# AntoineBlanot/LC2IS

Measured on AMD Instinct MI355X. Metric: training-step images/sec (512x512, ADE20K-150), higher is better.
Workload: dtype bf16; 1 GPU; BaseModelWithText ViT-B/16 + CLIP-text + decoder + fused head/CE train step, 512x512, 151 classes, text len 16, sgd; batch_per_gpu=32, global_batch=32, parallelism=dp1

## Files before the change

include/lc2is_hip.h:

```cpp
#ifndef LC2IS_HIP_H
#define LC2IS_HIP_H
#include <stddef.h>
#include <stdint.h>

#ifdef __cplusplus
extern "C" {
#endif

#define LC2IS_ACT_NONE 0
#define LC2IS_ACT_QUICK_GELU 1
#define LC2IS_ACT_RELU 2
#define LC2IS_ACT_DQUICK_GELU 3
#define LC2IS_ACT_DRELU 4
#define LC2IS_ACT_QUICK_GELU_GRAD 5
#define LC2IS_ACT_MUL_AUX 6
#define LC2IS_ACT_GELU_ERF 7
#define LC2IS_ACT_DGELU_ERF 8
#define LC2IS_ACT_ADD_AUX 9

#define LC2IS_INTERP_BICUBIC 0
#define LC2IS_INTERP_BILINEAR 1

typedef void* lc2is_stream_t;

// ... 29 lines not shown
int lc2is_gemm_tn_bf16(const void* dY, int ldy, const void* X, int ldx, float* dW, int ldw, float* db, int M,
                       int N, int K, int accumulate, void* workspace, size_t workspace_bytes,
                       lc2is_stream_t stream);

#define LC2IS_TN_GROUP_MAX 128
typedef struct lc2is_tn_problem {
  const void* dY; const void* X; float* dW; float* db;
  int ldy, ldx, ldw, M, N, K, accumulate;
} lc2is_tn_problem;
size_t lc2is_gemm_tn_grouped_workspace_bytes(const lc2is_tn_problem* problems, int n);
int lc2is_gemm_tn_grouped(const lc2is_tn_problem* problems, int n, void* workspace, size_t workspace_bytes,
                          lc2is_stream_t stream);
int lc2is_release_captured_tables(void);
int lc2is_captured_tables_mark(void);
int lc2is_release_captured_tables_range(int first, int last);

size_t lc2is_colsum_workspace_bytes(int M, int N);
int lc2is_colsum_bf16(const void* dY, int ldy, float* db, int M, int N, int accumulate, void* workspace,
                      size_t workspace_bytes, lc2is_stream_t stream);

int lc2is_layernorm_fwd(const void* x, int ldx, int x_is_bf16, const float* gamma, const float* beta, void* y_bf16,
                        int ldy, float* y_f32, int ldyf, float* mean, float* rstd, int M, int C, float eps,
                        lc2is_stream_t stream);

size_t lc2is_layernorm_bwd_workspace_bytes(int M, int C);
int lc2is_layernorm_bwd(const void* dy_bf16, int lddy, const float* dy_f32, int lddyf, const void* x,
                        int ldx, int x_is_bf16, const float* gamma, const float* mean, const float* rstd,
                        const void* dres, int lddres, int dres_is_bf16, float* dx_f32, int lddx, void* dx_bf16,
                        int lddxb, float* dgamma, float* dbeta, int accumulate, int M, int C, void* workspace,
                        size_t workspace_bytes, lc2is_stream_t stream);

#define LC2IS_LN_PARTIALS_MAX 64
typedef struct {
  const float* partials;
  float* dgamma;
  float* dbeta;
  int nparts;
  int C;
  int accumulate;
} lc2is_ln_partials;
int lc2is_layernorm_bwd_partials(int M, int C);
int lc2is_ln_partials_reduce(const lc2is_ln_partials* items, int n, lc2is_stream_t stream);

int lc2is_attention_fwd(const void* Q, int ldq, const void* K, int ldk, const void* V, int ldv, void* O,
                        int ldo, float* lse2, const float* kbias, int B, int H, int Sq, int Sk, int D,
                        float scale, int causal, lc2is_stream_t stream);

int lc2is_attention_bwd(const void* Q, int ldq, const void* K, int ldk, const void* V, int ldv,
                        const void* O, int ldo, const void* dO, int lddo, void* dQ, int lddq, void* dK,
                        int lddk, void* dV, int lddv, const float* lse2, float* delta, const float* kbias,
                        int B, int H, int Sq, int Sk, int D, float scale, int causal, lc2is_stream_t stream);

int lc2is_attention_fwd_dropout(const void* Q, int ldq, const void* K, int ldk, const void* V, int ldv, void* O,
                                int ldo, float* lse2, const float* kbias, int B, int H, int Sq, int Sk, int D,
                                float scale, int causal, float p_drop, unsigned long long seed, lc2is_stream_t stream);
int lc2is_attention_bwd_dropout(const void* Q, int ldq, const void* K, int ldk, const void* V, int ldv,
                                const void* O, int ldo, const void* dO, int lddo, void* dQ, int lddq, void* dK,
                                int lddk, void* dV, int lddv, const float* lse2, float* delta, const float* kbias,
                                int B, int H, int Sq, int Sk, int D, float scale, int causal, float p_drop,
                                unsigned long long seed, lc2is_stream_t stream);

int lc2is_dropout_rows_f32(const float* x, int ldx, const float* resid, int ldr, float* y32, int ldy, void* y16,
                           int ldy16, int M, int C, int rows_per_sample, float p, unsigned long long seed,
                           lc2is_stream_t stream);
int lc2is_dropout_rows_bf16(const void* x, int ldx, void* y, int ldy, int M, int C, float p, unsigned long long seed,
                            lc2is_stream_t stream);
int lc2is_dropout_mask(unsigned char* out, long rows, int cols, float p, unsigned long long seed, lc2is_stream_t stream);


int lc2is_shadow_refresh(const lc2is_shadow_desc* descs, int ndesc, int total_tiles, lc2is_stream_t stream);
int lc2is_cast_f32_bf16(const float* src, int ld_src, void* dst_bf16, int ld_dst, int M, int C,
                        lc2is_stream_t stream);
int lc2is_transpose_bf16(const void* src, int ld_src, void* dst, int ld_dst, int R, int C,
                         lc2is_stream_t stream);
int lc2is_transpose_bf16_batched(const void* src, int ld_src, long stride_src, void* dst, int ld_dst, long stride_dst,
                                 int R, int C, int batch, lc2is_stream_t stream);

int lc2is_patchify(const float* pixels, void* out_bf16, int ld_out, int B, int H, int W, int patch,
                   lc2is_stream_t stream);
int lc2is_vit_embed_fwd(const float* patch, int ld_patch, const float* cls, const float* pos, float* x,
                        int ldx, int B, int P, int C, lc2is_stream_t stream);
int lc2is_vit_embed_bwd(const float* dx, int ldx, float* dpos, float* dcls, void* dpatch_bf16, int ld_dpatch,
                        int B, int P, int C, int accumulate, lc2is_stream_t stream);
int lc2is_text_embed_fwd(const int64_t* ids, const float* tok, const float* pos, float* x, int ldx, int B,
                         int L, int C, int vocab, lc2is_stream_t stream);
int lc2is_text_embed_bwd(const int64_t* ids, const float* dx, int ldx, float* dtok, float* dpos, int B, int L,
                         int C, int vocab, int accumulate, lc2is_stream_t stream);
int lc2is_rows_copy_f32(const float* src, int S_src, int src_off, float* dst_f32, void* dst_bf16, int S_dst,
                        int dst_off, int B, int n, int C, lc2is_stream_t stream);
int lc2is_rows_copy_bf16(const void* src, int S_src, int src_off, float* dst_f32, void* dst_bf16, int S_dst,
                         int dst_off, int B, int n, int C, lc2is_stream_t stream);

int lc2is_sgd_step(float* params, const float* grads, float* momentum_buf, size_t n, float lr, float momentum,
                   float weight_decay, float grad_scale, lc2is_stream_t stream);
int lc2is_adamw_step(float* params, const float* grads, float* exp_avg, float* exp_avg_sq, size_t n, float lr,
                     float beta1, float beta2, float eps, float weight_decay, int step, float grad_scale,
                     lc2is_stream_t stream);

size_t lc2is_head_upsample_ce_workspace_bytes(int B, int h, int w, int C, int S, int mode, int want_grad);
int lc2is_head_upsample_ce(const float* scores_lo, int ld, const int64_t* labels, float* dscores_lo,
                           float* scores_hi, float* loss_sum, int B, int h, int w, int C, int S, int mode,
                           long ignore_index, float grad_scale, void* workspace, size_t workspace_bytes,
                           lc2is_stream_t stream);
int lc2is_head_upsample_ce_opts(const float* scores_lo, int ld, const int64_t* labels, float* dscores_lo,
                                float* scores_hi, float* loss_sum, int B, int h, int w, int C, int S, int mode,
                                long ignore_index, float grad_scale, const float* class_weight, float label_smoothing,
                                void* workspace, size_t workspace_bytes, lc2is_stream_t stream);
int lc2is_upsample_bwd_nchw(const float* dhi, float* dlo, int ld, int B, int h, int w, int C, int S, int mode,
                            lc2is_stream_t stream);
int lc2is_ce_nchw_fwd(const float* logits, const int64_t* labels, float* lse, float* loss_sum, int B, int C,
                      long HW, long ignore_index, lc2is_stream_t stream);
int lc2is_ce_nchw_bwd(const float* logits, const int64_t* labels, const float* lse, const float* grad_scale_dev,
                      float grad_scale, float* dlogits, int B, int C, long HW, long ignore_index,
                      lc2is_stream_t stream);
int lc2is_ce_nchw_fwd_opts(const float* logits, const int64_t* labels, float* lse, float* loss_sum, float* loss_px,
                           int B, int C, long HW, long ignore_index, const float* class_weight, float label_smoothing,
                           lc2is_stream_t stream);
int lc2is_ce_nchw_bwd_opts(const float* logits, const int64_t* labels, const float* lse, const float* grad_scale_dev,
                           float grad_scale, const float* grad_px, float* dlogits, int B, int C, long HW,
                           long ignore_index, const float* class_weight, float label_smoothing,
                           lc2is_stream_t stream);
size_t lc2is_ce_nchw_fwd_workspace_bytes(int B, long HW);
int lc2is_ce_nchw_fwd_ordered(const float* logits, const int64_t* labels, float* lse, float* loss_sum, float* loss_px,
                              int B, int C, long HW, long ignore_index, const float* class_weight, float label_smoothing,
                              void* workspace, size_t workspace_bytes, lc2is_stream_t stream);

int lc2is_bilinear_up_fwd(const float* in, float* out_f32, void* out_bf16, int B, int h, int w, int C, int S,
                          lc2is_stream_t stream);
int lc2is_bilinear_up_bwd(const float* dout, float* din_f32, void* din_bf16, int B, int h, int w, int C, int S,
                          int accumulate, lc2is_stream_t stream);
int lc2is_sr_gather(const void* src_bf16, void* dst_bf16, int B, int h, int w, int C, int scatter,
                    lc2is_stream_t stream);
int lc2is_sr_scatter_add_f32(const void* src_bf16, float* dst_f32, int B, int h, int w, int C, lc2is_stream_t stream);
int lc2is_l2norm_fwd(const float* x, float* y_f32, void* y_bf16, float* inv_norm, int M, int C, float eps,
                     lc2is_stream_t stream);
int lc2is_l2norm_bwd(const float* dy, const float* x, const float* inv_norm, float* dx, int M, int C, float eps,
                     lc2is_stream_t stream);
int lc2is_add_n(const float* a, const float* b, const float* c, const float* d, float* out_f32, void* out_bf16,
                size_t n, lc2is_stream_t stream);

int lc2is_rows_gather(const void* src, int ld_src, int src_bf16, void* dst, int ld_dst, int dst_bf16, const int* map,
                      const float* add, int ld_add, int rows, int cols, lc2is_stream_t stream);
int lc2is_swin_attn_fwd(const void* qkv, int ld, void* out, int ldo, float* lse, const float* bias, int nwin,
                        int win_per_img, int nwx, int Hp, int Wp, int ws, int shift, int nH, int C, float scale,
                        lc2is_stream_t stream);
size_t lc2is_swin_attn_bwd_workspace_bytes(int nwin, int ws, int nH);
int lc2is_swin_attn_bwd(const void* qkv, int ld, const void* o, int ld_o, const void* dout, int lddo, const float* lse,
                        const float* bias, void* dqkv, int lddq, float* dbias, int accumulate_dbias, int nwin,
                        int win_per_img, int nwx, int Hp, int Wp, int ws, int shift, int nH, int C, float scale,
                        void* workspace, size_t workspace_bytes, lc2is_stream_t stream);

int lc2is_swin_bias_table_grad(const float* dbias, const int* offsets, const int* positions, float* dtable, int nH, int SS,
                               int T, int accumulate, lc2is_stream_t stream);

int lc2is_resample_u8(const void* src_u8, int H, int W, int C, void* dst_u8, int out_size, int axis, const int* bounds,
                      const int* kk, int ksize, lc2is_stream_t stream);
int lc2is_gather2d_u8(const void* src_u8, int H, int W, int C, void* dst_u8, int out_h, int out_w, const int* yi,
                      const int* xi, lc2is_stream_t stream);
int lc2is_crop_lut(const void* src_u8, int H, int W, int C, int top, int left, int S, const float* lut_f32,
                   float* dst_f32, const int64_t* lut_i64, int64_t* dst_i64, lc2is_stream_t stream);

int lc2is_rows_ce(const float* x, const int64_t* labels, float* lse, float* loss_sum, float* dx, float grad_scale,
                  int M, int K, int accumulate_dx, lc2is_stream_t stream);
int lc2is_cols_ce(const float* x, const int64_t* labels, float* loss_sum, float* dx, float grad_scale, int B, int H,
                  int W, int K, lc2is_stream_t stream);
int lc2is_npair(const float* x, const float* x_pos, const float* x_neg, float* res, int n, int n_pos, int n_neg, int d,
                lc2is_stream_t stream);
int lc2is_npair_bwd(const float* x, const float* x_pos, const float* x_neg, const float* dres, float* dx, float* dx_pos,
                    float* dx_neg, float* workspace, int n, int n_pos, int n_neg, int d, lc2is_stream_t stream);
int lc2is_miou_counts(const float* scores_hi, const int64_t* labels_lo, int* counts, int B, int K, int H, int W, int S,
                      lc2is_stream_t stream);

#define LC2IS_RESIZE_TILE 16
size_t lc2is_resize_argmax_workspace_bytes(long n_tiles, int K);
int lc2is_resize_argmax(const float* scores, int ld, int N, int h, int w, int K, const int64_t* desc, long n_tiles,
                        long total_px, const void* gt, int gt_bytes, uint8_t* pred, int* counts, void* workspace,
                        size_t workspace_bytes, lc2is_stream_t stream);

typedef struct {
  int32_t calls;
  int32_t applied;
  int32_t skipped;
  int32_t finite;
  float grad_norm;
  float clip_coef;
  float lr;
  float bc1, bc2;
  float grad_mul;
  int32_t apply;
// ... 108 lines not shown
```

lc2is_amd/csrc/head.hip:

```cpp
#include "common.h"
#include "interp.h"
#include "lc2is_hip.h"

namespace {

constexpr int HT = 16;
constexpr int FMAX = 8;
constexpr int HEAD_THREADS = 512;
constexpr int CMAX = 192;
constexpr int HEAD_PAD = 4;

struct HeadArgs {
  const float* lo; int ld;
  const int64_t* labels;
  float* dlo;
  float* hi_out;
  float* loss_sum;
  int B, h, w, H, W, C, S, mode;
  long ignore_index;
  float gscale;
  float* ws_loss;
  float* ws_dlo;
  int cq;
  const float* cw;
  float eps;
};

__device__ __forceinline__ void lds_add(float* p, float v) {
  __hip_atomic_fetch_add((__attribute__((address_space(3))) float*)LDS_PTR(p), v, __ATOMIC_RELAXED,
                         __HIP_MEMORY_SCOPE_WORKGROUP);
}

template <int MODE>
__global__ __launch_bounds__(HEAD_THREADS) void head_ce_kernel(HeadArgs p) {
  constexpr int NTAP = (MODE == LC2IS_INTERP_BICUBIC) ? 4 : 2;
  extern __shared__ __attribute__((aligned(16))) char smem[];
  const int tid = threadIdx.x, lane = tid & 63, wid = tid >> 6;
  const int tiles_x = (p.W + HT - 1) / HT, tiles_y = (p.H + HT - 1) / HT;
  const int b = blockIdx.x / (tiles_x * tiles_y);
  const int ty = (blockIdx.x / tiles_x) % tiles_y, tx = blockIdx.x % tiles_x;
  const int Y0 = ty * HT, X0 = tx * HT;
  const float inv_scale = 1.f / (float)p.S;

  const Taps ty0 = make_taps(Y0, inv_scale, p.h, MODE);
  const Taps ty1 = make_taps(min(Y0 + HT - 1, p.H - 1), inv_scale, p.h, MODE);
  const Taps tx0 = make_taps(X0, inv_scale, p.w, MODE);
  const Taps tx1 = make_taps(min(X0 + HT - 1, p.W - 1), inv_scale, p.w, MODE);
  const int fy0 = ty0.idx[0], fx0 = tx0.idx[0];
  int fy1 = ty1.idx[0], fx1 = tx1.idx[0];
#pragma unroll
  for (int k = 1; k < 4; ++k) { fy1 = max(fy1, ty1.idx[k]); fx1 = max(fx1, tx1.idx[k]); }
  const int FH = fy1 - fy0 + 1, FW = fx1 - fx0 + 1;

  const int Cp = p.ld;
  float* s_lo = (float*)smem;
  float* s_dlo = s_lo + FMAX * FMAX * Cp;
  const int fsize = FH * FW * Cp;
  for (int i = tid * 4; i < fsize; i += HEAD_THREADS * 4) {
    const int cell = i / Cp, c = i % Cp;
    const int fy = cell / FW, fx = cell % FW;
    const float4 v = *reinterpret_cast<const float4*>(
        p.lo + (((size_t)b * p.h + fy0 + fy) * p.w + fx0 + fx) * p.ld + c);
    *reinterpret_cast<float4*>(s_lo + i) = v;
    if (p.dlo) *reinterpret_cast<float4*>(s_dlo + i) = make_float4(0.f, 0.f, 0.f, 0.f);
  }
  __syncthreads();

  const int py_l = 2 * wid + ((lane >> 4) & 1), px_l = lane & 15;
  const int Yl = Y0 + py_l, Xl = X0 + px_l;
  int my_label = -1;
  const bool my_valid = (Yl < p.H && Xl < p.W);
  if (my_valid && p.labels) {
    const int64_t lab64 = p.labels[((size_t)b * p.H + Yl) * p.W + Xl];
    my_label = (lab64 == (int64_t)p.ignore_index || lab64 < 0 || lab64 >= p.C) ? -1 : (int)lab64;
  }

  const bool c_ok[3] = {lane < p.C, lane + 64 < p.C, lane + 128 < p.C};
  float loss_acc = 0.f, cnt_acc = 0.f;

  for (int px = 0; px < 32; ++px) {
    const int Y = Y0 + 2 * wid + (px >> 4), X = X0 + (px & 15);
    if (Y >= p.H || X >= p.W) continue;
    const int label = __builtin_amdgcn_readlane(my_label, px);
    const Taps ay = make_taps(Y, inv_scale, p.h, MODE);
    const Taps ax = make_taps(X, inv_scale, p.w, MODE);
    float v[3] = {0.f, 0.f, 0.f};
#pragma unroll
    for (int i = 0; i < NTAP; ++i) {
      const float* rowp = s_lo + ((ay.idx[i] - fy0) * FW - fx0) * Cp + lane;
#pragma unroll
      for (int j = 0; j < NTAP; ++j) {
        const float wgt = ay.w[i] * ax.w[j];
        const float* cp = rowp + ax.idx[j] * Cp;
        v[0] += wgt * cp[0];
        v[1] += wgt * cp[64];
        v[2] += wgt * cp[128];
      }
    }
    if (p.hi_out) {
      const size_t plane = (size_t)p.H * p.W;
      float* o = p.hi_out + ((size_t)b * p.C) * plane + (size_t)Y * p.W + X;
      if (c_ok[0]) o[(size_t)lane * plane] = v[0];
      if (c_ok[1]) o[(size_t)(lane + 64) * plane] = v[1];
      if (c_ok[2]) o[(size_t)(lane + 128) * plane] = v[2];
    }
    if (!p.loss_sum) continue;
    const float NEG = -__builtin_inff();
    float m = fmaxf(fmaxf(c_ok[0] ? v[0] : NEG, c_ok[1] ? v[1] : NEG), c_ok[2] ? v[2] : NEG);
// ... 821 lines not shown
      }
      float mxl[4];
#pragma unroll
      for (int r = 0; r < 4; ++r) { mx[r] = row16_max(mx[r]); mxl[r] = -mx[r] * LOG2E; }
      float sum[4] = {0.f, 0.f, 0.f, 0.f};
      float sb[4] = {0.f, 0.f, 0.f, 0.f};
      float ey[4] = {0.f, 0.f, 0.f, 0.f};
#pragma unroll
      for (int t = 0; t < TN; ++t) {
        const float bt = s_ab[CMAX + 16 * t + m];
#pragma unroll
        for (int r = 0; r < 4; ++r) {
          const float e = __builtin_amdgcn_exp2f(__builtin_fmaf(acc[t][r], LOG2E, mxl[r]));
          acc[t][r] = e;
          sum[r] += e;
          sb[r] += e * bt;
          ey[r] += dl[r] == 16 * t ? e : 0.f;
        }
      }
      float inv[4], k1[4], oh[4];
#pragma unroll
      for (int r = 0; r < 4; ++r) {
        const bool counted = lab4[r] >= 0;
        inv[r] = counted ? 1.f / row16_sum(sum[r]) : 0.f;
        const float ay = s_ab[counted ? lab4[r] : 0];
        const float apy = ay * (row16_sum(ey[r]) * inv[r]);
        k1[r] = ces - (row16_sum(sb[r]) * inv[r] - apy);
        oh[r] = ces + apy;
      }
      have_d = true;
#pragma unroll
      for (int t = 0; t < TN; ++t) {
        const float bt = s_ab[CMAX + 16 * t + m];
        f32x4_t gv;
#pragma unroll
        for (int r = 0; r < 4; ++r) gv[r] = (acc[t][r] * inv[r]) * (k1[r] + bt) - (dl[r] == 16 * t ? oh[r] : 0.f);
        f32x4_t dd = {0.f, 0.f, 0.f, 0.f};
        if constexpr (SUMD) dd = dsum[t];
#pragma unroll
        for (int jj = 0; jj < 4; ++jj) dd = __builtin_amdgcn_mfma_f32_16x16x4f32(gv[jj], Bb[jj], dd, 0, 0, 0);
        if constexpr (SUMD) dsum[t] = dd; else acc[t] = dd;
      }
    }
    if (!SUMD || g2 == 1) {
      constexpr int NTURN = (S == 4 && MODE != LC2IS_INTERP_BICUBIC) ? 2 : HEAD_THREADS / 64;
      const int my_turn = (S == 4 && MODE != LC2IS_INTERP_BICUBIC) ? ((wid >> 1) & 1) : wid;
      for (int turn = 0; turn < NTURN; ++turn) {
        __syncthreads();
        if (turn == my_turn && have_d && m < NT * NT) {
          float* dp = s_dlo + gbase + cellm_off;
#pragma unroll
          for (int t = 0; t < TN; ++t) {
            f32x4_t v = *reinterpret_cast<f32x4_t*>(dp + 16 * t);
            if constexpr (SUMD) v += dsum[t]; else v += acc[t];
            *reinterpret_cast<f32x4_t*>(dp + 16 * t) = v;
          }
        }
      }
    }
  }
  __syncthreads();
  {
    const int q4 = p.cq >> 2;
    float* slab = p.ws_dlo + (size_t)blockIdx.x * (F4 * F4) * p.cq;
    for (int i = tid; i < F4 * F4 * q4; i += HEAD_THREADS) {
      const int cell = i / q4, c = (i % q4) * 4;
      *reinterpret_cast<float4*>(slab + (size_t)cell * p.cq + c) = *reinterpret_cast<const float4*>(s_dlo + cell * CS + c);
    }
  }
}

template <int MODE, int S>
__global__ __launch_bounds__(256) void head_finish_kernel(HeadArgs p, int nblk_main) {
  constexpr int NT = (MODE == LC2IS_INTERP_BICUBIC) ? 4 : 2;
  constexpr int OFF = (MODE == LC2IS_INTERP_BICUBIC) ? 1 : 0;
  constexpr int G = HT / S;
  constexpr int F4 = G + NT - 1;
  const int lane = threadIdx.x & 63, wave = threadIdx.x >> 6;
  if (p.loss_sum && blockIdx.x == 0 && wave == 0) {
    float l = 0.f, c = 0.f;
    for (int k = lane; k < nblk_main; k += 64) { l += p.ws_loss[2 * (size_t)k]; c += p.ws_loss[2 * (size_t)k + 1]; }
    l = wave_sum(l);
    c = wave_sum(c);
    if (lane == 0) { p.loss_sum[0] = l; p.loss_sum[1] = c; }
  }
  if (!p.dlo) return;
  const long ncell = (long)p.B * p.h * p.w;
  const long cid = (long)blockIdx.x * 4 + wave;
  if (cid >= ncell) return;
  const int x = (int)(cid % p.w), y = (int)((cid / p.w) % p.h), b = (int)(cid / ((long)p.w * p.h));
  const int tiles_x = (p.W + S / 2 + HT - 1) / HT, tiles_y = (p.H + S / 2 + HT - 1) / HT;
  auto floordiv = [](int a, int d) { return a >= 0 ? a / d : -((-a + d - 1) / d); };
  const int ty_lo = max(0, floordiv(y + 1 + OFF - (F4 - 1), G)), ty_hi = (y == p.h - 1) ? tiles_y - 1 : min(tiles_y - 1, (y + 1 + OFF) / G);
  const int tx_lo = max(0, floordiv(x + 1 + OFF - (F4 - 1), G)), tx_hi = (x == p.w - 1) ? tiles_x - 1 : min(tiles_x - 1, (x + 1 + OFF) / G);
  const int q4 = p.cq >> 2;
  float4 acc = make_float4(0.f, 0.f, 0.f, 0.f);
  for (int ty = ty_lo; ty <= ty_hi; ++ty) {
    const int by = G * ty - 1 - OFF;
    const int fy_lo = max(0, y == 0 ? 0 : y - by), fy_hi = min(F4 - 1, y == p.h - 1 ? F4 - 1 : y - by);
    for (int fy = fy_lo; fy <= fy_hi; ++fy)
      for (int tx = tx_lo; tx <= tx_hi; ++tx) {
        const int bx = G * tx - 1 - OFF;
        const int fx_lo = max(0, x == 0 ? 0 : x - bx), fx_hi = min(F4 - 1, x == p.w - 1 ? F4 - 1 : x - bx);
        const float* slab = p.ws_dlo + (((size_t)b * tiles_y + ty) * tiles_x + tx) * (F4 * F4) * p.cq;
        for (int fx = fx_lo; fx <= fx_hi; ++fx)
          if (lane < q4) {
            const float4 v = *reinterpret_cast<const float4*>(slab + (size_t)(fy * F4 + fx) * p.cq + 4 * lane);
            acc.x += v.x; acc.y += v.y; acc.z += v.z; acc.w += v.w;
          }
      }
  }
  if (4 * lane < p.ld) {
    float* o = p.dlo + (((size_t)b * p.h + y) * p.w + x) * p.ld + 4 * lane;
    if (4 * lane + 0 >= p.C) acc.x = 0.f;
    if (4 * lane + 1 >= p.C) acc.y = 0.f;
    if (4 * lane + 2 >= p.C) acc.z = 0.f;
    if (4 * lane + 3 >= p.C) acc.w = 0.f;
    *reinterpret_cast<float4*>(o) = acc;
  }
}

struct CeOpts { const float* cw; float eps; float* loss_px; const float* grad_px; };

template <bool OPT, bool ORDERED>
__global__ __launch_bounds__(256) void ce_nchw_fwd_kernel(const float* __restrict__ logits,
                                                           const int64_t* __restrict__ labels, float* lse,
                                                           float* out, int B, int C, size_t HW,
                                                           long ignore_index, CeOpts o) {
  const size_t total = (size_t)B * HW;
  float lacc = 0.f, cacc = 0.f;
  float wsum = 0.f;
  if constexpr (OPT) {
    if (o.cw) { for (int c = 0; c < C; ++c) wsum += o.cw[c]; } else wsum = (float)C;
  }
  for (size_t i = (size_t)blockIdx.x * 256 + threadIdx.x; i < total; i += (size_t)gridDim.x * 256) {
    const size_t b = i / HW, px = i % HW;
    const float* base = logits + b * C * HW + px;
    float m = -__builtin_inff();
    for (int c = 0; c < C; ++c) m = fmaxf(m, base[(size_t)c * HW]);
    float s = 0.f, wz = 0.f;
    for (int c = 0; c < C; ++c) {
      const float z = base[(size_t)c * HW];
      s += __expf(z - m);
      if constexpr (OPT) wz += (o.cw ? o.cw[c] : 1.f) * z;
    }
    const float l = m + __logf(s);
    if (lse) lse[i] = l;
    const long lab = (long)labels[i];
    const bool counted = lab != ignore_index && lab >= 0 && lab < C;
    if constexpr (OPT) {
      float li = 0.f;
      if (counted) {
        const float wy = o.cw ? o.cw[lab] : 1.f;
        li = (1.f - o.eps) * wy * (l - base[(size_t)lab * HW]) + (o.eps / (float)C) * (wsum * l - wz);
        lacc += li;
        cacc += wy;
      }
      if (o.loss_px) o.loss_px[i] = li;
    } else if (counted) {
      lacc += l - base[(size_t)lab * HW];
      cacc += 1.f;
    }
  }
  lacc = wave_sum(lacc);
  cacc = wave_sum(cacc);
  if constexpr (ORDERED) {
    __shared__ float red[2][4];
// ... 157 lines not shown
    }
    const float l = lse[i];
    float sb = 0.f;
    for (int c = 0; c < C; ++c) sb += __expf(base[(size_t)c * HW] - l) * beta[c];
    const float apy = alpha[lab] * __expf(base[(size_t)lab * HW] - l);
    const float k1 = ces - (sb - apy), oh = ces + apy;
    for (int c = 0; c < C; ++c)
      dbase[(size_t)c * HW] = gs * (__expf(base[(size_t)c * HW] - l) * (k1 + beta[c]) - (c == lab ? oh : 0.f));
  }
}

template <int MODE>
__global__ __launch_bounds__(256) void upsample_bwd_kernel(const float* __restrict__ dhi, float* dlo, int ld,
                                                            int h, int w, int C, int S) {
  const int y = blockIdx.x, c = blockIdx.y, b = blockIdx.z;
  const int H = h * S, W = w * S;
  const float inv_scale = 1.f / (float)S;
  const float* plane = dhi + ((size_t)b * C + c) * H * W;
  for (int x = threadIdx.x; x < w; x += 256) {
    float acc = 0.f;
    const int Y0 = max(0, S * (y - 2)), Y1 = min(H, S * (y + 3));
    const int X0 = max(0, S * (x - 2)), X1 = min(W, S * (x + 3));
    for (int Y = Y0; Y < Y1; ++Y) {
      const Taps ty = make_taps(Y, inv_scale, h, MODE);
      float wy = 0.f;
#pragma unroll
      for (int k = 0; k < 4; ++k) wy += (ty.idx[k] == y) ? ty.w[k] : 0.f;
      if (wy == 0.f) continue;
      float racc = 0.f;
      for (int X = X0; X < X1; ++X) {
        const Taps tx = make_taps(X, inv_scale, w, MODE);
        float wx = 0.f;
#pragma unroll
        for (int k = 0; k < 4; ++k) wx += (tx.idx[k] == x) ? tx.w[k] : 0.f;
        racc += wx * plane[(size_t)Y * W + X];
      }
      acc += wy * racc;
    }
    dlo[(((size_t)b * h + y) * w + x) * ld + c] = acc;
  }
}

}

extern "C" int lc2is_upsample_bwd_nchw(const float* dhi, float* dlo, int ld, int B, int h, int w, int C, int S,
                                       int mode, lc2is_stream_t stream_) {
  hipStream_t stream = (hipStream_t)stream_;
  if (!dhi || !dlo) return LC2IS_ERR_NULL;
  if (B <= 0 || h <= 0 || w <= 0 || C <= 0 || ld < C || S < 1) return LC2IS_ERR_SHAPE;
  if (mode == LC2IS_INTERP_BICUBIC)
    hipLaunchKernelGGL(upsample_bwd_kernel<LC2IS_INTERP_BICUBIC>, dim3(h, C, B), dim3(256), 0, stream, dhi, dlo,
                       ld, h, w, C, S);
  else if (mode == LC2IS_INTERP_BILINEAR)
    hipLaunchKernelGGL(upsample_bwd_kernel<LC2IS_INTERP_BILINEAR>, dim3(h, C, B), dim3(256), 0, stream, dhi, dlo,
                       ld, h, w, C, S);
  else
    return LC2IS_ERR_UNSUPPORTED;
  return lc2is_check_launch();
}

namespace {
struct HeadGrpPlan { int f4, t4, cq; size_t loss_bytes, dlo_bytes; };
HeadGrpPlan head_grp_plan(int B, int h, int w, int C, int S, int mode, bool want_grad) {
  HeadGrpPlan g;
  g.f4 = head_grp_footprint(mode, S);
  const int H = h * S, W = w * S;
  g.t4 = ((H + S / 2 + HT - 1) / HT) * ((W + S / 2 + HT - 1) / HT);
  g.cq = (C + 3) & ~3;
  g.loss_bytes = ((size_t)B * g.t4 * 2 * sizeof(float) + 255) & ~(size_t)255;
  g.dlo_bytes = want_grad ? (size_t)B * g.t4 * g.f4 * g.f4 * g.cq * sizeof(float) : 0;
  return g;
}
}

extern "C" size_t lc2is_head_upsample_ce_workspace_bytes(int B, int h, int w, int C, int S, int mode, int want_grad) {
  if (B <= 0 || h <= 0 || w <= 0 || C <= 0 || !(S == 4 || S == 8 || S == 16)) return 0;
  if (mode != LC2IS_INTERP_BICUBIC && mode != LC2IS_INTERP_BILINEAR) return 0;
  const HeadGrpPlan g = head_grp_plan(B, h, w, C, S, mode, want_grad != 0);
  return g.loss_bytes + g.dlo_bytes;
}

namespace {
int head_upsample_ce(const float* scores_lo, int ld, const int64_t* labels, float* dscores_lo, float* scores_hi,
                     float* loss_sum, int B, int h, int w, int C, int S, int mode, long ignore_index, float grad_scale,
                     const float* class_weight, float label_smoothing, void* workspace, size_t workspace_bytes,
                     lc2is_stream_t stream_) {
  hipStream_t stream = (hipStream_t)stream_;
  if (!scores_lo) return LC2IS_ERR_NULL;
  if (!scores_hi && !loss_sum) return LC2IS_ERR_NULL;
  if ((loss_sum || dscores_lo) && !labels) return LC2IS_ERR_NULL;
  if (dscores_lo && !loss_sum) return LC2IS_ERR_NULL;
  if (B <= 0 || h <= 0 || w <= 0 || C <= 0 || C > CMAX || ld < C || ld > CMAX || ld % 64) return LC2IS_ERR_SHAPE;
  if (S < 4 || (HT % S != 0 && S % HT != 0)) return LC2IS_ERR_UNSUPPORTED;
  if (mode != LC2IS_INTERP_BICUBIC && mode != LC2IS_INTERP_BILINEAR) return LC2IS_ERR_UNSUPPORTED;
  if (!(label_smoothing >= 0.f && label_smoothing <= 1.f)) return LC2IS_ERR_SHAPE;
  const bool opt = loss_sum && (class_weight || label_smoothing != 0.f);
  if (opt && !(S == 4 || S == 8 || S == 16)) return LC2IS_ERR_UNSUPPORTED;
  const int H = h * S, W = w * S;
  HeadArgs a{scores_lo, ld, labels, dscores_lo, scores_hi, loss_sum, B, h, w, H, W, C, S, mode, ignore_index,
             grad_scale, nullptr, nullptr, 0, class_weight, label_smoothing};
  const int lds_bytes = 2 * FMAX * FMAX * ld * (int)sizeof(float);
  static DevOnce attr_set;
  if (attr_set.need()) {
    const int mx = 2 * FMAX * FMAX * CMAX * (int)sizeof(float);
    if (hipFuncSetAttribute((const void*)head_ce_kernel<LC2IS_INTERP_BICUBIC>,
                            hipFuncAttributeMaxDynamicSharedMemorySize, mx) != hipSuccess ||
        hipFuncSetAttribute((const void*)head_ce_kernel<LC2IS_INTERP_BILINEAR>,
                            hipFuncAttributeMaxDynamicSharedMemorySize, mx) != hipSuccess)
      return LC2IS_ERR_LAUNCH;
    attr_set.done();
  }
  if (S == 4 || S == 8 || S == 16) {
    const int nt = (C + 15) / 16;
    const int tn = nt <= 4 ? 4 : (nt <= 8 ? 8 : (nt <= 10 ? 10 : 12));
    const HeadGrpPlan gp = head_grp_plan(B, h, w, C, S, mode, dscores_lo != nullptr);
    const int f4 = gp.f4, t4 = gp.t4;
    const int lds4 = 2 * f4 * f4 * (ld + HEAD_PAD) * (int)sizeof(float) + HT * HT * (int)sizeof(int) +
                     (opt ? CMAX * (int)sizeof(float) : 0);
    if (loss_sum) {
      if (!workspace || ((size_t)workspace & 15) || workspace_bytes < gp.loss_bytes + gp.dlo_bytes) return LC2IS_ERR_WORKSPACE;
      a.ws_loss = (float*)workspace;
      a.ws_dlo = dscores_lo ? (float*)((char*)workspace + gp.loss_bytes) : nullptr;
      a.cq = gp.cq;
    }
#define LC2IS_HEAD_GRP1(MODE_, TN_, S_, OPT_)                                                                                \
  do {                                                                                                                      \
    static DevOnce attr;                                                                                               \
    if (attr.need()) {                                                                                                            \
      if (hipFuncSetAttribute((const void*)head_ce_grp_kernel<MODE_, TN_, S_, OPT_>, hipFuncAttributeMaxDynamicSharedMemorySize,  \
                              2 * 7 * 7 * (CMAX + HEAD_PAD) * (int)sizeof(float) + HT * HT * (int)sizeof(int) +             \
                                  (OPT_ ? CMAX * (int)sizeof(float) : 0)) != hipSuccess)                                    \
        return LC2IS_ERR_LAUNCH;                                                                                            \
      attr.done();                                                                                                          \
    }                                                                                                                       \
    hipLaunchKernelGGL((head_ce_grp_kernel<MODE_, TN_, S_, OPT_>), dim3(B * t4), dim3(HEAD_THREADS), lds4, stream, a);      \
  } while (0)
#define LC2IS_HEAD_GRP(MODE_, TN_, S_)                                                                                       \
  do {                                                                                                                      \
    if (opt) LC2IS_HEAD_GRP1(MODE_, TN_, S_, true); else LC2IS_HEAD_GRP1(MODE_, TN_, S_, false);                             \
  } while (0)
#define LC2IS_HEAD_GRP_TN(MODE_, S_)                                                                                         \
  do {                                                                                                                      \
    if (tn == 4) LC2IS_HEAD_GRP(MODE_, 4, S_); else if (tn == 8) LC2IS_HEAD_GRP(MODE_, 8, S_);                               \
    else if (tn == 10) LC2IS_HEAD_GRP(MODE_, 10, S_); else LC2IS_HEAD_GRP(MODE_, 12, S_);                                    \
  } while (0)
#define LC2IS_HEAD_GRP_S(MODE_)                                                                                              \
  do {                                                                                                                      \
    if (S == 4) LC2IS_HEAD_GRP_TN(MODE_, 4); else if (S == 8) LC2IS_HEAD_GRP_TN(MODE_, 8); else LC2IS_HEAD_GRP_TN(MODE_, 16); \
  } while (0)
    if (mode == LC2IS_INTERP_BICUBIC) LC2IS_HEAD_GRP_S(LC2IS_INTERP_BICUBIC);
    else LC2IS_HEAD_GRP_S(LC2IS_INTERP_BILINEAR);
#undef LC2IS_HEAD_GRP_S
#undef LC2IS_HEAD_GRP_TN
#undef LC2IS_HEAD_GRP
#undef LC2IS_HEAD_GRP1
    int rc = lc2is_check_launch();
    if (rc || !loss_sum) return rc;
    const long ncell = dscores_lo ? (long)B * h * w : 1;
    const int fgrid = (int)((ncell + 3) / 4);
#define LC2IS_HEAD_FIN(MODE_, S_) hipLaunchKernelGGL((head_finish_kernel<MODE_, S_>), dim3(fgrid), dim3(256), 0, stream, a, B * t4)
    if (mode == LC2IS_INTERP_BICUBIC) { if (S == 4) LC2IS_HEAD_FIN(LC2IS_INTERP_BICUBIC, 4); else if (S == 8) LC2IS_HEAD_FIN(LC2IS_INTERP_BICUBIC, 8); else LC2IS_HEAD_FIN(LC2IS_INTERP_BICUBIC, 16); }
    else { if (S == 4) LC2IS_HEAD_FIN(LC2IS_INTERP_BILINEAR, 4); else if (S == 8) LC2IS_HEAD_FIN(LC2IS_INTERP_BILINEAR, 8); else LC2IS_HEAD_FIN(LC2IS_INTERP_BILINEAR, 16); }
#undef LC2IS_HEAD_FIN
    return lc2is_check_launch();
  }
  const int tiles = ((H + HT - 1) / HT) * ((W + HT - 1) / HT);
  if (mode == LC2IS_INTERP_BICUBIC)
    hipLaunchKernelGGL(head_ce_kernel<LC2IS_INTERP_BICUBIC>, dim3(B * tiles), dim3(HEAD_THREADS), lds_bytes,
                       stream, a);
  else
    hipLaunchKernelGGL(head_ce_kernel<LC2IS_INTERP_BILINEAR>, dim3(B * tiles), dim3(HEAD_THREADS), lds_bytes,
                       stream, a);
  return lc2is_check_launch();
}

size_t ce_nchw_fwd_grid(int B, long HW) {
  size_t g = ((size_t)B * HW + 255) / 256;
  return g > 8192 ? 8192 : g;
}

int ce_nchw_fwd(const float* logits, const int64_t* labels, float* lse, float* loss_sum, float* loss_px, int B, int C,
                long HW, long ignore_index, const float* class_weight, float label_smoothing, void* workspace,
                size_t workspace_bytes, lc2is_stream_t stream_) {
  hipStream_t stream = (hipStream_t)stream_;
  if (!logits || !labels || !loss_sum) return LC2IS_ERR_NULL;
  if (B <= 0 || C <= 0 || HW <= 0) return LC2IS_ERR_SHAPE;
  if (!(label_smoothing >= 0.f && label_smoothing <= 1.f)) return LC2IS_ERR_SHAPE;
  const size_t g = ce_nchw_fwd_grid(B, HW);
  const bool ordered = workspace != nullptr;
  if (ordered && workspace_bytes < 2 * sizeof(float) * g) return LC2IS_ERR_WORKSPACE;
  float* out = ordered ? (float*)workspace : loss_sum;
  const CeOpts o{class_weight, label_smoothing, loss_px, nullptr};
  const bool opt = class_weight || label_smoothing != 0.f || loss_px;
#define LC2IS_CE_FWD(OPT_, ORD_) \
  hipLaunchKernelGGL((ce_nchw_fwd_kernel<OPT_, ORD_>), dim3((int)g), dim3(256), 0, stream, logits, labels, lse, out, B, C, \
                     (size_t)HW, ignore_index, o)
  if (ordered) {
    if (opt) LC2IS_CE_FWD(true, true); else LC2IS_CE_FWD(false, true);
  } else {
    if (opt) LC2IS_CE_FWD(true, false); else LC2IS_CE_FWD(false, false);
  }
#undef LC2IS_CE_FWD
  int rc = lc2is_check_launch();
  if (rc || !ordered) return rc;
  hipLaunchKernelGGL(ce_nchw_finish_kernel, dim3(1), dim3(256), 0, stream, out, (int)g, loss_sum);
  return lc2is_check_launch();
}

int ce_nchw_bwd(const float* logits, const int64_t* labels, const float* lse, const float* grad_scale_dev, float grad_scale,
                const float* grad_px, float* dlogits, int B, int C, long HW, long ignore_index, const float* class_weight,
                float label_smoothing, lc2is_stream_t stream_) {
  hipStream_t stream = (hipStream_t)stream_;
  if (!logits || !labels || !lse || !dlogits) return LC2IS_ERR_NULL;
  if (B <= 0 || C <= 0 || HW <= 0) return LC2IS_ERR_SHAPE;
  if (!(label_smoothing >= 0.f && label_smoothing <= 1.f)) return LC2IS_ERR_SHAPE;
  size_t g = ((size_t)B * HW + 255) / 256;
  if (g > 8192) g = 8192;
  const CeOpts o{class_weight, label_smoothing, nullptr, grad_px};
  if (class_weight || label_smoothing != 0.f || grad_px)
    hipLaunchKernelGGL(ce_nchw_bwd_kernel<true>, dim3((int)g), dim3(256), 0, stream, logits, labels, lse, grad_scale_dev,
                       grad_scale, dlogits, B, C, (size_t)HW, ignore_index, o);
  else
    hipLaunchKernelGGL(ce_nchw_bwd_kernel<false>, dim3((int)g), dim3(256), 0, stream, logits, labels, lse, grad_scale_dev,
                       grad_scale, dlogits, B, C, (size_t)HW, ignore_index, o);
  return lc2is_check_launch();
}
}

extern "C" int lc2is_head_upsample_ce(const float* scores_lo, int ld, const int64_t* labels, float* dscores_lo,
                                      float* scores_hi, float* loss_sum, int B, int h, int w, int C, int S,
                                      int mode, long ignore_index, float grad_scale, void* workspace,
                                      size_t workspace_bytes, lc2is_stream_t stream) {
  return head_upsample_ce(scores_lo, ld, labels, dscores_lo, scores_hi, loss_sum, B, h, w, C, S, mode, ignore_index,
                          grad_scale, nullptr, 0.f, workspace, workspace_bytes, stream);
}

extern "C" int lc2is_head_upsample_ce_opts(const float* scores_lo, int ld, const int64_t* labels, float* dscores_lo,
                                           float* scores_hi, float* loss_sum, int B, int h, int w, int C, int S,
                                           int mode, long ignore_index, float grad_scale, const float* class_weight,
                                           float label_smoothing, void* workspace, size_t workspace_bytes,
                                           lc2is_stream_t stream) {
  return head_upsample_ce(scores_lo, ld, labels, dscores_lo, scores_hi, loss_sum, B, h, w, C, S, mode, ignore_index,
                          grad_scale, class_weight, label_smoothing, workspace, workspace_bytes, stream);
}

extern "C" int lc2is_head_upsample_px(const float* scores_lo, int ld, const int64_t* labels, float* loss_px, int B, int h,
                                      int w, int C, int S, int mode, long ignore_index, lc2is_stream_t stream_) {
  hipStream_t stream = (hipStream_t)stream_;
  if (!scores_lo || !labels || !loss_px) return LC2IS_ERR_NULL;
  if (B <= 0 || h <= 0 || w <= 0 || C <= 0 || C > CMAX || ld < C || ld > CMAX || ld % 64) return LC2IS_ERR_SHAPE;
  if (((size_t)scores_lo | (size_t)loss_px) & 15) return LC2IS_ERR_SHAPE;
  if (!(S == 4 || S == 8 || S == 16)) return LC2IS_ERR_UNSUPPORTED;
  if (mode != LC2IS_INTERP_BICUBIC && mode != LC2IS_INTERP_BILINEAR) return LC2IS_ERR_UNSUPPORTED;
  const int H = h * S, W = w * S;
  HeadArgs a{scores_lo, ld, labels, nullptr, nullptr, nullptr, B, h, w, H, W, C, S, mode, ignore_index,
             0.f, nullptr, nullptr, 0, nullptr, 0.f};
  const int nt = (C + 15) / 16;
  const int tn = nt <= 4 ? 4 : (nt <= 8 ? 8 : (nt <= 10 ? 10 : 12));
  const HeadGrpPlan gp = head_grp_plan(B, h, w, C, S, mode, false);
  const int lds = gp.f4 * gp.f4 * (ld + HEAD_PAD) * (int)sizeof(float) + HT * HT * (int)sizeof(int);
#define LC2IS_HEAD_PX(MODE_, TN_, S_) \
  hipLaunchKernelGGL((head_px_grp_kernel<MODE_, TN_, S_>), dim3(B * gp.t4), dim3(HEAD_THREADS), lds, stream, a, loss_px)
#define LC2IS_HEAD_PX_TN(MODE_, S_)                                                                 \
  do {                                                                                              \
    if (tn == 4) LC2IS_HEAD_PX(MODE_, 4, S_); else if (tn == 8) LC2IS_HEAD_PX(MODE_, 8, S_);        \
    else if (tn == 10) LC2IS_HEAD_PX(MODE_, 10, S_); else LC2IS_HEAD_PX(MODE_, 12, S_);             \
  } while (0)
#define LC2IS_HEAD_PX_S(MODE_)                                                                                            \
  do {                                                                                                                    \
    if (S == 4) LC2IS_HEAD_PX_TN(MODE_, 4); else if (S == 8) LC2IS_HEAD_PX_TN(MODE_, 8); else LC2IS_HEAD_PX_TN(MODE_, 16); \
  } while (0)
  if (mode == LC2IS_INTERP_BICUBIC) LC2IS_HEAD_PX_S(LC2IS_INTERP_BICUBIC);
  else LC2IS_HEAD_PX_S(LC2IS_INTERP_BILINEAR);
#undef LC2IS_HEAD_PX_S
#undef LC2IS_HEAD_PX_TN
#undef LC2IS_HEAD_PX
  return lc2is_check_launch();
}

namespace {
struct DicePlan { HeadGrpPlan g; int nblk; size_t stat_bytes, part_bytes, coef_bytes; };
size_t dice_align(size_t n) { return (n + 255) & ~(size_t)255; }
DicePlan dice_head_plan(int B, int h, int w, int C, int S, int mode, bool want_grad) {
  DicePlan d;
  d.g = head_grp_plan(B, h, w, C, S, mode, want_grad);
  d.nblk = B * d.g.t4;
  d.stat_bytes = dice_align((size_t)d.nblk * 3 * d.g.cq * sizeof(float));
  d.part_bytes = dice_align((size_t)d.nblk * 2 * sizeof(float));
  d.coef_bytes = dice_align((size_t)(2 * d.g.cq + 4) * sizeof(float));
  return d;
}
bool dice_weights_ok(float ce_weight, float dice_weight, float smooth, float grad_scale) {
  auto ok = [](float v) { return v >= 0.f && v <= 3.0e38f; };
  return ok(ce_weight) && ok(dice_weight) && ok(smooth) && (ce_weight > 0.f || dice_weight > 0.f) && grad_scale == grad_scale;
}
int dice_nchw_grid(int B, long HW) {
  const size_t g = ((size_t)B * HW + 255) / 256;
  return (int)(g > 2048 ? 2048 : g);
}
}

extern "C" size_t lc2is_head_upsample_ce_dice_workspace_bytes(int B, int h, int w, int C, int S, int mode, int want_grad) {
  if (B <= 0 || h <= 0 || w <= 0 || C <= 0 || C > CMAX || !(S == 4 || S == 8 || S == 16)) return 0;
  if (mode != LC2IS_INTERP_BICUBIC && mode != LC2IS_INTERP_BILINEAR) return 0;
  const DicePlan d = dice_head_plan(B, h, w, C, S, mode, want_grad != 0);
  return d.stat_bytes + d.part_bytes + d.coef_bytes + d.g.dlo_bytes;
}

extern "C" int lc2is_head_upsample_ce_dice(const float* scores_lo, int ld, const int64_t* labels, float* dscores_lo,
                                           float* loss_out, float* class_stats, int B, int h, int w, int C, int S, int mode,
                                           long ignore_index, float ce_weight, float dice_weight, float smooth,
                                           int present_only, float grad_scale, void* workspace, size_t workspace_bytes,
                                           lc2is_stream_t stream_) {
  hipStream_t stream = (hipStream_t)stream_;
  if (!scores_lo || !labels || !loss_out) return LC2IS_ERR_NULL;
  if (B <= 0 || h <= 0 || w <= 0 || C <= 0 || C > CMAX || ld < C || ld > CMAX || ld % 64) return LC2IS_ERR_SHAPE;
  if (((size_t)scores_lo | (size_t)dscores_lo) & 15) return LC2IS_ERR_SHAPE;
  if (!dice_weights_ok(ce_weight, dice_weight, smooth, grad_scale)) return LC2IS_ERR_SHAPE;
  if (!(S == 4 || S == 8 || S == 16)) return LC2IS_ERR_UNSUPPORTED;
  if (mode != LC2IS_INTERP_BICUBIC && mode != LC2IS_INTERP_BILINEAR) return LC2IS_ERR_UNSUPPORTED;
  const DicePlan dp = dice_head_plan(B, h, w, C, S, mode, dscores_lo != nullptr);
  if (!workspace || ((size_t)workspace & 15) ||
      workspace_bytes < dp.stat_bytes + dp.part_bytes + dp.coef_bytes + dp.g.dlo_bytes)
    return LC2IS_ERR_WORKSPACE;
  char* wsp = (char*)workspace;
// ... 146 lines not shown
```

lc2is_amd/csrc/layernorm.hip:

```cpp
#include "common.h"
#include "lc2is_hip.h"
#include <cstdlib>

namespace {

#ifndef LN_BWD_OCC
#define LN_BWD_OCC 4
#endif
constexpr int LN_MAXV = 8;

__device__ __forceinline__ float4 load_bf16x4(const bf16_t* p) {
  const uint2 pk = *reinterpret_cast<const uint2*>(p);
  return make_float4(bf16_to_f32((bf16_t)(pk.x & 0xffff)), bf16_to_f32((bf16_t)(pk.x >> 16)),
                     bf16_to_f32((bf16_t)(pk.y & 0xffff)), bf16_to_f32((bf16_t)(pk.y >> 16)));
}

template <int NV>
__global__ __launch_bounds__(256) void ln_fwd_kernel(const float* __restrict__ x, const bf16_t* __restrict__ xb, int ldx,
                                                      const float* __restrict__ gamma,
                                                      const float* __restrict__ beta, bf16_t* y, int ldy,
                                                      float* yf, int ldyf, float* mean_out, float* rstd_out,
                                                      int M, int C, float eps) {
  const int lane = threadIdx.x & 63;
  const int C4 = C >> 2;
  float4 gm[NV], bt[NV];
#pragma unroll
  for (int i = 0; i < NV; ++i) {
    const int c4 = lane + 64 * i;
    gm[i] = (c4 < C4) ? reinterpret_cast<const float4*>(gamma)[c4] : make_float4(0.f, 0.f, 0.f, 0.f);
    bt[i] = (beta && c4 < C4) ? reinterpret_cast<const float4*>(beta)[c4] : make_float4(0.f, 0.f, 0.f, 0.f);
  }
  const int stride = gridDim.x * 4;
  int row = blockIdx.x * 4 + (threadIdx.x >> 6);
  if (row >= M) return;
  auto load_row = [&](int r, float4 (&dst)[NV]) __attribute__((always_inline)) {
    if (xb) {
#pragma unroll
      for (int i = 0; i < NV; ++i) {
        const int c4 = lane + 64 * i;
        dst[i] = (c4 < C4) ? load_bf16x4(xb + (size_t)r * ldx + 4 * c4) : make_float4(0.f, 0.f, 0.f, 0.f);
      }
      return;
    }
    const float4* xr = reinterpret_cast<const float4*>(x + (size_t)r * ldx);
#pragma unroll
    for (int i = 0; i < NV; ++i) {
      const int c4 = lane + 64 * i;
      dst[i] = (c4 < C4) ? xr[c4] : make_float4(0.f, 0.f, 0.f, 0.f);
    }
  };
  float4 v[NV], nx[NV];
  load_row(row, v);
  for (; row < M; row += stride) {
    const bool more = row + stride < M;
    if (more) load_row(row + stride, nx);
    float s = 0.f;
#pragma unroll
    for (int i = 0; i < NV; ++i) {
      const int c4 = lane + 64 * i;
      if (c4 < C4) s += (v[i].x + v[i].y) + (v[i].z + v[i].w);
    }
    const float mean = wave_sum(s) / (float)C;
    float q = 0.f;
#pragma unroll
    for (int i = 0; i < NV; ++i) {
      const int c4 = lane + 64 * i;
      if (c4 < C4) {
        const float a = v[i].x - mean, b = v[i].y - mean, c = v[i].z - mean, d = v[i].w - mean;
        q += (a * a + b * b) + (c * c + d * d);
      }
    }
    const float rstd = rsqrtf(wave_sum(q) / (float)C + eps);
    if (lane == 0) {
      if (mean_out) mean_out[row] = mean;
      if (rstd_out) rstd_out[row] = rstd;
    }
#pragma unroll
    for (int i = 0; i < NV; ++i) {
      const int c4 = lane + 64 * i;
      if (c4 < C4) {
        float4 o;
        o.x = (v[i].x - mean) * rstd * gm[i].x;
        o.y = (v[i].y - mean) * rstd * gm[i].y;
        o.z = (v[i].z - mean) * rstd * gm[i].z;
        o.w = (v[i].w - mean) * rstd * gm[i].w;
        if (beta) { o.x += bt[i].x; o.y += bt[i].y; o.z += bt[i].z; o.w += bt[i].w; }
        if (y) {
          uint2 pk = make_uint2(pack_bf16x2(o.x, o.y), pack_bf16x2(o.z, o.w));
          *reinterpret_cast<uint2*>(y + (size_t)row * ldy + 4 * c4) = pk;
        }
        if (yf) *reinterpret_cast<float4*>(yf + (size_t)row * ldyf + 4 * c4) = o;
      }
    }
    if (more) {
#pragma unroll
      for (int i = 0; i < NV; ++i) v[i] = nx[i];
    }
  }
}

__device__ __forceinline__ float4 load_dy4(const bf16_t* dyb, const float* dyf, size_t off) {
  if (dyf) return *reinterpret_cast<const float4*>(dyf + off);
  return load_bf16x4(dyb + off);
}

template <int NV>
__global__ __launch_bounds__(256, (NV <= 3 ? LN_BWD_OCC : NV == 4 ? 3 : NV <= 6 ? 2 : 1)) void ln_bwd_kernel(const bf16_t* __restrict__ dyb, int lddy,
                                                      const float* __restrict__ dyf, int lddyf,
                                                      const float* __restrict__ x, const bf16_t* __restrict__ xb, int ldx,
                                                      const float* __restrict__ gamma,
                                                      const float* __restrict__ mean,
                                                      const float* __restrict__ rstd,
                                                      const float* __restrict__ dres, const bf16_t* __restrict__ dresb, int lddres,
                                                      float* dxf, int lddx, bf16_t* dxb, int lddxb,
                                                      float* ws, int M, int C) {
  __shared__ float red[4 * 2048];
  const int lane = threadIdx.x & 63, wave = threadIdx.x >> 6;
  const int C4 = C >> 2;
  float4 gm[NV], dg[NV], db[NV];
#pragma unroll
  for (int i = 0; i < NV; ++i) {
    const int c4 = lane + 64 * i;
    gm[i] = (c4 < C4) ? reinterpret_cast<const float4*>(gamma)[c4] : make_float4(0.f, 0.f, 0.f, 0.f);
    dg[i] = make_float4(0.f, 0.f, 0.f, 0.f);
    db[i] = make_float4(0.f, 0.f, 0.f, 0.f);
  }
  const int ldy_ = dyf ? lddyf : lddy;
  for (int row = blockIdx.x * 4 + wave; row < M; row += gridDim.x * 4) {
    const float mu = mean[row], rs = rstd[row];
    float4 xh[NV], dy[NV], rv[NV];
    float s1 = 0.f, s2 = 0.f;
#pragma unroll
    for (int i = 0; i < NV; ++i) {
      const int c4 = lane + 64 * i;
      if (dresb) rv[i] = (c4 < C4) ? load_bf16x4(dresb + (size_t)row * lddres + 4 * c4) : make_float4(0.f, 0.f, 0.f, 0.f);
      else rv[i] = (dres && c4 < C4) ? *reinterpret_cast<const float4*>(dres + (size_t)row * lddres + 4 * c4)
                                     : make_float4(0.f, 0.f, 0.f, 0.f);
    }
#pragma unroll
    for (int i = 0; i < NV; ++i) {
      const int c4 = lane + 64 * i;
      if (c4 < C4) {
        float4 xv;
        if (xb) {
          xv = load_bf16x4(xb + (size_t)row * ldx + 4 * c4);
        } else {
          const f32x4_t xv_ = __builtin_nontemporal_load(reinterpret_cast<const f32x4_t*>(x + (size_t)row * ldx + 4 * c4));
          xv = make_float4(xv_[0], xv_[1], xv_[2], xv_[3]);
        }
        dy[i] = load_dy4(dyb, dyf, (size_t)row * ldy_ + 4 * c4);
        xh[i] = make_float4((xv.x - mu) * rs, (xv.y - mu) * rs, (xv.z - mu) * rs, (xv.w - mu) * rs);
        const float a = dy[i].x * gm[i].x, b = dy[i].y * gm[i].y, c = dy[i].z * gm[i].z, d = dy[i].w * gm[i].w;
        s1 += (a + b) + (c + d);
        s2 += (a * xh[i].x + b * xh[i].y) + (c * xh[i].z + d * xh[i].w);
        dg[i].x += dy[i].x * xh[i].x; dg[i].y += dy[i].y * xh[i].y;
        dg[i].z += dy[i].z * xh[i].z; dg[i].w += dy[i].w * xh[i].w;
        db[i].x += dy[i].x; db[i].y += dy[i].y; db[i].z += dy[i].z; db[i].w += dy[i].w;
      }
    }
    const float c1 = wave_sum(s1) / (float)C, c2 = wave_sum(s2) / (float)C;
#pragma unroll
    for (int i = 0; i < NV; ++i) {
      const int c4 = lane + 64 * i;
      if (c4 < C4) {
        float4 o;
        o.x = rs * (dy[i].x * gm[i].x - c1 - xh[i].x * c2);
        o.y = rs * (dy[i].y * gm[i].y - c1 - xh[i].y * c2);
        o.z = rs * (dy[i].z * gm[i].z - c1 - xh[i].z * c2);
        o.w = rs * (dy[i].w * gm[i].w - c1 - xh[i].w * c2);
        o.x += rv[i].x; o.y += rv[i].y; o.z += rv[i].z; o.w += rv[i].w;
        if (dxf) __builtin_nontemporal_store(f32x4_t{o.x, o.y, o.z, o.w}, reinterpret_cast<f32x4_t*>(dxf + (size_t)row * lddx + 4 * c4));
        if (dxb) {
          uint2 pk = make_uint2(pack_bf16x2(o.x, o.y), pack_bf16x2(o.z, o.w));
          __builtin_nontemporal_store(i32x2_t{(int)pk.x, (int)pk.y}, reinterpret_cast<i32x2_t*>(dxb + (size_t)row * lddxb + 4 * c4));
        }
      }
    }
  }
  float* r = red;
// ... 30 lines not shown
#pragma unroll
  for (int i = 0; i < NV; ++i) {
    const int c4 = lane + 64 * i;
    gm[i] = (c4 < C4) ? reinterpret_cast<const float4*>(gamma)[c4] : make_float4(0.f, 0.f, 0.f, 0.f);
    dg[i] = make_float4(0.f, 0.f, 0.f, 0.f);
    db[i] = make_float4(0.f, 0.f, 0.f, 0.f);
  }
  struct Raw { uint2 dy[NV], rv[NV]; f32x4_t xf[XB ? 1 : NV]; uint2 xb[XB ? NV : 1]; };
  auto load_row = [&](int row, Raw& r) __attribute__((always_inline)) {
#pragma unroll
    for (int i = 0; i < NV; ++i) {
      const int c4 = lane + 64 * i;
      const bool ok = c4 < C4;
      r.rv[i] = (dresb && ok) ? *reinterpret_cast<const uint2*>(dresb + (size_t)row * lddres + 4 * c4) : make_uint2(0u, 0u);
      r.dy[i] = ok ? *reinterpret_cast<const uint2*>(dyb + (size_t)row * lddy + 4 * c4) : make_uint2(0u, 0u);
      if constexpr (XB) r.xb[i] = ok ? *reinterpret_cast<const uint2*>((const bf16_t*)xv_ + (size_t)row * ldx + 4 * c4) : make_uint2(0u, 0u);
      else r.xf[i] = ok ? __builtin_nontemporal_load(reinterpret_cast<const f32x4_t*>((const float*)xv_ + (size_t)row * ldx + 4 * c4))
                        : f32x4_t{0.f, 0.f, 0.f, 0.f};
    }
  };
  auto widen = [](uint2 pk) {
    return make_float4(bf16_to_f32((bf16_t)(pk.x & 0xffff)), bf16_to_f32((bf16_t)(pk.x >> 16)),
                       bf16_to_f32((bf16_t)(pk.y & 0xffff)), bf16_to_f32((bf16_t)(pk.y >> 16)));
  };
  const int stride = gridDim.x * 4;
  int row = blockIdx.x * 4 + wave;
  Raw cur, nxt;
  if (row < M) load_row(row, cur);
  for (; row < M; row += stride) {
    const bool more = row + stride < M;
    if (more) load_row(row + stride, nxt);
    const float mu = mean[row], rs = rstd[row];
    float4 xh[NV], dy[NV];
    float s1 = 0.f, s2 = 0.f;
#pragma unroll
    for (int i = 0; i < NV; ++i) {
      const int c4 = lane + 64 * i;
      if (c4 < C4) {
        float4 xv;
        if constexpr (XB) xv = widen(cur.xb[i]);
        else xv = make_float4(cur.xf[i][0], cur.xf[i][1], cur.xf[i][2], cur.xf[i][3]);
        dy[i] = widen(cur.dy[i]);
        xh[i] = make_float4((xv.x - mu) * rs, (xv.y - mu) * rs, (xv.z - mu) * rs, (xv.w - mu) * rs);
        const float a = dy[i].x * gm[i].x, b = dy[i].y * gm[i].y, c = dy[i].z * gm[i].z, d = dy[i].w * gm[i].w;
        s1 += (a + b) + (c + d);
        s2 += (a * xh[i].x + b * xh[i].y) + (c * xh[i].z + d * xh[i].w);
        dg[i].x += dy[i].x * xh[i].x; dg[i].y += dy[i].y * xh[i].y;
        dg[i].z += dy[i].z * xh[i].z; dg[i].w += dy[i].w * xh[i].w;
        db[i].x += dy[i].x; db[i].y += dy[i].y; db[i].z += dy[i].z; db[i].w += dy[i].w;
      }
    }
    const float c1 = wave_sum(s1) / (float)C, c2 = wave_sum(s2) / (float)C;
#pragma unroll
    for (int i = 0; i < NV; ++i) {
      const int c4 = lane + 64 * i;
      if (c4 < C4) {
        const float4 rv = widen(cur.rv[i]);
        float4 o;
        o.x = rs * (dy[i].x * gm[i].x - c1 - xh[i].x * c2);
        o.y = rs * (dy[i].y * gm[i].y - c1 - xh[i].y * c2);
        o.z = rs * (dy[i].z * gm[i].z - c1 - xh[i].z * c2);
        o.w = rs * (dy[i].w * gm[i].w - c1 - xh[i].w * c2);
        o.x += rv.x; o.y += rv.y; o.z += rv.z; o.w += rv.w;
        uint2 pk = make_uint2(pack_bf16x2(o.x, o.y), pack_bf16x2(o.z, o.w));
        __builtin_nontemporal_store(i32x2_t{(int)pk.x, (int)pk.y}, reinterpret_cast<i32x2_t*>(dxb + (size_t)row * lddxb + 4 * c4));
      }
    }
    if (more) cur = nxt;
  }
  float* r = red;
#pragma unroll
  for (int pass = 0; pass < 2; ++pass) {
    __syncthreads();
#pragma unroll
    for (int i = 0; i < NV; ++i) {
      const int c4 = lane + 64 * i;
      if (c4 < C4) *reinterpret_cast<float4*>(r + wave * 2048 + 4 * c4) = pass ? db[i] : dg[i];
    }
    __syncthreads();
    for (int c = threadIdx.x; c < C; c += 256) {
      const float t = (r[c] + r[2048 + c]) + (r[4096 + c] + r[6144 + c]);
      ws[((size_t)blockIdx.x * 2 + pass) * C + c] = t;
    }
  }
}

__global__ __launch_bounds__(256) void ln_bwd_reduce_kernel(const float* __restrict__ ws, int nblk, int C,
                                                             float* dgamma, float* dbeta, int accumulate) {
  const int c = blockIdx.x * 256 + threadIdx.x;
  if (c >= C) return;
  float g = 0.f, b = 0.f;
  for (int k = 0; k < nblk; ++k) {
    g += ws[((size_t)k * 2 + 0) * C + c];
    b += ws[((size_t)k * 2 + 1) * C + c];
  }
  if (dgamma) dgamma[c] = accumulate ? dgamma[c] + g : g;
  if (dbeta) dbeta[c] = accumulate ? dbeta[c] + b : b;
}

inline int ln_bwd_blocks(int M, int C) {
  const int nv = (C / 4 + 63) / 64;
  const int cap = 256 * (nv <= 3 ? LN_BWD_OCC : nv == 4 ? 3 : nv <= 6 ? 2 : 1);
  int nb = (M + 3) / 4;
  return nb > cap ? cap : nb;
}

}

static int ln_fwd_blocks(int M) {
  static const int cap = getenv("LC2IS_LN_FWD_BLOCKS") ? atoi(getenv("LC2IS_LN_FWD_BLOCKS")) : 2048;
  const int need = (M + 3) / 4;
  return need < cap ? need : (cap > 0 ? cap : need);
}

extern "C" int lc2is_layernorm_fwd(const void* x, int ldx, int x_is_bf16, const float* gamma, const float* beta,
                                   void* y_bf16, int ldy, float* y_f32, int ldyf, float* mean, float* rstd,
                                   int M, int C, float eps, lc2is_stream_t stream_) {
  hipStream_t stream = (hipStream_t)stream_;
  if (!x || !gamma || (!y_bf16 && !y_f32)) return LC2IS_ERR_NULL;
  const float* xf = x_is_bf16 ? nullptr : (const float*)x;
  const bf16_t* xb = x_is_bf16 ? (const bf16_t*)x : nullptr;
  if (M <= 0 || C <= 0 || C % 4 || C > LN_MAXV * 256) return LC2IS_ERR_SHAPE;
  if (ldx < C || ldx % 4 || (y_bf16 && (ldy < C || ldy % 4)) || (y_f32 && (ldyf < C || ldyf % 4)))
    return LC2IS_ERR_SHAPE;
#define LN_FWD(NV_)                                                                                  \
  hipLaunchKernelGGL(ln_fwd_kernel<NV_>, dim3(ln_fwd_blocks(M)), dim3(256), 0, stream, xf, xb, ldx, gamma, beta, \
                     (bf16_t*)y_bf16, ldy, y_f32, ldyf, mean, rstd, M, C, eps)
  const int nv = (C / 4 + 63) / 64;
  if (nv <= 1) LN_FWD(1); else if (nv == 2) LN_FWD(2); else if (nv == 3) LN_FWD(3);
  else if (nv == 4) LN_FWD(4); else if (nv <= 6) LN_FWD(6); else LN_FWD(8);
#undef LN_FWD
  return lc2is_check_launch();
}

extern "C" size_t lc2is_layernorm_bwd_workspace_bytes(int M, int C) {
  if (M <= 0 || C <= 0) return 0;
  return (size_t)ln_bwd_blocks(M, C) * 2 * (size_t)C * sizeof(float);
}

extern "C" int lc2is_layernorm_bwd(const void* dy_bf16, int lddy, const float* dy_f32, int lddyf,
                                   const void* x, int ldx, int x_is_bf16, const float* gamma, const float* mean,
                                   const float* rstd, const void* dres, int lddres, int dres_is_bf16, float* dx_f32,
                                   int lddx, void* dx_bf16, int lddxb, float* dgamma, float* dbeta, int accumulate,
                                   int M, int C, void* workspace, size_t workspace_bytes,
                                   lc2is_stream_t stream_) {
  hipStream_t stream = (hipStream_t)stream_;
  const float* xf = x_is_bf16 ? nullptr : (const float*)x;
  const bf16_t* xb = x_is_bf16 ? (const bf16_t*)x : nullptr;
  const float* dresf = dres_is_bf16 ? nullptr : (const float*)dres;
  const bf16_t* dresb = dres_is_bf16 ? (const bf16_t*)dres : nullptr;
  if ((!dy_bf16 && !dy_f32) || !x || !gamma || !mean || !rstd || (!dx_f32 && !dx_bf16)) return LC2IS_ERR_NULL;
  if (M <= 0 || C <= 0 || C % 4 || C > LN_MAXV * 256) return LC2IS_ERR_SHAPE;
  if (ldx < C || ldx % 4) return LC2IS_ERR_SHAPE;
  if ((dy_f32 ? (lddyf < C || lddyf % 4) : (lddy < C || lddy % 4))) return LC2IS_ERR_SHAPE;
  if ((dres && (lddres < C || lddres % 4)) || (dx_f32 && (lddx < C || lddx % 4)) ||
      (dx_bf16 && (lddxb < C || lddxb % 4)))
    return LC2IS_ERR_SHAPE;
  if (!workspace || workspace_bytes < lc2is_layernorm_bwd_workspace_bytes(M, C)) return LC2IS_ERR_WORKSPACE;
  const int nblk = ln_bwd_blocks(M, C);
  const int nv = (C / 4 + 63) / 64;
  static const bool lean_on = !(getenv("LC2IS_LN_BWD_LEAN") && atoi(getenv("LC2IS_LN_BWD_LEAN")) == 0);
  if (lean_on && dy_bf16 && !dy_f32 && !dx_f32 && dx_bf16 && (!dres || dres_is_bf16) && nv <= 4) {
    const int cap = 256 * (nv <= 2 ? 4 : nv == 3 ? 3 : 2);
    const int lgrid = nblk < cap ? nblk : cap;
#define LN_LEAN(NV_)                                                                                                       \
  do {                                                                                                                     \
    if (x_is_bf16)                                                                                                         \
      hipLaunchKernelGGL((ln_bwd_lean_kernel<NV_, true>), dim3(lgrid), dim3(256), 0, stream, (const bf16_t*)dy_bf16, lddy, x, \
                         ldx, gamma, mean, rstd, (const bf16_t*)dres, lddres, (bf16_t*)dx_bf16, lddxb, (float*)workspace, nblk, M, C); \
    else                                                                                                                   \
      hipLaunchKernelGGL((ln_bwd_lean_kernel<NV_, false>), dim3(lgrid), dim3(256), 0, stream, (const bf16_t*)dy_bf16, lddy, x, \
                         ldx, gamma, mean, rstd, (const bf16_t*)dres, lddres, (bf16_t*)dx_bf16, lddxb, (float*)workspace, nblk, M, C); \
  } while (0)
    if (nv <= 1) LN_LEAN(1); else if (nv == 2) LN_LEAN(2); else if (nv == 3) LN_LEAN(3); else LN_LEAN(4);
#undef LN_LEAN
    int rc = lc2is_check_launch();
    if (rc) return rc;
    if (dgamma || dbeta) {
      hipLaunchKernelGGL(partials_reduce_kernel, dim3((C + 31) / 32, 2), dim3(1024), 0, stream,
                         (const float*)workspace, nblk, (size_t)2 * C, (size_t)C, C, dgamma, dbeta, accumulate);
      rc = lc2is_check_launch();
    }
    return rc;
  }
#define LN_BWD(NV_)                                                                                   \
  hipLaunchKernelGGL(ln_bwd_kernel<NV_>, dim3(nblk), dim3(256), 0, stream, (const bf16_t*)dy_bf16, lddy, \
                     dy_f32, lddyf, xf, xb, ldx, gamma, mean, rstd, dresf, dresb, lddres, dx_f32, lddx,  \
                     (bf16_t*)dx_bf16, lddxb, (float*)workspace, M, C)
  if (nv <= 1) LN_BWD(1); else if (nv == 2) LN_BWD(2); else if (nv == 3) LN_BWD(3);
  else if (nv == 4) LN_BWD(4); else if (nv <= 6) LN_BWD(6); else LN_BWD(8);
#undef LN_BWD
  int rc = lc2is_check_launch();
  if (rc) return rc;
  if (dgamma || dbeta) {
    hipLaunchKernelGGL(partials_reduce_kernel, dim3((C + 31) / 32, 2), dim3(1024), 0, stream,
                       (const float*)workspace, nblk, (size_t)2 * C, (size_t)C, C, dgamma, dbeta, accumulate);
    rc = lc2is_check_launch();
  }
  return rc;
}

extern "C" int lc2is_layernorm_bwd_partials(int M, int C) {
  if (M <= 0 || C <= 0 || C % 4 || C > LN_MAXV * 256) return 0;
  return ln_bwd_blocks(M, C);
}

namespace {
struct LnPartialsGroup {
  lc2is_ln_partials item[LC2IS_LN_PARTIALS_MAX];
};
__global__ __launch_bounds__(1024) void ln_partials_reduce_grouped_kernel(LnPartialsGroup g) {
  const lc2is_ln_partials& it = g.item[blockIdx.z];
  if ((int)blockIdx.x * 32 >= it.C) return;
  float* out = blockIdx.y ? it.dbeta : it.dgamma;
  if (!out) return;
  partials_reduce_body(it.partials + (size_t)blockIdx.y * it.C, it.nparts, (size_t)2 * it.C, it.C, out, it.accumulate,
                       blockIdx.x);
}
}

extern "C" int lc2is_ln_partials_reduce(const lc2is_ln_partials* items, int n, lc2is_stream_t stream_) {
  hipStream_t stream = (hipStream_t)stream_;
  if (!items) return LC2IS_ERR_NULL;
  if (n <= 0 || n > LC2IS_LN_PARTIALS_MAX) return LC2IS_ERR_SHAPE;
  LnPartialsGroup g{};
  int cmax = 0;
  for (int i = 0; i < n; ++i) {
    const lc2is_ln_partials& it = items[i];
    if (!it.partials || (!it.dgamma && !it.dbeta)) return LC2IS_ERR_NULL;
    if (it.nparts <= 0 || it.C <= 0 || it.C % 4) return LC2IS_ERR_SHAPE;
    for (int j = 0; j < i; ++j)
      if ((it.dgamma && (it.dgamma == items[j].dgamma || it.dgamma == items[j].dbeta)) ||
          (it.dbeta && (it.dbeta == items[j].dgamma || it.dbeta == items[j].dbeta)))
        return LC2IS_ERR_UNSUPPORTED;
    g.item[i] = it;
    cmax = it.C > cmax ? it.C : cmax;
  }
  hipLaunchKernelGGL(ln_partials_reduce_grouped_kernel, dim3((cmax + 31) / 32, 2, n), dim3(1024), 0, stream, g);
  return lc2is_check_launch();
}
```

lc2is_amd/csrc/misc.hip:

```cpp
#include "common.h"
#include "lc2is_hip.h"

namespace {

__global__ __launch_bounds__(256) void shadow_refresh_kernel(const lc2is_shadow_desc* __restrict__ descs,
                                                              int ndesc) {
  __shared__ bf16_t tile[64][66];
  int lo = 0, hi = ndesc - 1;
  const int bid = blockIdx.x;
  while (lo < hi) {
    const int mid = (lo + hi + 1) >> 1;
    if (descs[mid].tile_start <= bid) lo = mid; else hi = mid - 1;
  }
  const lc2is_shadow_desc d = descs[lo];
  const int t = bid - d.tile_start;
  const int tk = (d.K + 63) / 64;
  const int n0 = (t / tk) * 64, k0 = (t % tk) * 64;
  const float* src = (const float*)d.src;
  bf16_t* dst = (bf16_t*)d.dst;
  bf16_t* dstT = (bf16_t*)d.dstT;
  const int tx = threadIdx.x & 15, ty = threadIdx.x >> 4;
#pragma unroll
  for (int r = 0; r < 4; ++r) {
    const int n = n0 + ty + 16 * r, k = k0 + 4 * tx;
// ... 141 lines not shown
      *dc = cacc;
    }
  }
}

__global__ __launch_bounds__(256) void text_embed_fwd_kernel(const int64_t* __restrict__ ids,
                                                              const float* __restrict__ tok,
                                                              const float* __restrict__ pos, float* x, int ldx,
                                                              int BL, int L, int C, int vocab) {
  const int C4 = C >> 2;
  const size_t total = (size_t)BL * C4;
  for (size_t i = (size_t)blockIdx.x * 256 + threadIdx.x; i < total; i += (size_t)gridDim.x * 256) {
    const int c4 = (int)(i % C4), r = (int)(i / C4);
    int64_t id = ids[r];
    if (id < 0) id = 0;
    if (id >= vocab) id = vocab - 1;
    const float4 t = *reinterpret_cast<const float4*>(tok + (size_t)id * C + 4 * c4);
    const float4 pe = *reinterpret_cast<const float4*>(pos + (size_t)(r % L) * C + 4 * c4);
    *reinterpret_cast<float4*>(x + (size_t)r * ldx + 4 * c4) =
        make_float4(t.x + pe.x, t.y + pe.y, t.z + pe.z, t.w + pe.w);
  }
}

__global__ __launch_bounds__(256) void text_embed_dtok_kernel(const int64_t* __restrict__ ids, const float* __restrict__ dx,
                                                               int ldx, float* dtok, int R, int C, int vocab) {
  const int r = blockIdx.x;
  auto clampid = [&](int64_t v) { return v < 0 ? (int64_t)0 : (v >= vocab ? (int64_t)(vocab - 1) : v); };
  const int64_t id = clampid(ids[r]);
  int seen = 0;
  for (int q = threadIdx.x; q < r; q += 256) seen |= (clampid(ids[q]) == id);
  if (__syncthreads_or(seen)) return;
  for (int c = threadIdx.x; c < C; c += 256) {
    float acc = 0.f;
    for (int q = r; q < R; ++q)
      if (clampid(ids[q]) == id) acc += dx[(size_t)q * ldx + c];
    dtok[(size_t)id * C + c] += acc;
  }
}

__global__ __launch_bounds__(256) void text_embed_bwd_kernel(const float* __restrict__ dx, int ldx, float* dpos, int B, int L,
                                                              int C, int accumulate) {
  const int total = L * C;
  for (int i = blockIdx.x * 256 + threadIdx.x; i < total; i += gridDim.x * 256) {
    const int c = i % C, l = i / C;
    float acc = 0.f;
    for (int b = 0; b < B; ++b) acc += dx[((size_t)b * L + l) * ldx + c];
    dpos[(size_t)l * C + c] = accumulate ? dpos[(size_t)l * C + c] + acc : acc;
  }
}

__global__ __launch_bounds__(256) void rows_copy_bf16_kernel(const bf16_t* __restrict__ src, int S_src, int src_off,
                                                              float* dst, bf16_t* dst_b, int S_dst, int dst_off,
                                                              int B, int n, int C) {
  const int C4 = C >> 2;
  const size_t total = (size_t)B * n * C4;
  for (size_t i = (size_t)blockIdx.x * 256 + threadIdx.x; i < total; i += (size_t)gridDim.x * 256) {
    const int c4 = (int)(i % C4);
    const int r = (int)(i / C4);
    const int s = r % n, b = r / n;
    const uint2 pk = *reinterpret_cast<const uint2*>(src + ((size_t)b * S_src + src_off + s) * C + 4 * c4);
    const size_t o = ((size_t)b * S_dst + dst_off + s) * C + 4 * c4;
    if (dst) *reinterpret_cast<float4*>(dst + o) = make_float4(bf16_to_f32((bf16_t)(pk.x & 0xffff)), bf16_to_f32((bf16_t)(pk.x >> 16)),
                                                               bf16_to_f32((bf16_t)(pk.y & 0xffff)), bf16_to_f32((bf16_t)(pk.y >> 16)));
    if (dst_b) *reinterpret_cast<uint2*>(dst_b + o) = pk;
  }
}

__global__ __launch_bounds__(256) void rows_copy_kernel(const float* __restrict__ src, int S_src, int src_off,
                                                         float* dst, bf16_t* dst_b, int S_dst, int dst_off,
                                                         int B, int n, int C) {
  const int C4 = C >> 2;
  const size_t total = (size_t)B * n * C4;
  for (size_t i = (size_t)blockIdx.x * 256 + threadIdx.x; i < total; i += (size_t)gridDim.x * 256) {
    const int c4 = (int)(i % C4);
    const int r = (int)(i / C4);
    const int s = r % n, b = r / n;
    const float4 v = *reinterpret_cast<const float4*>(src + ((size_t)b * S_src + src_off + s) * C + 4 * c4);
    const size_t o = ((size_t)b * S_dst + dst_off + s) * C + 4 * c4;
    if (dst) *reinterpret_cast<float4*>(dst + o) = v;
    if (dst_b) *reinterpret_cast<uint2*>(dst_b + o) = make_uint2(pack_bf16x2(v.x, v.y), pack_bf16x2(v.z, v.w));
  }
}

__global__ __launch_bounds__(256) void sgd_kernel(float* p, const float* __restrict__ g, float* mom, size_t n4,
                                                   float lr, float momentum, float wd, float gscale) {
  for (size_t i = (size_t)blockIdx.x * 256 + threadIdx.x; i < n4; i += (size_t)gridDim.x * 256) {
    float4 pv = reinterpret_cast<float4*>(p)[i];
    const float4 gv = reinterpret_cast<const float4*>(g)[i];
    float d[4] = {gv.x * gscale + wd * pv.x, gv.y * gscale + wd * pv.y, gv.z * gscale + wd * pv.z,
                  gv.w * gscale + wd * pv.w};
    if (mom) {
      float4 mv = reinterpret_cast<float4*>(mom)[i];
      mv.x = momentum * mv.x + d[0]; mv.y = momentum * mv.y + d[1];
      mv.z = momentum * mv.z + d[2]; mv.w = momentum * mv.w + d[3];
      reinterpret_cast<float4*>(mom)[i] = mv;
      d[0] = mv.x; d[1] = mv.y; d[2] = mv.z; d[3] = mv.w;
    }
    pv.x -= lr * d[0]; pv.y -= lr * d[1]; pv.z -= lr * d[2]; pv.w -= lr * d[3];
    reinterpret_cast<float4*>(p)[i] = pv;
  }
}

__global__ __launch_bounds__(256) void adamw_kernel(float* p, const float* __restrict__ g, float* m, float* v,
                                                     size_t n4, float lr, float b1, float b2, float eps,
                                                     float wd, float bc1, float bc2, float gscale) {
  for (size_t i = (size_t)blockIdx.x * 256 + threadIdx.x; i < n4; i += (size_t)gridDim.x * 256) {
    float4 pv = reinterpret_cast<float4*>(p)[i];
    const float4 gv = reinterpret_cast<const float4*>(g)[i];
    float4 mv = reinterpret_cast<float4*>(m)[i], vv = reinterpret_cast<float4*>(v)[i];
    float* pp = &pv.x; const float* gp = &gv.x; float* mp = &mv.x; float* vp = &vv.x;
#pragma unroll
    for (int k = 0; k < 4; ++k) {
      const float gg = gp[k] * gscale;
      pp[k] *= (1.f - lr * wd);
      mp[k] = b1 * mp[k] + (1.f - b1) * gg;
      vp[k] = b2 * vp[k] + (1.f - b2) * gg * gg;
      const float denom = sqrtf(vp[k]) / sqrtf(bc2) + eps;
      pp[k] -= (lr / bc1) * (mp[k] / denom);
    }
    reinterpret_cast<float4*>(p)[i] = pv;
    reinterpret_cast<float4*>(m)[i] = mv;
    reinterpret_cast<float4*>(v)[i] = vv;
  }
}

inline int ew_grid(size_t work_items) {
  size_t g = (work_items + 255) / 256;
  if (g > 4096) g = 4096;
  if (g < 1) g = 1;
  return (int)g;
}

}

extern "C" int lc2is_shadow_refresh(const lc2is_shadow_desc* descs_dev, int ndesc, int total_tiles,
                                    lc2is_stream_t stream_) {
  hipStream_t stream = (hipStream_t)stream_;
  if (!descs_dev) return LC2IS_ERR_NULL;
  if (ndesc <= 0 || total_tiles <= 0) return LC2IS_ERR_SHAPE;
  hipLaunchKernelGGL(shadow_refresh_kernel, dim3(total_tiles), dim3(256), 0, stream, descs_dev, ndesc);
  return lc2is_check_launch();
}

extern "C" int lc2is_cast_f32_bf16(const float* src, int ld_src, void* dst, int ld_dst, int M, int C,
                                   lc2is_stream_t stream_) {
  hipStream_t stream = (hipStream_t)stream_;
  if (!src || !dst) return LC2IS_ERR_NULL;
  if (M <= 0 || C <= 0 || C % 4 || ld_src < C || ld_dst < C || ld_src % 4 || ld_dst % 4) return LC2IS_ERR_SHAPE;
  hipLaunchKernelGGL(cast_f32_bf16_kernel, dim3(ew_grid((size_t)M * C / 4)), dim3(256), 0, stream, src, ld_src,
                     (bf16_t*)dst, ld_dst, M, C);
  return lc2is_check_launch();
}

extern "C" int lc2is_transpose_bf16(const void* src, int ld_src, void* dst, int ld_dst, int R, int C,
                                    lc2is_stream_t stream_) {
  hipStream_t stream = (hipStream_t)stream_;
  if (!src || !dst) return LC2IS_ERR_NULL;
  if (R <= 0 || C <= 0 || ld_src < C || ld_dst < R) return LC2IS_ERR_SHAPE;
  hipLaunchKernelGGL(transpose_bf16_kernel, dim3((C + 63) / 64, (R + 63) / 64), dim3(256), 0, stream,
                     (const bf16_t*)src, ld_src, (bf16_t*)dst, ld_dst, R, C, 0L, 0L);
  return lc2is_check_launch();
}

extern "C" int lc2is_transpose_bf16_batched(const void* src, int ld_src, long stride_src, void* dst, int ld_dst,
                                            long stride_dst, int R, int C, int batch, lc2is_stream_t stream_) {
  hipStream_t stream = (hipStream_t)stream_;
// ... 13 lines not shown
  if (ld_out < kdim) return LC2IS_ERR_SHAPE;
  if (patch % 8 == 0 && W % 8 == 0 && ld_out % 8 == 0 && ((uintptr_t)pixels & 15) == 0 && ((uintptr_t)out_bf16 & 15) == 0)
    hipLaunchKernelGGL(patchify8_kernel, dim3(ew_grid((size_t)B * 3 * H * W / 8)), dim3(256), 0, stream, pixels, (bf16_t*)out_bf16,
                       ld_out, B, H, W, patch, G);
  else
    hipLaunchKernelGGL(patchify_kernel, dim3(B * G * 3 * patch), dim3(256), 0, stream, pixels, (bf16_t*)out_bf16,
                       ld_out, B, H, W, patch, G);
  int rc = lc2is_check_launch();
  if (rc || ld_out == kdim) return rc;
  hipLaunchKernelGGL(zero_pad_cols_kernel, dim3(ew_grid((size_t)B * G * G * (ld_out - kdim))), dim3(256), 0,
                     stream, (bf16_t*)out_bf16, ld_out, B * G * G, kdim);
  return lc2is_check_launch();
}

extern "C" int lc2is_vit_embed_fwd(const float* patch, int ld_patch, const float* cls, const float* pos,
                                   float* x, int ldx, int B, int P, int C, lc2is_stream_t stream_) {
  hipStream_t stream = (hipStream_t)stream_;
  if (!patch || !cls || !pos || !x) return LC2IS_ERR_NULL;
  if (B <= 0 || P <= 0 || C <= 0 || C % 4 || ld_patch < C || ld_patch % 4 || ldx < C || ldx % 4)
    return LC2IS_ERR_SHAPE;
  hipLaunchKernelGGL(vit_embed_fwd_kernel, dim3(ew_grid((size_t)B * (P + 1) * C / 4)), dim3(256), 0, stream,
                     patch, ld_patch, cls, pos, x, ldx, B, P, C);
  return lc2is_check_launch();
}

extern "C" int lc2is_vit_embed_bwd(const float* dx, int ldx, float* dpos, float* dcls, void* dpatch_bf16,
                                   int ld_dpatch, int B, int P, int C, int accumulate, lc2is_stream_t stream_) {
  hipStream_t stream = (hipStream_t)stream_;
  if (!dx || !dpos || !dcls) return LC2IS_ERR_NULL;
  if (B <= 0 || P <= 0 || C <= 0 || C % 4 || ldx < C || ldx % 4 || (dpatch_bf16 && (ld_dpatch < C || ld_dpatch % 4)))
    return LC2IS_ERR_SHAPE;
  hipLaunchKernelGGL(vit_embed_bwd_kernel, dim3(ew_grid((size_t)(P + 1) * C / 4)), dim3(256), 0, stream, dx, ldx,
                     dpos, dcls, (bf16_t*)dpatch_bf16, ld_dpatch, B, P, C, accumulate);
  return lc2is_check_launch();
}

extern "C" int lc2is_text_embed_fwd(const int64_t* ids, const float* tok, const float* pos, float* x, int ldx,
                                    int B, int L, int C, int vocab, lc2is_stream_t stream_) {
  hipStream_t stream = (hipStream_t)stream_;
  if (!ids || !tok || !pos || !x) return LC2IS_ERR_NULL;
  if (B <= 0 || L <= 0 || C <= 0 || C % 4 || vocab <= 0 || ldx < C || ldx % 4) return LC2IS_ERR_SHAPE;
  hipLaunchKernelGGL(text_embed_fwd_kernel, dim3(ew_grid((size_t)B * L * C / 4)), dim3(256), 0, stream, ids, tok,
                     pos, x, ldx, B * L, L, C, vocab);
  return lc2is_check_launch();
}

extern "C" int lc2is_text_embed_bwd(const int64_t* ids, const float* dx, int ldx, float* dtok, float* dpos,
                                    int B, int L, int C, int vocab, int accumulate, lc2is_stream_t stream_) {
  hipStream_t stream = (hipStream_t)stream_;
  if (!ids || !dx || !dtok || !dpos) return LC2IS_ERR_NULL;
  if (B <= 0 || L <= 0 || C <= 0 || vocab <= 0 || ldx < C) return LC2IS_ERR_SHAPE;
  hipLaunchKernelGGL(text_embed_dtok_kernel, dim3(B * L), dim3(256), 0, stream, ids, dx, ldx, dtok, B * L, C, vocab);
  int rc = lc2is_check_launch();
  if (rc) return rc;
  hipLaunchKernelGGL(text_embed_bwd_kernel, dim3(ew_grid((size_t)L * C)), dim3(256), 0, stream, dx, ldx, dpos, B, L, C,
                     accumulate);
  return lc2is_check_launch();
}

extern "C" int lc2is_rows_copy_f32(const float* src, int S_src, int src_off, float* dst_f32, void* dst_bf16,
                                   int S_dst, int dst_off, int B, int n, int C, lc2is_stream_t stream_) {
  hipStream_t stream = (hipStream_t)stream_;
  if (!src || (!dst_f32 && !dst_bf16)) return LC2IS_ERR_NULL;
  if (B <= 0 || n <= 0 || C <= 0 || C % 4 || src_off < 0 || dst_off < 0 || src_off + n > S_src ||
      dst_off + n > S_dst)
    return LC2IS_ERR_SHAPE;
  hipLaunchKernelGGL(rows_copy_kernel, dim3(ew_grid((size_t)B * n * C / 4)), dim3(256), 0, stream, src, S_src,
                     src_off, dst_f32, (bf16_t*)dst_bf16, S_dst, dst_off, B, n, C);
  return lc2is_check_launch();
}

extern "C" int lc2is_rows_copy_bf16(const void* src, int S_src, int src_off, float* dst_f32, void* dst_bf16,
                                    int S_dst, int dst_off, int B, int n, int C, lc2is_stream_t stream_) {
  hipStream_t stream = (hipStream_t)stream_;
  if (!src || (!dst_f32 && !dst_bf16)) return LC2IS_ERR_NULL;
  if (B <= 0 || n <= 0 || C <= 0 || C % 4 || src_off < 0 || dst_off < 0 || src_off + n > S_src ||
      dst_off + n > S_dst)
    return LC2IS_ERR_SHAPE;
  hipLaunchKernelGGL(rows_copy_bf16_kernel, dim3(ew_grid((size_t)B * n * C / 4)), dim3(256), 0, stream, (const bf16_t*)src,
                     S_src, src_off, dst_f32, (bf16_t*)dst_bf16, S_dst, dst_off, B, n, C);
  return lc2is_check_launch();
}

extern "C" int lc2is_sgd_step(float* params, const float* grads, float* momentum_buf, size_t n, float lr,
                              float momentum, float weight_decay, float grad_scale, lc2is_stream_t stream_) {
  hipStream_t stream = (hipStream_t)stream_;
  if (!params || !grads) return LC2IS_ERR_NULL;
  if (n == 0 || n % 4) return LC2IS_ERR_SHAPE;
  hipLaunchKernelGGL(sgd_kernel, dim3(ew_grid(n / 4)), dim3(256), 0, stream, params, grads, momentum_buf, n / 4,
                     lr, momentum, weight_decay, grad_scale);
  return lc2is_check_launch();
}

extern "C" int lc2is_adamw_step(float* params, const float* grads, float* exp_avg, float* exp_avg_sq, size_t n,
                                float lr, float beta1, float beta2, float eps, float weight_decay, int step,
                                float grad_scale, lc2is_stream_t stream_) {
  hipStream_t stream = (hipStream_t)stream_;
  if (!params || !grads || !exp_avg || !exp_avg_sq) return LC2IS_ERR_NULL;
  if (n == 0 || n % 4 || step < 1) return LC2IS_ERR_SHAPE;
  const float bc1 = 1.f - powf(beta1, (float)step), bc2 = 1.f - powf(beta2, (float)step);
  hipLaunchKernelGGL(adamw_kernel, dim3(ew_grid(n / 4)), dim3(256), 0, stream, params, grads, exp_avg,
                     exp_avg_sq, n / 4, lr, beta1, beta2, eps, weight_decay, bc1, bc2, grad_scale);
  return lc2is_check_launch();
}
```

lc2is_amd/nn/clip.py:

```python
from __future__ import annotations

import math
from dataclasses import dataclass

import torch
from torch import nn

from .. import ops
from .base import HipModule, WgradBatch, grad_buf, linear_bwd_params, require_cuda, vec_grad


@dataclass
class ClipArch:
    hidden: int = 768
    heads: int = 12
    layers: int = 12
    intermediate: int = 3072
    eps: float = 1e-5
    vocab: int = 49408
    max_pos: int = 77
    eos_token_id: int = 49407


VIT_B16 = ClipArch(768, 12, 12, 3072)
# ... 30 lines not shown


class _VisionEmbeddings(nn.Module):
    def __init__(self, a: ClipArch, image_size: int, patch: int):
        super().__init__()
        self.class_embedding = nn.Parameter(torch.randn(a.hidden))
        self.patch_embedding = nn.Conv2d(3, a.hidden, patch, stride=patch, bias=False)
        self.position_embedding = nn.Embedding((image_size // patch) ** 2 + 1, a.hidden)


class _TextEmbeddings(nn.Module):
    def __init__(self, a: ClipArch):
        super().__init__()
        self.token_embedding = nn.Embedding(a.vocab, a.hidden)
        self.position_embedding = nn.Embedding(a.max_pos, a.hidden)


class _VisionParams(nn.Module):
    def __init__(self, a: ClipArch, image_size: int, patch: int):
        super().__init__()
        self.embeddings = _VisionEmbeddings(a, image_size, patch)
        self.pre_layrnorm = nn.LayerNorm(a.hidden, eps=a.eps)
        self.encoder = _Stack(a)
        self.post_layernorm = nn.LayerNorm(a.hidden, eps=a.eps)


class _TextParams(nn.Module):
    def __init__(self, a: ClipArch):
        super().__init__()
        self.embeddings = _TextEmbeddings(a)
        self.encoder = _Stack(a)
        self.final_layer_norm = nn.LayerNorm(a.hidden, eps=a.eps)


def _clip_init(enc: nn.Module, a: ClipArch) -> None:
    in_std = a.hidden ** -0.5 * (2 * a.layers) ** -0.5
    out_std = a.hidden ** -0.5
    fc_std = (2 * a.hidden) ** -0.5
    with torch.no_grad():
        for layer in enc.encoder.layers:
            for n in ("q_proj", "k_proj", "v_proj"):
                getattr(layer.self_attn, n).weight.normal_(0, in_std)
                getattr(layer.self_attn, n).bias.zero_()
            layer.self_attn.out_proj.weight.normal_(0, out_std)
            layer.self_attn.out_proj.bias.zero_()
            layer.mlp.fc1.weight.normal_(0, fc_std)
            layer.mlp.fc2.weight.normal_(0, in_std)
            layer.mlp.fc1.bias.zero_()
            layer.mlp.fc2.bias.zero_()
        emb = enc.embeddings
        if hasattr(emb, "class_embedding"):
            emb.class_embedding.normal_(0, a.hidden ** -0.5)
            emb.patch_embedding.weight.normal_(0, 0.02)
            emb.position_embedding.weight.normal_(0, 0.02)
        else:
            emb.token_embedding.weight.normal_(0, 0.02)
            emb.position_embedding.weight.normal_(0, 0.02)


def _stack_shadows(stack: _Stack, a: ClipArch, device):
    C, I = a.hidden, a.intermediate
    bf = dict(dtype=torch.bfloat16, device=device)
    per, entries = [], []
    for layer in stack.layers:
        at, mlp = layer.self_attn, layer.mlp
        s = dict(wqkv=torch.empty(3 * C, C, **bf), wqkvT=torch.empty(C, 3 * C, **bf),
                 bqkv=torch.empty(3 * C, dtype=torch.float32, device=device),
                 wo=torch.empty(C, C, **bf), woT=torch.empty(C, C, **bf),
                 w1=torch.empty(I, C, **bf), w1T=torch.empty(C, I, **bf),
                 w2=torch.empty(C, I, **bf), w2T=torch.empty(I, C, **bf))
        for j, proj in enumerate((at.q_proj, at.k_proj, at.v_proj)):
            entries.append((proj.weight, s["wqkv"][j * C:(j + 1) * C], s["wqkvT"][:, j * C:(j + 1) * C]))
            entries.append((proj.bias, s["bqkv"][j * C:(j + 1) * C], None))
        entries.append((at.out_proj.weight, s["wo"], s["woT"]))
        entries.append((mlp.fc1.weight, s["w1"], s["w1T"]))
        entries.append((mlp.fc2.weight, s["w2"], s["w2T"]))
        per.append(s)
    return per, entries


_RESID_BF16 = __import__('os').environ.get("LC2IS_RESID_STREAM", "f32") == "bf16"


def _stack_fwd(x, stack: _Stack, sh, a: ClipArch, B: int, S: int, kbias, causal: bool, save: bool):
    C, H = a.hidden, a.heads
    D = C // H
    scale = D ** -0.5
    saved = []
    lean = x.dtype == torch.bfloat16
    fuse = (not lean) and ops.gemm_nt_ln_ok(x.shape[0], C, C) and ops.gemm_nt_ln_ok(x.shape[0], C, a.intermediate)
    nxt_ln = None
    layers = list(stack.layers)
    for li, (layer, s) in enumerate(zip(layers, sh)):
        if nxt_ln is not None:
            h, m1, r1 = nxt_ln
        else:
            h, _, m1, r1 = ops.layernorm_fwd(x, layer.layer_norm1.weight, layer.layer_norm1.bias, a.eps, save_stats=save)
        qkv, _, _ = ops.gemm_nt(h, s["wqkv"], s["bqkv"])
        o, lse = ops.attention_fwd(qkv[:, :C], qkv[:, C:2 * C], qkv[:, 2 * C:], B, H, S, S, D, scale, causal=causal,
                                   kbias=kbias, save_lse=save)
        if fuse:
            x_mid, h2, m2, r2 = ops.gemm_nt_ln(o, s["wo"], layer.self_attn.out_proj.bias, x, layer.layer_norm2.weight,
                                               layer.layer_norm2.bias, a.eps, save_stats=save)
        else:
            if lean:
                x_mid, _, _ = ops.gemm_nt(o, s["wo"], layer.self_attn.out_proj.bias, resid=x)
            else:
                _, x_mid, _ = ops.gemm_nt(o, s["wo"], layer.self_attn.out_proj.bias, resid=x, out_bf16=None, out_f32=True)
            h2, _, m2, r2 = ops.layernorm_fwd(x_mid, layer.layer_norm2.weight, layer.layer_norm2.bias, a.eps,
                                              save_stats=save)
        act, _, z = ops.gemm_nt(h2, s["w1"], layer.mlp.fc1.bias, act=ops.ACT_QUICK_GELU, aux_out=True if save else None)
        nxt_ln = None
        if fuse and li + 1 < len(layers):
            nl = layers[li + 1].layer_norm1
            x_out, hn, mn, rn = ops.gemm_nt_ln(act, s["w2"], layer.mlp.fc2.bias, x_mid, nl.weight, nl.bias, a.eps, save_stats=save)
            nxt_ln = (hn, mn, rn)
        elif lean:
            x_out, _, _ = ops.gemm_nt(act, s["w2"], layer.mlp.fc2.bias, resid=x_mid)
        else:
            _, x_out, _ = ops.gemm_nt(act, s["w2"], layer.mlp.fc2.bias, resid=x_mid, out_bf16=None, out_f32=True)
        if save:
            saved.append((x, m1, r1, h, qkv, o, lse, x_mid, m2, r2, h2, z, act))
        x = x_out
    return x, saved


_GRAD_STREAM_BF16 = __import__('os').environ.get("LC2IS_GRAD_STREAM", "bf16") != "f32"


def _stack_bwd(g32, g16, stack: _Stack, sh, saved, a: ClipArch, B: int, S: int, kbias, causal: bool, on_layer_done=None,
               final_f32: bool = True):
    C, H = a.hidden, a.heads
    D = C // H
    scale = D ** -0.5
    if on_layer_done is not None:
        default_pair = min(3, len(stack.layers))
    else:
        default_pair = len(stack.layers)
    pair = int(__import__('os').environ.get('LC2IS_WGRAD_PAIR', str(default_pair)))
    batch, waiting = WgradBatch(), []
    batch.__enter__()
    lean = _GRAD_STREAM_BF16
    if lean:
        g32 = None
    first = stack.layers[0]
    try:
        for layer, s, sv in zip(reversed(stack.layers), reversed(sh), reversed(saved)):
            x, m1, r1, h, qkv, o, lse, x_mid, m2, r2, h2, z, act = sv
            at, mlp = layer.self_attn, layer.mlp
            linear_bwd_params(g16, act, mlp.fc2.weight, mlp.fc2.bias)
            dz, _, _ = ops.gemm_nt(g16, s["w2T"], None, act=ops.ACT_DQUICK_GELU, aux_in=z)
            linear_bwd_params(dz, h2, mlp.fc1.weight, mlp.fc1.bias)
            dh2, _, _ = ops.gemm_nt(dz, s["w1T"], None)
            dg, accg = vec_grad(layer.layer_norm2.weight)
            db, _ = vec_grad(layer.layer_norm2.bias)
            gm32, gm16, _, _ = ops.layernorm_bwd(dh2, x_mid, layer.layer_norm2.weight, m2, r2, dres=g16 if lean else g32,
                                                 dgamma=dg, dbeta=db, accumulate=accg, want_f32=not lean,
                                                 need_param_grads=dg is not None)
            linear_bwd_params(gm16, o, at.out_proj.weight, at.out_proj.bias)
            do, _, _ = ops.gemm_nt(gm16, s["woT"], None)
            dqkv = torch.empty_like(qkv)
            ops.attention_bwd(qkv[:, :C], qkv[:, C:2 * C], qkv[:, 2 * C:], o, do, lse, B, H, S, S, D, scale, causal=causal,
                              kbias=kbias, dq=dqkv[:, :C], dk=dqkv[:, C:2 * C], dv=dqkv[:, 2 * C:])
            for j, proj in enumerate((at.q_proj, at.k_proj, at.v_proj)):
                linear_bwd_params(dqkv[:, j * C:(j + 1) * C], h, proj.weight, proj.bias)
            dh, _, _ = ops.gemm_nt(dqkv, s["wqkvT"], None)
            dg, accg = vec_grad(layer.layer_norm1.weight)
            db, _ = vec_grad(layer.layer_norm1.bias)
            g32, g16, _, _ = ops.layernorm_bwd(dh, x, layer.layer_norm1.weight, m1, r1, dres=gm16 if lean else gm32,
                                               dgamma=dg, dbeta=db, accumulate=accg,
                                               want_f32=(not lean) or (final_f32 and layer is first),
                                               need_param_grads=dg is not None)
            waiting.append(layer)
            if len(waiting) >= pair:
# ... 28 lines not shown
        i0 = math.floor(src)
        t = src - i0
        for k, wgt in enumerate((c2(t + 1), c1(t), c1(1 - t), c2(2 - t))):
            U[o, min(max(i0 - 1 + k, 0), n_in - 1)] += wgt
    return U


VIT_PRETRAINED_SIZE = 224


class _VisionFn(torch.autograd.Function):
    @staticmethod
    def forward(ctx, pixel_values, anchor, mod, keep_cls, save):
        out, saved = mod._fwd(pixel_values, keep_cls, save)
        ctx.mod, ctx.saved, ctx.keep_cls = mod, saved, keep_cls
        return out

    @staticmethod
    def backward(ctx, gout):
        ctx.mod._bwd(gout.contiguous(), ctx.saved, ctx.keep_cls)
        ctx.saved = None
        return None, None, None, None, None


class ImageEncoderCLIP(HipModule):

    keep_cls = False

    def __init__(self, in_size: int, patch_size: int = 16, arch: ClipArch | None = None) -> None:
        super().__init__()
        self.in_size, self.patch_size = in_size, patch_size
        if arch is None:
            if patch_size == 16:
                arch = VIT_B16
            elif patch_size == 14:
                arch = VIT_L14
            else:
                raise ValueError("ImageEncoderCLIP: only patch_size 16 (ViT-B/16) and 14 (ViT-L/14) have defaults")
        self.arch = arch
        self.enc = _VisionParams(arch, in_size, patch_size)
        _clip_init(self.enc, arch)

    def hidden_size(self) -> int:
        return self.arch.hidden

    def pos_emebedding_interpolate(self, tgt_size: int, ignore_index: int = 1, weight: torch.Tensor | None = None) -> torch.Tensor:
        w = (self.enc.embeddings.position_embedding.weight if weight is None else weight).detach().double().cpu()
        old = VIT_PRETRAINED_SIZE // self.patch_size
        keep, grid = w[:ignore_index], w[ignore_index:].reshape(old, old, -1)
        U = _interp_matrix_bicubic(old, tgt_size)
        new = torch.einsum("yi,ijc,xj->yxc", U, grid, U).reshape(tgt_size * tgt_size, -1)
        return torch.cat([keep, new], dim=0).float()

    def _load_from_state_dict(self, state_dict, prefix, *args, **kwargs):
        _remap_legacy_keys(state_dict, prefix, "vision_model")
        key = prefix + "enc.embeddings.position_embedding.weight"
        old_rows = (VIT_PRETRAINED_SIZE // self.patch_size) ** 2 + 1
        mine = self.enc.embeddings.position_embedding.weight.shape[0]
        if key in state_dict and state_dict[key].shape[0] == old_rows and mine != old_rows:
            state_dict[key] = self.pos_emebedding_interpolate(self.in_size // self.patch_size, weight=state_dict[key])
        super()._load_from_state_dict(state_dict, prefix, *args, **kwargs)

    def _build_shadows(self, device):
        a = self.arch
        per, entries = _stack_shadows(self.enc.encoder, a, device)
        k = 3 * self.patch_size ** 2
        kpad = (k + 63) // 64 * 64
        wp = torch.zeros(a.hidden, kpad, dtype=torch.bfloat16, device=device)
        entries.append((self.enc.embeddings.patch_embedding.weight.view(a.hidden, k), wp[:, :k], None))
        return dict(layers=per, wpatch=wp, kpad=kpad), entries

    def _fwd(self, pixel_values, keep_cls, save):
        require_cuda(pixel_values, "pixel_values")
        a, sh = self.arch, self._ensure_ready()
        B = pixel_values.shape[0]
        G = self.in_size // self.patch_size
        P = G * G
        if pixel_values.shape[-1] != self.in_size or pixel_values.shape[-2] != self.in_size:
            raise ValueError(f"Input image size ({pixel_values.shape[-2]}*{pixel_values.shape[-1]}) doesn't match "
                             f"model ({self.in_size}*{self.in_size}).")
        emb = self.enc.embeddings
        cols = ops.patchify(pixel_values.float().contiguous(), self.patch_size, sh["kpad"])
        _, pe, _ = ops.gemm_nt(cols, sh["wpatch"], None, out_bf16=None, out_f32=True)
        x0 = ops.vit_embed_fwd(pe, emb.class_embedding, emb.position_embedding.weight, B, P)
        xb, xf, m0, r0 = ops.layernorm_fwd(x0, self.enc.pre_layrnorm.weight, self.enc.pre_layrnorm.bias, a.eps,
                                           save_stats=save, out_bf16=True if _RESID_BF16 else None,
                                           out_f32=None if _RESID_BF16 else True)
        x, saved = _stack_fwd(xb if _RESID_BF16 else xf, self.enc.encoder, sh["layers"], a, B, P + 1, None, False, save)
        if keep_cls and x.dtype == torch.float32:
            out = x.view(B, P + 1, a.hidden)
        else:
            n, off = (P + 1, 0) if keep_cls else (P, 1)
            out = torch.empty(B * n, a.hidden, dtype=torch.float32, device=x.device)
            ops.rows_copy(x, P + 1, off, n, 0, B, n, dst_f32=out)
            out = out.view(B, n, a.hidden)
        return out, (dict(cols=cols, x0=x0, m0=m0, r0=r0, layers=saved, B=B, P=P) if save else None)

    def _bwd(self, gout, saved, keep_cls):
        a, sh = self.arch, self._sh
        B, P = saved["B"], saved["P"]
        C = a.hidden
        if keep_cls:
            g32 = gout.reshape(B * (P + 1), C).float()
            g16 = ops.cast_bf16(g32)
        elif _GRAD_STREAM_BF16:
            g32 = None
            g16 = torch.zeros(B * (P + 1), C, dtype=torch.bfloat16, device=gout.device)
            ops.rows_copy(gout.reshape(B * P, C).float().contiguous(), P, 0, P + 1, 1, B, P, dst_bf16=g16)
        else:
            g32 = torch.zeros(B * (P + 1), C, dtype=torch.float32, device=gout.device)
            ops.rows_copy(gout.reshape(B * P, C).float().contiguous(), P, 0, P + 1, 1, B, P, dst_f32=g32)
            g16 = ops.cast_bf16(g32)
        g32, g16 = _stack_bwd(g32, g16, self.enc.encoder, sh["layers"], saved["layers"], a, B, P + 1, None, False,
                              on_layer_done=self._part_grads_ready if self._part_ready_cb is not None else None,
                              final_f32=False)
        dg, accg = vec_grad(self.enc.pre_layrnorm.weight)
        db, _ = vec_grad(self.enc.pre_layrnorm.bias)
        dx0, _, _, _ = ops.layernorm_bwd(g32 if g32 is not None else g16, saved["x0"], self.enc.pre_layrnorm.weight, saved["m0"], saved["r0"],
                                         dgamma=dg, dbeta=db, accumulate=accg, want_bf16=False,
                                         need_param_grads=dg is not None)
        emb = self.enc.embeddings
        gpos, accp = grad_buf(emb.position_embedding.weight)
        gcls, accc = grad_buf(emb.class_embedding)
        if accp != accc:
            raise RuntimeError("lc2is_amd: inconsistent gradient state of the ViT embeddings")
        dpatch = ops.vit_embed_bwd(dx0, gpos, gcls, B, P, accumulate=accp)
        gw, accw = grad_buf(emb.patch_embedding.weight)
        k = 3 * self.patch_size ** 2
        if sh["kpad"] == k:
            ops.gemm_tn(dpatch, saved["cols"], gw.view(C, k), accumulate=accw)
        else:
            tmp = ops.gemm_tn(dpatch, saved["cols"])
            gw.view(C, k).copy_(tmp[:, :k]) if not accw else gw.view(C, k).add_(tmp[:, :k])
        self._grads_ready()

    def forward(self, pixel_values: torch.Tensor) -> torch.Tensor:
        anchor = self.enc.pre_layrnorm.weight
        return _VisionFn.apply(pixel_values, anchor, self, self.keep_cls, torch.is_grad_enabled() and anchor.requires_grad)


class ImageEncoderCLIPFull(ImageEncoderCLIP):

    keep_cls = True


class _TextFn(torch.autograd.Function):
    @staticmethod
    def forward(ctx, input_ids, attention_mask, anchor, mod, save):
        out, saved = mod._fwd(input_ids, attention_mask, save)
        ctx.mod, ctx.saved = mod, saved
        return out

    @staticmethod
    def backward(ctx, gout):
        here = torch.cuda.current_stream(gout.device)
        gout.record_stream(here)
        torch.autograd.Variable._execution_engine.queue_callback(
            lambda: torch.cuda.current_stream(gout.device).wait_stream(here))
        ctx.mod._bwd(gout.contiguous(), ctx.saved)
        ctx.saved = None
        return None, None, None, None, None


class TextEncoderCLIP(HipModule):

    def __init__(self, patch_size: int = 16, arch: ClipArch | None = None) -> None:
        super().__init__()
        self.patch_size = patch_size
        if arch is None:
            arch = TEXT_B if patch_size == 16 else TEXT_L
        self.arch = arch
        self.enc = _TextParams(arch)
        _clip_init(self.enc, arch)

    def hidden_size(self) -> int:
        return self.arch.hidden

    def _load_from_state_dict(self, state_dict, prefix, *args, **kwargs):
        _remap_legacy_keys(state_dict, prefix, "text_model")
        super()._load_from_state_dict(state_dict, prefix, *args, **kwargs)

    def _build_shadows(self, device):
        per, entries = _stack_shadows(self.enc.encoder, self.arch, device)
        return dict(layers=per), entries

    def _fwd(self, input_ids, attention_mask, save):
        require_cuda(input_ids, "input_ids")
        a, sh = self.arch, self._ensure_ready()
        B, L = input_ids.shape
        if L > a.max_pos:
            raise ValueError(f"Sequence length must be less than max_position_embeddings (got `sequence length`: "
                             f"{L} and max_position_embeddings: {a.max_pos}")
        emb = self.enc.embeddings
        ids = input_ids.contiguous()
        x = ops.text_embed_fwd(ids, emb.token_embedding.weight, emb.position_embedding.weight)
        if _RESID_BF16:
            x = ops.cast_bf16(x)
        kbias = None
        if attention_mask is not None:
            kbias = torch.zeros(B, L, dtype=torch.float32, device=ids.device)
            kbias.masked_fill_(attention_mask == 0, float("-inf"))
        x, saved = _stack_fwd(x, self.enc.encoder, sh["layers"], a, B, L, kbias, True, save)
        fl = self.enc.final_layer_norm
        _, y, mf, rf = ops.layernorm_fwd(x, fl.weight, fl.bias, a.eps, save_stats=save, out_bf16=None, out_f32=True)
        return y.view(B, L, a.hidden), (dict(ids=ids, kbias=kbias, xf=x, mf=mf, rf=rf, layers=saved, B=B, L=L)
                                        if save else None)

    def _bwd(self, gout, saved):
        a, sh = self.arch, self._sh
# ... 33 lines not shown
```

lc2is_amd/nn/model.py:

```python
from __future__ import annotations

from pathlib import Path

import torch
from torch import nn

from .. import ops
from .base import HipModule, grad_buf, linear_bwd_params, require_cuda, vec_grad
from .clip import ClipArch, ImageEncoderCLIP, TextEncoderCLIP, TextEncoderCLIPPooler
from .decoder import DecoderBlock, DecoderLayer
from .loss import check_dice, check_ohem

_DATA = Path(__file__).resolve().parent.parent / "data"
KPAD = 192


class _LinearFn(torch.autograd.Function):

    @staticmethod
    def forward(ctx, x, weight, bias, w16, w16T, save):
        lead = x.shape[:-1]
        x2 = x.reshape(-1, x.shape[-1]).float().contiguous()
        x16 = ops.cast_bf16(x2)
        _, y, _ = ops.gemm_nt(x16, w16, bias, out_bf16=None, out_f32=True)
        if save:
            ctx.x16, ctx.weight, ctx.bias, ctx.w16T, ctx.lead = x16, weight, bias, w16T, lead
        return y.view(*lead, weight.shape[0])

    @staticmethod
    def backward(ctx, gy):
        g2 = gy.reshape(-1, gy.shape[-1]).float().contiguous()
        g16 = ops.cast_bf16(g2)
        linear_bwd_params(g16, ctx.x16, ctx.weight, ctx.bias)
        _, dx, _ = ops.gemm_nt(g16, ctx.w16T, None, out_bf16=None, out_f32=True)
        return dx.view(*ctx.lead, dx.shape[-1]), None, None, None, None, None


class TextToPatch(HipModule):

    def __init__(self, img_in: int, text_in: int, out: int = 512) -> None:
        super().__init__()
        self.textual = nn.Linear(in_features=text_in, out_features=out)
        self.visual = nn.Linear(in_features=img_in, out_features=out)

    def _build_shadows(self, device):
        bf = dict(dtype=torch.bfloat16, device=device)
        t, v = self.textual.weight, self.visual.weight
        s = dict(wt=torch.empty(*t.shape, **bf), wtT=torch.empty(t.shape[1], t.shape[0], **bf),
                 wv=torch.empty(*v.shape, **bf), wvT=torch.empty(v.shape[1], v.shape[0], **bf))
        return s, [(t, s["wt"], s["wtT"]), (v, s["wv"], s["wvT"])]

    def forward(self, img: torch.Tensor, text: torch.Tensor):
        require_cuda(img, "img")
        sh = self._ensure_ready()
        save = torch.is_grad_enabled()
        t_feature = _LinearFn.apply(text, self.textual.weight, self.textual.bias, sh["wt"], sh["wtT"], save)
        v_feature = _LinearFn.apply(img, self.visual.weight, self.visual.bias, sh["wv"], sh["wvT"], save)
        return t_feature, v_feature


def fused_loss_options(weight, label_smoothing: float, reduction: str):
    if reduction not in ("mean", "sum", "none"):
        raise ValueError(f"{reduction} is not a valid value for reduction")
    if reduction == "none":
        raise NotImplementedError("lc2is_amd: the fused cross-entropy heads reduce to a scalar ('mean' or 'sum'); "
                                  "reduction='none' needs the materialised logits (forward + CrossEntropyLoss)")
    if not 0.0 <= label_smoothing <= 1.0:
        raise ValueError(f"label_smoothing must be between 0.0 and 1.0. Got: {label_smoothing}")
    if weight is None and label_smoothing == 0.0 and reduction == "mean":
        return None
    return weight, float(label_smoothing), reduction


def fused_dice_options(dice, opts, ohem):
    if dice is None:
        return None
    if opts is not None or ohem is not None:
        raise ValueError("lc2is_amd: dice= cannot be combined with weight=, label_smoothing, a reduction other than 'mean' "
                         "or ohem=")
    return check_dice(*dice)


def _reduce(loss2, reduction: str, save: bool):
    if reduction == "sum":
        return loss2[0], None
    inv = loss2[1].masked_fill(loss2[1] == 0, 1.0).reciprocal() if save else None
    return loss2[0] / loss2[1], inv


class _HeadFn(torch.autograd.Function):

    @staticmethod
    def forward(ctx, dec, protos, model, labels, save, ignore_index, loss_opts=None, ohem=None, dice=None):
        out, saved = model._head_fwd(dec, labels, save, ignore_index, loss_opts, ohem, dice)
        ctx.model, ctx.saved = model, saved
        return out

    @staticmethod
    def backward(ctx, gout):
        ddec = ctx.model._head_bwd(gout, ctx.saved)
        ctx.saved = None
        return ddec, None, None, None, None, None, None, None, None


class BaseModelWithText(HipModule):

    def __init__(self, patch_size: int = 16, in_size: int = 224, out_size: int = 224, dropout: float = 0,
                 num_layers: int = 1, *, prototypes: torch.Tensor | str | None = None,
                 vision_arch: ClipArch | None = None, text_arch: ClipArch | None = None, nhead: int = 8,
                 dim_feedforward: int = 2048, out_dim: int = 512) -> None:
        super().__init__()
        self.patch_size, self.in_size, self.out_size = patch_size, in_size, out_size
        if out_size != 4 * (in_size // patch_size):
            raise ValueError("BaseModelWithText: out_size must be 4 * (in_size // patch_size) "
                             "(model/model.py:41-44 upsamples the patch grid by 4)")
        self.vision_encoder = ImageEncoderCLIP(in_size=in_size, patch_size=patch_size, arch=vision_arch)
        self.text_encoder = TextEncoderCLIP(patch_size=patch_size, arch=text_arch)
        if prototypes is None:
            prototypes = _DATA / "ade20k_prototypes.pt"
        if not isinstance(prototypes, torch.Tensor):
            prototypes = torch.load(prototypes, weights_only=True)
        self.class_prototypes = nn.Parameter(prototypes.detach().clone().float(), requires_grad=True)
        cv, ct = self.vision_encoder.hidden_size(), self.text_encoder.hidden_size()
        layer = DecoderLayer(d_model=cv, d_kv=ct, nhead=nhead, dim_feedforward=dim_feedforward, dropout=dropout,
                             batch_first=True, norm_first=True)
        self.vision_decoder = DecoderBlock(decoder_layer=layer, num_layers=num_layers)
        self.pixel_patch = TextToPatch(out=out_dim, img_in=cv, text_in=self.class_prototypes.shape[1])
        if self.class_prototypes.shape[0] > KPAD:
            raise ValueError(f"BaseModelWithText: at most {KPAD} classes are supported by the fused head")
        self.overlap_text = True
        self._text_stream = None

    def _params_for_version(self):
        return [self.class_prototypes]

    def _build_shadows(self, device):
        K, Ct = self.class_prototypes.shape
        p16 = torch.zeros(KPAD, Ct, dtype=torch.bfloat16, device=device)
        return dict(p16=p16, K=K), [(self.class_prototypes, p16[:K], None)]

    def _head_scores(self, dec16):
        sh = self._ensure_ready()
        pp = self.pixel_patch
        psh = pp._ensure_ready()
        ft16, _, _ = ops.gemm_nt(sh["p16"], psh["wt"], pp.textual.bias)
        fv16, _, _ = ops.gemm_nt(dec16, psh["wv"], pp.visual.bias)
        _, scores, _ = ops.gemm_nt(fv16, ft16, None, out_bf16=None, out_f32=True)
        return ft16, fv16, scores

    def _head_fwd(self, dec, labels, save, ignore_index, loss_opts=None, ohem=None, dice=None):
        B, P, C = dec.shape
        g = self.in_size // self.patch_size
        K = self.class_prototypes.shape[0]
        dec16 = ops.cast_bf16(dec.reshape(B * P, C).float().contiguous())
        ft16, fv16, scores = self._head_scores(dec16)
        if labels is None:
            _, _, hi = ops.head_upsample_ce(scores, None, B, g, g, K, 4, ops.INTERP_BICUBIC, want_scores=True,
                                            want_loss=False)
            return hi, (dict(dec16=dec16, ft16=ft16, fv16=fv16, dims=(B, P, C, g, K), fused=None) if save else None)
        labels = labels.contiguous()
        if dice is not None:
            ce_weight, dice_weight, smooth, present_only = dice
            loss4, stats, dlo = ops.head_upsample_ce_dice(scores, labels, B, g, g, K, 4, ops.INTERP_BICUBIC, want_grad=save,
                                                          ignore_index=ignore_index, ce_weight=ce_weight, dice_weight=dice_weight,
                                                          smooth=smooth, present_only=present_only)
            self.last_dice = (stats[0], stats[1], stats[2], loss4)
            return loss4[0], (dict(dec16=dec16, ft16=ft16, fv16=fv16, dims=(B, P, C, g, K), fused=dlo, inv_count=None)
                              if save else None)
        if ohem is not None:
            labels, info = ops.ohem_labels(scores, labels, B, g, g, K, 4, ops.INTERP_BICUBIC, ignore_index, ohem)
            self.last_ohem = (labels, info)
        if loss_opts is None:
            loss2, dlo, _ = ops.head_upsample_ce(scores, labels.contiguous(), B, g, g, K, 4, ops.INTERP_BICUBIC,
                                                 want_grad=save, ignore_index=ignore_index, grad_scale=1.0)
            loss = loss2[0] / loss2[1]
            inv_count = (1.0 / loss2[1].clamp_min(1.0)) if save else None
        else:
            weight, label_smoothing, reduction = loss_opts
            loss2, dlo, _ = ops.head_upsample_ce(scores, labels.contiguous(), B, g, g, K, 4, ops.INTERP_BICUBIC,
                                                 want_grad=save, ignore_index=ignore_index, grad_scale=1.0,
                                                 class_weight=weight, label_smoothing=label_smoothing)
            loss, inv_count = _reduce(loss2, reduction, save)
        return loss, (dict(dec16=dec16, ft16=ft16, fv16=fv16, dims=(B, P, C, g, K), fused=dlo, inv_count=inv_count)
                      if save else None)

    def _head_bwd(self, gout, saved):
        B, P, C, g, K = saved["dims"]
        pp = self.pixel_patch
        psh, sh = pp._sh, self._sh
        if saved["fused"] is not None:
            ds = saved["fused"]
            inv = saved["inv_count"]
            if inv is None:
                ds16 = ops.cast_bf16(ds if gout is None else ds * gout)
            else:
                ds16 = ops.cast_bf16(ds * (inv if gout is None else gout * inv))
        else:
            ds = ops.upsample_bwd_nchw(gout.float().contiguous(), B, g, g, K, 4, ops.INTERP_BICUBIC, KPAD)
            ds16 = ops.cast_bf16(ds)
        ft16, fv16, dec16 = saved["ft16"], saved["fv16"], saved["dec16"]
        ftT = ops.transpose_bf16(ft16)
        dfv, _, _ = ops.gemm_nt(ds16, ftT, None)
        dft = ops.gemm_tn(ds16, fv16)
        linear_bwd_params(dfv, dec16, pp.visual.weight, pp.visual.bias)
        _, ddec, _ = ops.gemm_nt(dfv, psh["wvT"], None, out_bf16=None, out_f32=True)
        dft16 = ops.cast_bf16(dft)
        linear_bwd_params(dft16, sh["p16"], pp.textual.weight, pp.textual.bias)
        if self.class_prototypes.requires_grad:
            _, dp, _ = ops.gemm_nt(dft16, psh["wtT"], None, out_bf16=None, out_f32=True)
            gp, acc = grad_buf(self.class_prototypes)
            if acc:
                gp.add_(dp[:K])
            else:
                gp.copy_(dp[:K])
        pp._grads_ready()
        self._grads_ready()
        return ddec.view(B, P, C)

    def _decode(self, inputs):
        vision_inputs = {k: v for k, v in inputs.items() if k in ["pixel_values"]}
        text_inputs = {k: v for k, v in inputs.items() if k in ["input_ids", "attention_mask"]}
        if self.overlap_text and text_inputs["input_ids"].is_cuda:
            dev = text_inputs["input_ids"].device
            main = torch.cuda.current_stream(dev)
            if self._text_stream is None or self._text_stream.device != dev:
                prio = int(__import__("os").environ.get("LC2IS_TEXT_STREAM_PRIO", "-1"))
                self._text_stream = torch.cuda.Stream(dev, priority=prio)
            side = self._text_stream
            side.wait_stream(main)
            with torch.cuda.stream(side):
                for t in text_inputs.values():
                    t.record_stream(side)
                enc_t = self.text_encoder(**text_inputs)
            enc_v = self.vision_encoder(**vision_inputs)
            main.wait_stream(side)
            enc_t.record_stream(main)
        else:
            enc_t = self.text_encoder(**text_inputs)
            enc_v = self.vision_encoder(**vision_inputs)
        kpm = text_inputs["attention_mask"] != 1
        return self.vision_decoder(tgt=enc_v, memory=enc_t, memory_key_padding_mask=kpm)

    def forward(self, inputs: dict) -> dict:
        dec_v = self._decode(inputs)
        save = torch.is_grad_enabled() and dec_v.requires_grad
        logits = _HeadFn.apply(dec_v, self.class_prototypes, self, None, save, -100)
        return dict(outputs=logits)

    def forward_loss(self, inputs: dict, labels: torch.Tensor, ignore_index: int = -100, *, weight=None,
                     label_smoothing: float = 0.0, reduction: str = "mean", ohem=None, dice=None) -> torch.Tensor:
        opts = fused_loss_options(weight, label_smoothing, reduction)
        if ohem is not None:
            ohem = check_ohem(*ohem)
        dice = fused_dice_options(dice, opts, ohem)
        dec_v = self._decode(inputs)
        save = torch.is_grad_enabled() and dec_v.requires_grad
        return _HeadFn.apply(dec_v, self.class_prototypes, self, labels, save, ignore_index, opts, ohem, dice)

    @torch.no_grad()
    def forward_tuple(self, inputs: dict):
        dec_v = self._decode(inputs)
        B, P, C = dec_v.shape
        g = self.in_size // self.patch_size
        K = self.class_prototypes.shape[0]
        dec16 = ops.cast_bf16(dec_v.reshape(B * P, C).float().contiguous())
        ft16, fv16, scores = self._head_scores(dec16)
        _, _, logits = ops.head_upsample_ce(scores, None, B, g, g, K, 4, ops.INTERP_BICUBIC, want_scores=True,
                                            want_loss=False)
        fv = fv16.float()
        outs = []
        for c0 in range(0, fv.shape[1], KPAD):
            c1 = min(c0 + KPAD, fv.shape[1])
            ld = (c1 - c0 + 63) // 64 * 64
            chunk = torch.zeros(B * P, ld, dtype=torch.float32, device=fv.device)
            chunk[:, :c1 - c0] = fv[:, c0:c1]
            _, _, hi = ops.head_upsample_ce(chunk, None, B, g, g, c1 - c0, 4, ops.INTERP_BICUBIC, want_scores=True,
# ... 105 lines not shown
```

lc2is_amd/ops.py:

```python
from __future__ import annotations

import ctypes as C
import math
import os

import torch

from . import _lib

ACT_NONE, ACT_QUICK_GELU, ACT_RELU, ACT_DQUICK_GELU, ACT_DRELU, ACT_QUICK_GELU_GRAD, ACT_MUL_AUX = 0, 1, 2, 3, 4, 5, 6
ACT_GELU_ERF, ACT_DGELU_ERF, ACT_ADD_AUX = 7, 8, 9

_P, _I, _F, _Z, _L, _U64 = C.c_void_p, C.c_int, C.c_float, C.c_size_t, C.c_long, C.c_ulonglong
_ARGTYPES = {
    "lc2is_gemm_nt_bf16": [_P, _I, _P, _I, _P, _P, _I, _P, _I, _P, _I, _P, _I, _P, _I, _I, _I, _I, _I, _I, _P],
    "lc2is_gemm_nt_ln_xchg_bytes": [_I, _I],
    "lc2is_gemm_nt_ln_bf16": [_P, _I, _P, _I, _P, _P, _I, _P, _I, _P, _P, _F, _P, _I, _P, _P, _P, _Z, _I, _I, _I, _P],
    "lc2is_gemm_nt_bf16_batched": [_P, _I, _L, _P, _I, _L, _P, _I, _L, _P, _I, _L, _I, _I, _I, _I, _P],
    "lc2is_transpose_bf16_batched": [_P, _I, _L, _P, _I, _L, _I, _I, _I, _P],
    "lc2is_gemm_tn_workspace_bytes": [_I, _I, _I],
    "lc2is_gemm_tn_bf16": [_P, _I, _P, _I, _P, _I, _P, _I, _I, _I, _I, _P, _Z, _P],
    "lc2is_colsum_workspace_bytes": [_I, _I],
    "lc2is_colsum_bf16": [_P, _I, _P, _I, _I, _I, _P, _Z, _P],
    "lc2is_layernorm_fwd": [_P, _I, _I, _P, _P, _P, _I, _P, _I, _P, _P, _I, _I, _F, _P],
    "lc2is_layernorm_bwd_partials": [_I, _I],
    "lc2is_ln_partials_reduce": [_P, _I, _P],
    "lc2is_layernorm_bwd_workspace_bytes": [_I, _I],
    "lc2is_layernorm_bwd": [_P, _I, _P, _I, _P, _I, _I, _P, _P, _P, _P, _I, _I, _P, _I, _P, _I, _P, _P, _I, _I, _I,
                            _P, _Z, _P],
    "lc2is_attention_fwd": [_P, _I, _P, _I, _P, _I, _P, _I, _P, _P, _I, _I, _I, _I, _I, _F, _I, _P],
    "lc2is_attention_bwd": [_P, _I, _P, _I, _P, _I, _P, _I, _P, _I, _P, _I, _P, _I, _P, _I, _P, _P, _P,
                            _I, _I, _I, _I, _I, _F, _I, _P],
    "lc2is_attention_fwd_dropout": [_P, _I, _P, _I, _P, _I, _P, _I, _P, _P, _I, _I, _I, _I, _I, _F, _I, _F, _U64, _P],
    "lc2is_attention_bwd_dropout": [_P, _I, _P, _I, _P, _I, _P, _I, _P, _I, _P, _I, _P, _I, _P, _I, _P, _P, _P,
                                    _I, _I, _I, _I, _I, _F, _I, _F, _U64, _P],
    "lc2is_dropout_rows_f32": [_P, _I, _P, _I, _P, _I, _P, _I, _I, _I, _I, _F, _U64, _P],
    "lc2is_dropout_rows_bf16": [_P, _I, _P, _I, _I, _I, _F, _U64, _P],
    "lc2is_dropout_mask": [_P, _L, _I, _F, _U64, _P],
    "lc2is_shadow_refresh": [_P, _I, _I, _P],
    "lc2is_set_cu_budget": [_I],
    "lc2is_get_cu_budget": [],
    "lc2is_cast_f32_bf16": [_P, _I, _P, _I, _I, _I, _P],
    "lc2is_transpose_bf16": [_P, _I, _P, _I, _I, _I, _P],
    "lc2is_patchify": [_P, _P, _I, _I, _I, _I, _I, _P],
    "lc2is_vit_embed_fwd": [_P, _I, _P, _P, _P, _I, _I, _I, _I, _P],
    "lc2is_vit_embed_bwd": [_P, _I, _P, _P, _P, _I, _I, _I, _I, _I, _P],
    "lc2is_text_embed_fwd": [_P, _P, _P, _P, _I, _I, _I, _I, _I, _P],
    "lc2is_text_embed_bwd": [_P, _P, _I, _P, _P, _I, _I, _I, _I, _I, _P],
    "lc2is_rows_copy_bf16": [_P, _I, _I, _P, _P, _I, _I, _I, _I, _I, _P],
    "lc2is_rows_copy_f32": [_P, _I, _I, _P, _P, _I, _I, _I, _I, _I, _P],
    "lc2is_sgd_step": [_P, _P, _P, _Z, _F, _F, _F, _F, _P],
    "lc2is_adamw_step": [_P, _P, _P, _P, _Z, _F, _F, _F, _F, _F, _I, _F, _P],
    "lc2is_grad_sumsq_blocks": [_Z],
    "lc2is_grad_sumsq_workspace_bytes": [_Z],
    "lc2is_grad_sumsq": [_P, _Z, _P, _Z, _P],
    "lc2is_optim_ctrl_update": [_P, _P, _P, _I, _P, _I, _F, _F, _I, _F, _F, _P],
    "lc2is_sgd_step_ctrl": [_P, _P, _P, _Z, _P, _F, _F, _I, _P],
    "lc2is_adamw_step_ctrl": [_P, _P, _P, _P, _Z, _P, _F, _F, _F, _F, _I, _P],
    "lc2is_sgd_step_groups": [_P, _P, _P, _Z, _P, _P, _P, _I, _F, _I, _P],
    "lc2is_adamw_step_groups": [_P, _P, _P, _P, _Z, _P, _P, _P, _I, _F, _F, _F, _I, _P],
    "lc2is_ema_update_ctrl": [_P, _P, _Z, _P, _F, _I, _I, _I, _P],
    "lc2is_swap_f32": [_P, _P, _Z, _P],
    "lc2is_head_upsample_ce_workspace_bytes": [_I, _I, _I, _I, _I, _I, _I],
    "lc2is_head_upsample_ce": [_P, _I, _P, _P, _P, _P, _I, _I, _I, _I, _I, _I, C.c_long, _F, _P, _Z, _P],
    "lc2is_ce_nchw_fwd": [_P, _P, _P, _P, _I, _I, C.c_long, C.c_long, _P],
    "lc2is_ce_nchw_bwd": [_P, _P, _P, _P, _F, _P, _I, _I, C.c_long, C.c_long, _P],
    "lc2is_head_upsample_ce_opts": [_P, _I, _P, _P, _P, _P, _I, _I, _I, _I, _I, _I, C.c_long, _F, _P, _F, _P, _Z, _P],
    "lc2is_ce_nchw_fwd_opts": [_P, _P, _P, _P, _P, _I, _I, C.c_long, C.c_long, _P, _F, _P],
    "lc2is_ce_nchw_fwd_workspace_bytes": [_I, C.c_long],
    "lc2is_ce_nchw_fwd_ordered": [_P, _P, _P, _P, _P, _I, _I, C.c_long, C.c_long, _P, _F, _P, _Z, _P],
    "lc2is_ce_nchw_bwd_opts": [_P, _P, _P, _P, _F, _P, _P, _I, _I, C.c_long, C.c_long, _P, _F, _P],
    "lc2is_upsample_bwd_nchw": [_P, _P, _I, _I, _I, _I, _I, _I, _I, _P],
    "lc2is_head_upsample_px": [_P, _I, _P, _P, _I, _I, _I, _I, _I, _I, _L, _P],
    "lc2is_ohem_select_workspace_bytes": [_L],
    "lc2is_ohem_select": [_P, _P, _P, _L, _I, _L, _F, _L, _P, _P, _Z, _P],
    "lc2is_head_upsample_ce_dice_workspace_bytes": [_I, _I, _I, _I, _I, _I, _I],
    "lc2is_head_upsample_ce_dice": [_P, _I, _P, _P, _P, _P, _I, _I, _I, _I, _I, _I, _L, _F, _F, _F, _I, _F, _P, _Z, _P],
    "lc2is_ce_dice_nchw_workspace_bytes": [_I, _I, _L],
    "lc2is_ce_dice_nchw_fwd": [_P, _P, _P, _P, _P, _P, _I, _I, _L, _L, _F, _F, _F, _I, _P, _Z, _P],
    "lc2is_ce_dice_nchw_bwd": [_P, _P, _P, _P, _P, _F, _P, _I, _I, _L, _L, _P],
    "lc2is_bilinear_up_fwd": [_P, _P, _P, _I, _I, _I, _I, _I, _P],
    "lc2is_bilinear_up_bwd": [_P, _P, _P, _I, _I, _I, _I, _I, _I, _P],
    "lc2is_sr_gather": [_P, _P, _I, _I, _I, _I, _I, _P],
    "lc2is_sr_scatter_add_f32": [_P, _P, _I, _I, _I, _I, _P],
    "lc2is_l2norm_fwd": [_P, _P, _P, _P, _I, _I, _F, _P],
    "lc2is_l2norm_bwd": [_P, _P, _P, _P, _I, _I, _F, _P],
    "lc2is_add_n": [_P, _P, _P, _P, _P, _P, _Z, _P],
    "lc2is_rows_ce": [_P, _P, _P, _P, _P, _F, _I, _I, _I, _P],
    "lc2is_cols_ce": [_P, _P, _P, _P, _F, _I, _I, _I, _I, _P],
    "lc2is_npair": [_P, _P, _P, _P, _I, _I, _I, _I, _P],
    "lc2is_miou_counts": [_P, _P, _P, _I, _I, _I, _I, _I, _P],
    "lc2is_resize_argmax_workspace_bytes": [_L, _I],
    "lc2is_resize_argmax": [_P, _I, _I, _I, _I, _I, _P, _L, _L, _P, _I, _P, _P, _P, _Z, _P],
    "lc2is_npair_bwd": [_P, _P, _P, _P, _P, _P, _P, _P, _I, _I, _I, _I, _P],
    "lc2is_gemm_tn_grouped_workspace_bytes": [_P, _I],
    "lc2is_gemm_tn_grouped": [_P, _I, _P, _Z, _P],
    "lc2is_release_captured_tables": [],
    "lc2is_captured_tables_mark": [],
    "lc2is_release_captured_tables_range": [_I, _I],
    "lc2is_rows_gather": [_P, _I, _I, _P, _I, _I, _P, _P, _I, _I, _I, _P],
    "lc2is_resample_u8": [_P, _I, _I, _I, _P, _I, _I, _P, _P, _I, _P],
    "lc2is_gather2d_u8": [_P, _I, _I, _I, _P, _I, _I, _P, _P, _P],
    "lc2is_crop_lut": [_P, _I, _I, _I, _I, _I, _I, _P, _P, _P, _P, _P],
    "lc2is_aug_params": [_P, _P, _I, _P, _P, _L, _P, _P, _P],
    "lc2is_aug_apply": [_P, _Z, _P, _Z, _P, _L, _P, _P, _I, _I, _I, _P, _L, _P, _P, _P],
    "lc2is_swin_attn_fwd": [_P, _I, _P, _I, _P, _P, _I, _I, _I, _I, _I, _I, _I, _I, _I, _F, _P],
    "lc2is_swin_bias_table_grad": [_P, _P, _P, _P, _I, _I, _I, _I, _P],
    "lc2is_swin_attn_bwd_workspace_bytes": [_I, _I, _I],
    "lc2is_swin_attn_bwd": [_P, _I, _P, _I, _P, _I, _P, _P, _P, _I, _P, _I, _I, _I, _I, _I, _I, _I, _I, _I, _I, _F,
                            _P, _Z, _P],
}
_bound = {}


def _fn(name: str):
    f = _bound.get(name)
    if f is None:
        f = getattr(_lib.load(), name)
        if name in _ARGTYPES:
            f.argtypes = _ARGTYPES[name]
        if name.endswith("_workspace_bytes"):
            f.restype = C.c_size_t
        _bound[name] = f
    return f


def _stream() -> int:
    return torch.cuda.current_stream().cuda_stream


def _chk(t: torch.Tensor | None, dtype, name: str, ndim: int | None = 2):
    if t is None:
        return
# ... 358 lines not shown
        rc = _fn("lc2is_attention_bwd_dropout")(*args, float(dropout_p), int(seed), _stream())
    else:
        rc = _fn("lc2is_attention_bwd")(*args, _stream())
    _lib.check(rc, f"attention_bwd B={B} H={H} Sq={Sq} Sk={Sk} D={D}")
    return dq, dk, dv


def dropout_rows_f32(x: torch.Tensor, p: float, seed: int, *, resid: torch.Tensor | None = None,
                     out_f32: torch.Tensor | bool | None = True, out_bf16: torch.Tensor | bool | None = None,
                     rows_per_sample: int = 0):
    _chk(x, torch.float32, "x"); _chk(resid, torch.float32, "resid")
    M, Cc = x.shape
    yf = _out(out_f32, (M, Cc), torch.float32, x.device)
    yb = _out(out_bf16, (M, Cc), torch.bfloat16, x.device)
    _chk(yf, torch.float32, "out_f32"); _chk(yb, torch.bfloat16, "out_bf16")
    rc = _fn("lc2is_dropout_rows_f32")(_ptr(x), _ld(x), _ptr(resid), _ld(resid), _ptr(yf), _ld(yf), _ptr(yb), _ld(yb), M, Cc,
                                       int(rows_per_sample), float(p), int(seed), _stream())
    _lib.check(rc, f"dropout_rows_f32 M={M} C={Cc}")
    return yf, yb


def dropout_rows_bf16(x: torch.Tensor, p: float, seed: int, out: torch.Tensor | None = None):
    _chk(x, torch.bfloat16, "x")
    y = x if out is None else out
    _chk(y, torch.bfloat16, "out")
    M, Cc = x.shape
    rc = _fn("lc2is_dropout_rows_bf16")(_ptr(x), _ld(x), _ptr(y), _ld(y), M, Cc, float(p), int(seed), _stream())
    _lib.check(rc, f"dropout_rows_bf16 M={M} C={Cc}")
    return y


def dropout_mask(rows: int, cols: int, p: float, seed: int, device) -> torch.Tensor:
    out = torch.empty((rows, cols), dtype=torch.uint8, device=device)
    _lib.check(_fn("lc2is_dropout_mask")(_ptr(out), rows, cols, float(p), int(seed), _stream()), "dropout_mask")
    return out


INTERP_BICUBIC, INTERP_BILINEAR = 0, 1


class ShadowDesc(C.Structure):
    _fields_ = [("src", C.c_void_p), ("dst", C.c_void_p), ("dstT", C.c_void_p), ("N", C.c_int), ("K", C.c_int),
                ("ld_dst", C.c_int), ("ld_dstT", C.c_int), ("tile_start", C.c_int), ("flags", C.c_int)]


class ShadowTable:

    def __init__(self, entries, device):
        descs = (ShadowDesc * len(entries))()
        start = 0
        self._keep = []
        for i, (src, dst, dstT) in enumerate(entries):
            if src.dim() == 1:
                src = src.unsqueeze(0)
                dst = dst.unsqueeze(0) if dst is not None and dst.dim() == 1 else dst
            f32copy = dst is not None and dst.dtype == torch.float32
            _chk(src, torch.float32, "shadow src")
            _chk(dst, torch.float32 if f32copy else torch.bfloat16, "shadow dst")
            _chk(dstT, torch.bfloat16, "shadow dstT")
            if f32copy and dstT is not None:
                raise RuntimeError("lc2is_amd: fp32 shadow copies have no transposed twin")
            if not src.is_contiguous():
                raise RuntimeError("lc2is_amd: shadow source must be contiguous")
            N, K = src.shape
            if K % 4 or (dstT is not None and N % 4):
                raise RuntimeError(f"lc2is_amd: shadow shape [{N},{K}] not supported")
            if dst is not None and tuple(dst.shape) != (N, K):
                raise RuntimeError("lc2is_amd: shadow dst shape mismatch")
            if dstT is not None and tuple(dstT.shape) != (K, N):
                raise RuntimeError("lc2is_amd: shadow dstT shape mismatch")
            descs[i] = ShadowDesc(src.data_ptr(), _ptr(dst), _ptr(dstT), N, K, _ld(dst), _ld(dstT), start, int(f32copy))
            start += ((N + 63) // 64) * ((K + 63) // 64)
            self._keep.append((src, dst, dstT))
        self.n = len(entries)
        self.total_tiles = start
        raw = bytes(descs)
        self.dev = torch.frombuffer(bytearray(raw), dtype=torch.uint8).to(device)

    def refresh(self):
        rc = _fn("lc2is_shadow_refresh")(self.dev.data_ptr(), self.n, self.total_tiles, _stream())
        _lib.check(rc, "shadow_refresh")


def cast_bf16(src: torch.Tensor, out: torch.Tensor | None = None):
    _chk(src, torch.float32, "src")
    M, Cc = src.shape
    out = out if out is not None else torch.empty((M, Cc), dtype=torch.bfloat16, device=src.device)
    _chk(out, torch.bfloat16, "out")
    _lib.check(_fn("lc2is_cast_f32_bf16")(_ptr(src), _ld(src), _ptr(out), _ld(out), M, Cc, _stream()), "cast")
    return out


def transpose_bf16(src: torch.Tensor, out: torch.Tensor | None = None):
    _chk(src, torch.bfloat16, "src")
    R, Cc = src.shape
    out = out if out is not None else torch.empty((Cc, R), dtype=torch.bfloat16, device=src.device)
    _chk(out, torch.bfloat16, "out")
    _lib.check(_fn("lc2is_transpose_bf16")(_ptr(src), _ld(src), _ptr(out), _ld(out), R, Cc, _stream()),
               "transpose")
    return out


def patchify(pixels: torch.Tensor, patch: int, kpad: int | None = None):
    _chk(pixels, torch.float32, "pixel_values", 4)
    if not pixels.is_contiguous() or pixels.shape[1] != 3:
        raise RuntimeError("lc2is_amd.patchify: pixel_values must be contiguous [B,3,H,W]")
    B, _, H, W = pixels.shape
    G = H // patch
    k = 3 * patch * patch
    kpad = kpad or ((k + 63) // 64) * 64
    out = torch.empty((B * G * G, kpad), dtype=torch.bfloat16, device=pixels.device)
    _lib.check(_fn("lc2is_patchify")(_ptr(pixels), _ptr(out), kpad, B, H, W, patch, _stream()), "patchify")
    return out


def vit_embed_fwd(patch_f32, cls, pos, B: int, P: int):
    _chk(patch_f32, torch.float32, "patch"); _chk(cls, torch.float32, "cls", 1); _chk(pos, torch.float32, "pos")
    Cc = patch_f32.shape[1]
    x = torch.empty((B * (P + 1), Cc), dtype=torch.float32, device=patch_f32.device)
    _lib.check(_fn("lc2is_vit_embed_fwd")(_ptr(patch_f32), _ld(patch_f32), _ptr(cls), _ptr(pos), _ptr(x), Cc, B,
                                          P, Cc, _stream()), "vit_embed_fwd")
    return x


def vit_embed_bwd(dx, dpos, dcls, B: int, P: int, accumulate: bool = False):
    _chk(dx, torch.float32, "dx"); _chk(dpos, torch.float32, "dpos"); _chk(dcls, torch.float32, "dcls", 1)
    Cc = dx.shape[1]
    dpatch = torch.empty((B * P, Cc), dtype=torch.bfloat16, device=dx.device)
    _lib.check(_fn("lc2is_vit_embed_bwd")(_ptr(dx), _ld(dx), _ptr(dpos), _ptr(dcls), _ptr(dpatch), Cc, B, P, Cc,
                                          int(accumulate), _stream()), "vit_embed_bwd")
    return dpatch


def text_embed_fwd(ids, tok, pos):
    _chk(ids, torch.int64, "input_ids"); _chk(tok, torch.float32, "tok"); _chk(pos, torch.float32, "pos")
    if not ids.is_contiguous():
        raise RuntimeError("lc2is_amd.text_embed_fwd: input_ids must be contiguous")
    B, L = ids.shape
    V, Cc = tok.shape
    x = torch.empty((B * L, Cc), dtype=torch.float32, device=tok.device)
    _lib.check(_fn("lc2is_text_embed_fwd")(_ptr(ids), _ptr(tok), _ptr(pos), _ptr(x), Cc, B, L, Cc, V, _stream()),
               "text_embed_fwd")
    return x


def text_embed_bwd(ids, dx, dtok, dpos, accumulate: bool = False):
    _chk(ids, torch.int64, "input_ids"); _chk(dx, torch.float32, "dx")
    B, L = ids.shape
    V, Cc = dtok.shape
    _lib.check(_fn("lc2is_text_embed_bwd")(_ptr(ids), _ptr(dx), _ld(dx), _ptr(dtok), _ptr(dpos), B, L, Cc, V,
                                           int(accumulate), _stream()), "text_embed_bwd")


def rows_copy(src, S_src: int, src_off: int, S_dst: int, dst_off: int, B: int, n: int, *, dst_f32=None,
              dst_bf16=None):
    sb = src.dtype == torch.bfloat16
    _chk(src, torch.bfloat16 if sb else torch.float32, "src")
    Cc = src.shape[1]
    if not src.is_contiguous() or src.shape[0] != B * S_src:
        raise RuntimeError("lc2is_amd.rows_copy: src must be contiguous [B*S_src, C]")
    for t in (dst_f32, dst_bf16):
        if t is not None and (not t.is_contiguous() or tuple(t.shape) != (B * S_dst, Cc)):
            raise RuntimeError("lc2is_amd.rows_copy: dst must be contiguous [B*S_dst, C]")
    _lib.check(_fn("lc2is_rows_copy_bf16" if sb else "lc2is_rows_copy_f32")(_ptr(src), S_src, src_off, _ptr(dst_f32), _ptr(dst_bf16),
                                                                            S_dst, dst_off, B, n, Cc, _stream()), "rows_copy")


def sgd_step(params, grads, momentum_buf, lr, momentum=0.0, weight_decay=0.0, grad_scale=1.0):
    _chk(params, torch.float32, "params", 1); _chk(grads, torch.float32, "grads", 1)
    _lib.check(_fn("lc2is_sgd_step")(_ptr(params), _ptr(grads), _ptr(momentum_buf), params.numel(), lr, momentum,
                                     weight_decay, grad_scale, _stream()), "sgd_step")


def adamw_step(params, grads, m, v, lr, beta1, beta2, eps, weight_decay, step, grad_scale=1.0):
    _chk(params, torch.float32, "params", 1); _chk(grads, torch.float32, "grads", 1)
    _lib.check(_fn("lc2is_adamw_step")(_ptr(params), _ptr(grads), _ptr(m), _ptr(v), params.numel(), lr, beta1,
                                       beta2, eps, weight_decay, int(step), grad_scale, _stream()), "adamw_step")


OPTIM_CTRL_WORDS = 12
(CTRL_CALLS, CTRL_APPLIED, CTRL_SKIPPED, CTRL_FINITE, CTRL_GRAD_NORM, CTRL_CLIP_COEF, CTRL_LR, CTRL_BC1, CTRL_BC2, CTRL_GRAD_MUL,
 CTRL_APPLY) = range(11)


def _chk_ctrl(ctrl):
    _chk(ctrl, torch.int32, "ctrl", 1)
    if ctrl.numel() != OPTIM_CTRL_WORDS:
        raise RuntimeError(f"lc2is_amd: ctrl must be an int32 [{OPTIM_CTRL_WORDS}] control block (lc2is_optim_ctrl)")


def _chk_same_numel(name, params, *others):
    for t in others:
        if t is not None:
            _chk(t, torch.float32, name + " buffer", 1)
            if t.numel() != params.numel():
                raise RuntimeError(f"lc2is_amd.{name}: every buffer must have params' {params.numel()} elements, got {t.numel()}")


def grad_sumsq(grads):
    _chk(grads, torch.float32, "grads", 1)
    n = grads.numel()
    nb = _fn("lc2is_grad_sumsq_blocks")(n)
    if nb <= 0:
        raise RuntimeError(f"lc2is_amd.grad_sumsq: numel must be a positive multiple of 4, got {n}")
    need = _fn("lc2is_grad_sumsq_workspace_bytes")(n)
    ws = workspace(need, grads.device, "grad_sumsq")
    _lib.check(_fn("lc2is_grad_sumsq")(_ptr(grads), n, _ptr(ws), ws.numel(), _stream()), "grad_sumsq")
    return ws[:4 * nb].view(torch.float32), ws[4 * nb:8 * nb].view(torch.int32)


def optim_ctrl_update(ctrl, partials, flags, lr_table, *, grad_scale=1.0, max_norm=float("inf"), skip_nonfinite=False,
                      beta1=0.0, beta2=0.0):
    _chk_ctrl(ctrl); _chk(partials, torch.float32, "partials", 1); _chk(flags, torch.int32, "flags", 1)
    _chk(lr_table, torch.float32, "lr_table", 1)
    if flags.numel() != partials.numel() or not partials.is_contiguous() or not flags.is_contiguous():
        raise RuntimeError("lc2is_amd.optim_ctrl_update: partials and flags must be contiguous and of one length")
    if lr_table.numel() < 1 or not lr_table.is_contiguous():
        raise RuntimeError("lc2is_amd.optim_ctrl_update: lr_table must be a non-empty contiguous fp32 tensor")
    _lib.check(_fn("lc2is_optim_ctrl_update")(_ptr(ctrl), _ptr(partials), _ptr(flags), partials.numel(), _ptr(lr_table),
                                              lr_table.numel(), grad_scale, max_norm, int(bool(skip_nonfinite)), beta1, beta2,
                                              _stream()), "optim_ctrl_update")


def sgd_step_ctrl(params, grads, momentum_buf, ctrl, momentum=0.0, weight_decay=0.0, reverse=False):
    _chk(params, torch.float32, "params", 1); _chk_same_numel("sgd_step_ctrl", params, grads, momentum_buf); _chk_ctrl(ctrl)
    _lib.check(_fn("lc2is_sgd_step_ctrl")(_ptr(params), _ptr(grads), _ptr(momentum_buf), params.numel(), _ptr(ctrl), momentum,
                                          weight_decay, int(bool(reverse)), _stream()), "sgd_step_ctrl")


def adamw_step_ctrl(params, grads, m, v, ctrl, beta1, beta2, eps, weight_decay, reverse=False):
    _chk(params, torch.float32, "params", 1); _chk_same_numel("adamw_step_ctrl", params, grads, m, v); _chk_ctrl(ctrl)
    _lib.check(_fn("lc2is_adamw_step_ctrl")(_ptr(params), _ptr(grads), _ptr(m), _ptr(v), params.numel(), _ptr(ctrl), beta1,
                                            beta2, eps, weight_decay, int(bool(reverse)), _stream()), "adamw_step_ctrl")


GROUP_GRANULE, MAX_PARAM_GROUPS, GROUP_SKIP = 64, 255, 255


def _chk_groups(name, params, granule_group, groups):
    _chk(granule_group, torch.uint8, "granule_group", 1); _chk(groups, torch.float32, "groups", 2)
    if granule_group is None or groups is None:
        raise RuntimeError(f"lc2is_amd.{name}: granule_group and groups are required")
    n = params.numel()
    if n == 0 or n % GROUP_GRANULE:
        raise RuntimeError(f"lc2is_amd.{name}: numel must be a positive multiple of {GROUP_GRANULE}, got {n}")
    if not params.is_contiguous() or not granule_group.is_contiguous() or granule_group.numel() != n // GROUP_GRANULE:
        raise RuntimeError(f"lc2is_amd.{name}: granule_group must be a contiguous uint8 [{n // GROUP_GRANULE}] map (one id per "
                           f"{GROUP_GRANULE} elements), got {tuple(granule_group.shape)}")
    if not groups.is_contiguous() or groups.shape[1] != 2 or not 1 <= groups.shape[0] <= MAX_PARAM_GROUPS:
        raise RuntimeError(f"lc2is_amd.{name}: groups must be a contiguous fp32 [ngroups, 2] table of (lr_scale, weight_decay), "
                           f"1 <= ngroups <= {MAX_PARAM_GROUPS}, got {tuple(groups.shape)}")


def sgd_step_groups(params, grads, momentum_buf, ctrl, granule_group, groups, momentum=0.0, reverse=False):
    _chk(params, torch.float32, "params", 1); _chk_same_numel("sgd_step_groups", params, grads, momentum_buf); _chk_ctrl(ctrl)
    _chk_groups("sgd_step_groups", params, granule_group, groups)
    _lib.check(_fn("lc2is_sgd_step_groups")(_ptr(params), _ptr(grads), _ptr(momentum_buf), params.numel(), _ptr(ctrl),
                                            _ptr(granule_group), _ptr(groups), groups.shape[0], momentum, int(bool(reverse)),
                                            _stream()), "sgd_step_groups")


def adamw_step_groups(params, grads, m, v, ctrl, granule_group, groups, beta1, beta2, eps, reverse=False):
    _chk(params, torch.float32, "params", 1); _chk_same_numel("adamw_step_groups", params, grads, m, v); _chk_ctrl(ctrl)
    _chk_groups("adamw_step_groups", params, granule_group, groups)
    _lib.check(_fn("lc2is_adamw_step_groups")(_ptr(params), _ptr(grads), _ptr(m), _ptr(v), params.numel(), _ptr(ctrl),
                                              _ptr(granule_group), _ptr(groups), groups.shape[0], beta1, beta2, eps,
                                              int(bool(reverse)), _stream()), "adamw_step_groups")


def ema_update_ctrl(ema, params, ctrl, one_minus_decay, warmup=False, every=1, reverse=False):
    _chk(ema, torch.float32, "ema", 1); _chk_same_numel("ema_update_ctrl", ema, params); _chk_ctrl(ctrl)
    if params is None:
        raise RuntimeError("lc2is_amd.ema_update_ctrl: params is required")
    _lib.check(_fn("lc2is_ema_update_ctrl")(_ptr(ema), _ptr(params), ema.numel(), _ptr(ctrl), float(one_minus_decay),
                                            int(bool(warmup)), int(every), int(bool(reverse)), _stream()), "ema_update_ctrl")


def swap_f32(a, b):
    _chk(a, torch.float32, "a", 1); _chk_same_numel("swap_f32", a, b)
    if b is None:
        raise RuntimeError("lc2is_amd.swap_f32: b is required")
    _lib.check(_fn("lc2is_swap_f32")(_ptr(a), _ptr(b), a.numel(), _stream()), "swap_f32")


def _ce_options(class_weight, label_smoothing: float, C: int, dev):
    if not 0.0 <= label_smoothing <= 1.0:
        raise RuntimeError(f"label_smoothing must be between 0.0 and 1.0. Got: {label_smoothing}")
    if class_weight is None:
        return label_smoothing != 0.0
    if class_weight.dim() != 1 or class_weight.numel() != C:
        raise RuntimeError(f"weight tensor should be defined either for all {C} classes or no classes but got weight "
                           f"tensor of shape: {list(class_weight.shape)}")
    _chk(class_weight, torch.float32, "class_weight", 1)
    if class_weight.device != dev:
        raise RuntimeError(f"lc2is_amd: class_weight must be on {dev}, got {class_weight.device}")
    return True


def head_upsample_ce(scores_lo, labels, B: int, h: int, w: int, C: int, S: int, mode: int = INTERP_BICUBIC, *,
                     want_grad: bool = False, want_scores: bool = False, want_loss: bool = True,
                     ignore_index: int = -100, grad_scale: float = 1.0, class_weight=None, label_smoothing: float = 0.0):
    _chk(scores_lo, torch.float32, "scores_lo"); _chk(labels, torch.int64, "labels", 3)
    opts = _ce_options(class_weight, label_smoothing, C, scores_lo.device) and want_loss
    if not scores_lo.is_contiguous():
        raise RuntimeError("lc2is_amd.head_upsample_ce: scores_lo must be contiguous")
    ld = scores_lo.shape[1]
    dev = scores_lo.device
    if labels is not None and (tuple(labels.shape) != (B, h * S, w * S) or not labels.is_contiguous()):
        raise RuntimeError(f"lc2is_amd.head_upsample_ce: labels must be contiguous [{B},{h*S},{w*S}]")
    nbytes = _fn("lc2is_head_upsample_ce_workspace_bytes")(B, h, w, C, S, mode, int(want_grad)) if want_loss else 0
    alloc = torch.empty if nbytes else torch.zeros
    loss = alloc(2, dtype=torch.float32, device=dev) if want_loss else None
    dlo = alloc(scores_lo.shape, dtype=torch.float32, device=dev) if want_grad else None
    hi = torch.empty((B, C, h * S, w * S), dtype=torch.float32, device=dev) if want_scores else None
    ws = torch.empty(nbytes, dtype=torch.uint8, device=dev) if nbytes else None
    if opts:
        rc = _fn("lc2is_head_upsample_ce_opts")(_ptr(scores_lo), ld, _ptr(labels), _ptr(dlo), _ptr(hi), _ptr(loss), B, h,
                                                w, C, S, mode, ignore_index, grad_scale, _ptr(class_weight),
                                                label_smoothing, _ptr(ws), nbytes, _stream())
    else:
        rc = _fn("lc2is_head_upsample_ce")(_ptr(scores_lo), ld, _ptr(labels), _ptr(dlo), _ptr(hi), _ptr(loss), B, h,
                                           w, C, S, mode, ignore_index, grad_scale, _ptr(ws), nbytes, _stream())
    _lib.check(rc, f"head_upsample_ce B={B} h={h} w={w} C={C} S={S}")
    return loss, dlo, hi


def head_upsample_px(scores_lo, labels, B: int, h: int, w: int, C: int, S: int, mode: int = INTERP_BICUBIC, *,
                     ignore_index: int = -100):
    _chk(scores_lo, torch.float32, "scores_lo"); _chk(labels, torch.int64, "labels", 3)
    if not scores_lo.is_contiguous():
        raise RuntimeError("lc2is_amd.head_upsample_px: scores_lo must be contiguous")
    if labels is None or tuple(labels.shape) != (B, h * S, w * S) or not labels.is_contiguous():
        raise RuntimeError(f"lc2is_amd.head_upsample_px: labels must be contiguous [{B},{h*S},{w*S}]")
    lpx = torch.empty((B, h * S, w * S), dtype=torch.float32, device=scores_lo.device)
    _lib.check(_fn("lc2is_head_upsample_px")(_ptr(scores_lo), scores_lo.shape[1], _ptr(labels), _ptr(lpx), B, h, w, C, S, mode,
                                             ignore_index, _stream()), f"head_upsample_px B={B} h={h} w={w} C={C} S={S}")
    return lpx


OHEM_INFO_WORDS = 3


def ohem_loss_thresh(thresh: float) -> float:
    if not 0.0 < thresh <= 1.0:
        raise ValueError(f"OHEM thresh must be in (0, 1], got {thresh}")
    return float(torch.tensor(-math.log(thresh), dtype=torch.float64).to(torch.float32))


def ohem_select(loss_px, labels, C: int, thresh: float, min_kept_total: int, ignore_index: int = -100):
    _chk(loss_px, torch.float32, "loss_px", None); _chk(labels, torch.int64, "labels", None)
    if loss_px is None or labels is None or loss_px.shape != labels.shape or not loss_px.is_contiguous() or not labels.is_contiguous():
        raise RuntimeError("lc2is_amd.ohem_select: loss_px (fp32) and labels (int64) must be contiguous and of one shape")
    if int(min_kept_total) < 0:
        raise ValueError(f"OHEM min_kept must be >= 0, got {min_kept_total}")
    tau = ohem_loss_thresh(thresh)
    n = loss_px.numel()
    need = _fn("lc2is_ohem_select_workspace_bytes")(n)
    if need == 0:
        raise RuntimeError(f"lc2is_amd.ohem_select: 1 <= numel < 2^31 required, got {n}")
    dev = loss_px.device
    ws = workspace(need, dev, "ohem_select")
    out = torch.empty_like(labels)
    info = torch.empty(OHEM_INFO_WORDS, dtype=torch.int64, device=dev)
    _lib.check(_fn("lc2is_ohem_select")(_ptr(loss_px), _ptr(labels), _ptr(out), n, C, ignore_index, tau, int(min_kept_total),
                                        _ptr(info), _ptr(ws), ws.numel(), _stream()), f"ohem_select n={n}")
    return out, info


def ohem_info_fields(info) -> dict:
    host = info.detach().cpu()
    L, L_eff = host[2:3].view(torch.float32).tolist()
    return dict(n_valid=int(host[0]), k=int(host[1]), L=L, L_eff=L_eff)


def ohem_labels(scores_lo, labels, B: int, h: int, w: int, C: int, S: int, mode: int, ignore_index: int, ohem):
    thresh, min_kept = ohem
    lpx = head_upsample_px(scores_lo, labels, B, h, w, C, S, mode, ignore_index=ignore_index)
    return ohem_select(lpx, labels, C, thresh, int(min_kept) * B, ignore_index)


DICE_CMAX = 192


def dice_options(ce_weight, dice_weight, smooth, present_only) -> tuple[float, float, float, bool]:
    for name, v in (("ce_weight", ce_weight), ("dice_weight", dice_weight), ("smooth", smooth)):
        if isinstance(v, bool) or not isinstance(v, (int, float)) or not math.isfinite(v) or v < 0:
            raise ValueError(f"Dice + CE: {name} must be a finite number >= 0, got {v!r}")
    if float(ce_weight) == 0.0 and float(dice_weight) == 0.0:
        raise ValueError("Dice + CE: ce_weight and dice_weight must not both be 0")
    if not isinstance(present_only, bool):
        raise ValueError(f"Dice + CE: present_only must be a bool, got {present_only!r}")
    return float(ce_weight), float(dice_weight), float(smooth), present_only


def head_upsample_ce_dice(scores_lo, labels, B: int, h: int, w: int, C: int, S: int, mode: int = INTERP_BICUBIC, *,
                          want_grad: bool = False, ignore_index: int = -100, ce_weight: float = 1.0, dice_weight: float = 1.0,
                          smooth: float = 1.0, present_only: bool = True, grad_scale: float = 1.0):
    _chk(scores_lo, torch.float32, "scores_lo"); _chk(labels, torch.int64, "labels", 3)
    ce_weight, dice_weight, smooth, present_only = dice_options(ce_weight, dice_weight, smooth, present_only)
# ... 519 lines not shown
```

Baseline: 1078 images/s.

## Fuse ViT embedding with double LayerNorm and fold loss mean into head

```diff
diff --git a/include/lc2is_hip.h b/include/lc2is_hip.h
--- a/include/lc2is_hip.h
+++ b/include/lc2is_hip.h
@@ -135,6 +135,14 @@
                         int ldx, int B, int P, int C, lc2is_stream_t stream);
 int lc2is_vit_embed_bwd(const float* dx, int ldx, float* dpos, float* dcls, void* dpatch_bf16, int ld_dpatch,
                         int B, int P, int C, int accumulate, lc2is_stream_t stream);
+int lc2is_vit_embed_ln2_fwd(const float* patch, int ld_patch, const float* cls, const float* pos, const float* gamma_a,
+                            const float* beta_a, const float* gamma_b, const float* beta_b, float* x0, float* xf, void* h_bf16,
+                            float* mean_a, float* rstd_a, float* mean_b, float* rstd_b, int B, int P, int C, float eps,
+                            lc2is_stream_t stream);
+int lc2is_vit_embed_ln_bwd(const void* dy_bf16, const float* x0, const float* gamma, const float* mean, const float* rstd,
+                           void* dpatch_bf16, int ld_dpatch, float* dpos, float* dcls, float* dgamma, float* dbeta,
+                           int accumulate_ln, int accumulate_emb, int B, int P, int C, void* workspace, size_t workspace_bytes,
+                           lc2is_stream_t stream);
 int lc2is_text_embed_fwd(const int64_t* ids, const float* tok, const float* pos, float* x, int ldx, int B,
                          int L, int C, int vocab, lc2is_stream_t stream);
 int lc2is_text_embed_bwd(const int64_t* ids, const float* dx, int ldx, float* dtok, float* dpos, int B, int L,
@@ -143,6 +151,10 @@
                         int dst_off, int B, int n, int C, lc2is_stream_t stream);
 int lc2is_rows_copy_bf16(const void* src, int S_src, int src_off, float* dst_f32, void* dst_bf16, int S_dst,
                          int dst_off, int B, int n, int C, lc2is_stream_t stream);
+int lc2is_rows_copy_zfill(const void* src, int src_is_bf16, int S_src, int src_off, float* dst_f32, void* dst_bf16, int S_dst,
+                          int dst_off, int B, int n, int C, lc2is_stream_t stream);
+int lc2is_scale_cast_bf16(const float* src, int ld_src, const float* scalar_a, const float* scalar_b, void* dst_bf16,
+                          int ld_dst, int M, int C, lc2is_stream_t stream);
 
 int lc2is_sgd_step(float* params, const float* grads, float* momentum_buf, size_t n, float lr, float momentum,
                    float weight_decay, float grad_scale, lc2is_stream_t stream);
@@ -158,6 +170,9 @@
 int lc2is_head_upsample_ce_opts(const float* scores_lo, int ld, const int64_t* labels, float* dscores_lo,
                                 float* scores_hi, float* loss_sum, int B, int h, int w, int C, int S, int mode,
                                 long ignore_index, float grad_scale, const float* class_weight, float label_smoothing,
+                                void* workspace, size_t workspace_bytes, lc2is_stream_t stream);
+int lc2is_head_upsample_ce_mean(const float* scores_lo, int ld, const int64_t* labels, float* dscores_lo, float* loss_out,
+                                int B, int h, int w, int C, int S, int mode, long ignore_index, float grad_scale,
                                 void* workspace, size_t workspace_bytes, lc2is_stream_t stream);
 int lc2is_upsample_bwd_nchw(const float* dhi, float* dlo, int ld, int B, int h, int w, int C, int S, int mode,
                             lc2is_stream_t stream);
diff --git a/lc2is_amd/csrc/head.hip b/lc2is_amd/csrc/head.hip
--- a/lc2is_amd/csrc/head.hip
+++ b/lc2is_amd/csrc/head.hip
@@ -24,6 +24,7 @@
   int cq;
   const float* cw;
   float eps;
+  float* loss_mean;
 };
 
 __device__ __forceinline__ void lds_add(float* p, float v) {
@@ -1011,7 +1012,10 @@
     for (int k = lane; k < nblk_main; k += 64) { l += p.ws_loss[2 * (size_t)k]; c += p.ws_loss[2 * (size_t)k + 1]; }
     l = wave_sum(l);
     c = wave_sum(c);
-    if (lane == 0) { p.loss_sum[0] = l; p.loss_sum[1] = c; }
+    if (lane == 0) {
+      p.loss_sum[0] = l; p.loss_sum[1] = c;
+      if (p.loss_mean) { p.loss_mean[0] = l / c; p.loss_mean[1] = 1.f / fmaxf(c, 1.f); }
+    }
   }
   if (!p.dlo) return;
   const long ncell = (long)p.B * p.h * p.w;
@@ -1335,7 +1339,7 @@
 
 namespace {
 int head_upsample_ce(const float* scores_lo, int ld, const int64_t* labels, float* dscores_lo, float* scores_hi,
-                     float* loss_sum, int B, int h, int w, int C, int S, int mode, long ignore_index, float grad_scale,
+                     float* loss_sum, float* loss_mean, int B, int h, int w, int C, int S, int mode, long ignore_index, float grad_scale,
                      const float* class_weight, float label_smoothing, void* workspace, size_t workspace_bytes,
                      lc2is_stream_t stream_) {
   hipStream_t stream = (hipStream_t)stream_;
@@ -1351,7 +1355,8 @@
   if (opt && !(S == 4 || S == 8 || S == 16)) return LC2IS_ERR_UNSUPPORTED;
   const int H = h * S, W = w * S;
   HeadArgs a{scores_lo, ld, labels, dscores_lo, scores_hi, loss_sum, B, h, w, H, W, C, S, mode, ignore_index,
-             grad_scale, nullptr, nullptr, 0, class_weight, label_smoothing};
+             grad_scale, nullptr, nullptr, 0, class_weight, label_smoothing, loss_mean};
+  if (loss_mean && (!loss_sum || !(S == 4 || S == 8 || S == 16))) return LC2IS_ERR_UNSUPPORTED;
   const int lds_bytes = 2 * FMAX * FMAX * ld * (int)sizeof(float);
   static DevOnce attr_set;
   if (attr_set.need()) {
@@ -1484,7 +1489,15 @@
                                       float* scores_hi, float* loss_sum, int B, int h, int w, int C, int S,
                                       int mode, long ignore_index, float grad_scale, void* workspace,
                                       size_t workspace_bytes, lc2is_stream_t stream) {
-  return head_upsample_ce(scores_lo, ld, labels, dscores_lo, scores_hi, loss_sum, B, h, w, C, S, mode, ignore_index,
+  return head_upsample_ce(scores_lo, ld, labels, dscores_lo, scores_hi, loss_sum, nullptr, B, h, w, C, S, mode, ignore_index,
+                          grad_scale, nullptr, 0.f, workspace, workspace_bytes, stream);
+}
+
+extern "C" int lc2is_head_upsample_ce_mean(const float* scores_lo, int ld, const int64_t* labels, float* dscores_lo,
+                                           float* loss_out, int B, int h, int w, int C, int S, int mode, long ignore_index,
+                                           float grad_scale, void* workspace, size_t workspace_bytes, lc2is_stream_t stream) {
+  if (!loss_out) return LC2IS_ERR_NULL;
+  return head_upsample_ce(scores_lo, ld, labels, dscores_lo, nullptr, loss_out, loss_out + 2, B, h, w, C, S, mode, ignore_index,
                           grad_scale, nullptr, 0.f, workspace, workspace_bytes, stream);
 }
 
@@ -1493,7 +1506,7 @@
                                            int mode, long ignore_index, float grad_scale, const float* class_weight,
                                            float label_smoothing, void* workspace, size_t workspace_bytes,
                                            lc2is_stream_t stream) {
-  return head_upsample_ce(scores_lo, ld, labels, dscores_lo, scores_hi, loss_sum, B, h, w, C, S, mode, ignore_index,
+  return head_upsample_ce(scores_lo, ld, labels, dscores_lo, scores_hi, loss_sum, nullptr, B, h, w, C, S, mode, ignore_index,
                           grad_scale, class_weight, label_smoothing, workspace, workspace_bytes, stream);
 }
 
diff --git a/lc2is_amd/csrc/layernorm.hip b/lc2is_amd/csrc/layernorm.hip
--- a/lc2is_amd/csrc/layernorm.hip
+++ b/lc2is_amd/csrc/layernorm.hip
@@ -13,6 +13,37 @@
   const uint2 pk = *reinterpret_cast<const uint2*>(p);
   return make_float4(bf16_to_f32((bf16_t)(pk.x & 0xffff)), bf16_to_f32((bf16_t)(pk.x >> 16)),
                      bf16_to_f32((bf16_t)(pk.y & 0xffff)), bf16_to_f32((bf16_t)(pk.y >> 16)));
+}
+
+template <int NV>
+__device__ __forceinline__ void ln_row_stats(const float4 (&v)[NV], int lane, int C4, int C, float eps, float& mean, float& rstd) {
+  float s = 0.f;
+#pragma unroll
+  for (int i = 0; i < NV; ++i) {
+    const int c4 = lane + 64 * i;
+    if (c4 < C4) s += (v[i].x + v[i].y) + (v[i].z + v[i].w);
+  }
+  mean = wave_sum(s) / (float)C;
+  float q = 0.f;
+#pragma unroll
+  for (int i = 0; i < NV; ++i) {
+    const int c4 = lane + 64 * i;
+    if (c4 < C4) {
+      const float a = v[i].x - mean, b = v[i].y - mean, c = v[i].z - mean, d = v[i].w - mean;
+      q += (a * a + b * b) + (c * c + d * d);
+    }
+  }
+  rstd = rsqrtf(wave_sum(q) / (float)C + eps);
+}
+
+__device__ __forceinline__ float4 ln_row_apply(const float4 v, float mean, float rstd, const float4 g, const float4 b, bool has_beta) {
+  float4 o;
+  o.x = (v.x - mean) * rstd * g.x;
+  o.y = (v.y - mean) * rstd * g.y;
+  o.z = (v.z - mean) * rstd * g.z;
+  o.w = (v.w - mean) * rstd * g.w;
+  if (has_beta) { o.x += b.x; o.y += b.y; o.z += b.z; o.w += b.w; }
+  return o;
 }
 
 template <int NV>
@@ -54,23 +85,8 @@
   for (; row < M; row += stride) {
     const bool more = row + stride < M;
     if (more) load_row(row + stride, nx);
-    float s = 0.f;
-#pragma unroll
-    for (int i = 0; i < NV; ++i) {
-      const int c4 = lane + 64 * i;
-      if (c4 < C4) s += (v[i].x + v[i].y) + (v[i].z + v[i].w);
-    }
-    const float mean = wave_sum(s) / (float)C;
-    float q = 0.f;
-#pragma unroll
-    for (int i = 0; i < NV; ++i) {
-      const int c4 = lane + 64 * i;
-      if (c4 < C4) {
-        const float a = v[i].x - mean, b = v[i].y - mean, c = v[i].z - mean, d = v[i].w - mean;
-        q += (a * a + b * b) + (c * c + d * d);
-      }
-    }
-    const float rstd = rsqrtf(wave_sum(q) / (float)C + eps);
+    float mean, rstd;
+    ln_row_stats<NV>(v, lane, C4, C, eps, mean, rstd);
     if (lane == 0) {
       if (mean_out) mean_out[row] = mean;
       if (rstd_out) rstd_out[row] = rstd;
@@ -79,12 +95,7 @@
     for (int i = 0; i < NV; ++i) {
       const int c4 = lane + 64 * i;
       if (c4 < C4) {
-        float4 o;
-        o.x = (v[i].x - mean) * rstd * gm[i].x;
-        o.y = (v[i].y - mean) * rstd * gm[i].y;
-        o.z = (v[i].z - mean) * rstd * gm[i].z;
-        o.w = (v[i].w - mean) * rstd * gm[i].w;
-        if (beta) { o.x += bt[i].x; o.y += bt[i].y; o.z += bt[i].z; o.w += bt[i].w; }
+        const float4 o = ln_row_apply(v[i], mean, rstd, gm[i], bt[i], beta != nullptr);
         if (y) {
           uint2 pk = make_uint2(pack_bf16x2(o.x, o.y), pack_bf16x2(o.z, o.w));
           *reinterpret_cast<uint2*>(y + (size_t)row * ldy + 4 * c4) = pk;
@@ -95,6 +106,87 @@
     if (more) {
 #pragma unroll
       for (int i = 0; i < NV; ++i) v[i] = nx[i];
+    }
+  }
+}
+
+template <int NV>
+__global__ __launch_bounds__(256, (NV <= 2 ? 4 : NV == 3 ? 3 : NV == 4 ? 2 : 1)) void vit_embed_ln2_fwd_kernel(const float* __restrict__ patch, int ldp, const float* __restrict__ cls,
+                                                                 const float* __restrict__ pos,
+                                                                 const float* __restrict__ gamma_a, const float* __restrict__ beta_a,
+                                                                 const float* __restrict__ gamma_b, const float* __restrict__ beta_b,
+                                                                 float* x0, float* xf, bf16_t* h, float* mean_a, float* rstd_a,
+                                                                 float* mean_b, float* rstd_b, int B, int P, int C, float eps) {
+  const int lane = threadIdx.x & 63;
+  const int C4 = C >> 2;
+  const int M = B * (P + 1);
+  float4 ga[NV], ba[NV], gb[NV], bb[NV];
+#pragma unroll
+  for (int i = 0; i < NV; ++i) {
+    const int c4 = lane + 64 * i;
+    ga[i] = (c4 < C4) ? reinterpret_cast<const float4*>(gamma_a)[c4] : make_float4(0.f, 0.f, 0.f, 0.f);
+    ba[i] = (beta_a && c4 < C4) ? reinterpret_cast<const float4*>(beta_a)[c4] : make_float4(0.f, 0.f, 0.f, 0.f);
+    gb[i] = (c4 < C4) ? reinterpret_cast<const float4*>(gamma_b)[c4] : make_float4(0.f, 0.f, 0.f, 0.f);
+    bb[i] = (beta_b && c4 < C4) ? reinterpret_cast<const float4*>(beta_b)[c4] : make_float4(0.f, 0.f, 0.f, 0.f);
+  }
+  const int stride = gridDim.x * 4;
+  int row = blockIdx.x * 4 + (threadIdx.x >> 6);
+  if (row >= M) return;
+  auto load_row = [&](int r, float4 (&e)[NV], float4 (&pe)[NV]) __attribute__((always_inline)) {
+    const int t = r % (P + 1), b = r / (P + 1);
+    const float4* er = (t == 0) ? reinterpret_cast<const float4*>(cls)
+                                : reinterpret_cast<const float4*>(patch + ((size_t)b * P + t - 1) * ldp);
+    const float4* pr = reinterpret_cast<const float4*>(pos + (size_t)t * C);
+#pragma unroll
+    for (int i = 0; i < NV; ++i) {
+      const int c4 = lane + 64 * i;
+      e[i] = (c4 < C4) ? er[c4] : make_float4(0.f, 0.f, 0.f, 0.f);
+      pe[i] = (c4 < C4) ? pr[c4] : make_float4(0.f, 0.f, 0.f, 0.f);
+    }
+  };
+  float4 v[NV], pv[NV], ne[NV], np[NV];
+  load_row(row, v, pv);
+  for (; row < M; row += stride) {
+    const bool more = row + stride < M;
+    if (more) load_row(row + stride, ne, np);
+#pragma unroll
+    for (int i = 0; i < NV; ++i) {
+      const int c4 = lane + 64 * i;
+      v[i].x += pv[i].x; v[i].y += pv[i].y; v[i].z += pv[i].z; v[i].w += pv[i].w;
+      if (x0 && c4 < C4) *reinterpret_cast<float4*>(x0 + (size_t)row * C + 4 * c4) = v[i];
+    }
+    float mean, rstd;
+    ln_row_stats<NV>(v, lane, C4, C, eps, mean, rstd);
+    if (lane == 0) {
+      if (mean_a) mean_a[row] = mean;
+      if (rstd_a) rstd_a[row] = rstd;
+    }
+    float4 o[NV];
+#pragma unroll
+    for (int i = 0; i < NV; ++i) {
+      const int c4 = lane + 64 * i;
+      o[i] = make_float4(0.f, 0.f, 0.f, 0.f);
+      if (c4 < C4) {
+        o[i] = ln_row_apply(v[i], mean, rstd, ga[i], ba[i], beta_a != nullptr);
+        if (xf) *reinterpret_cast<float4*>(xf + (size_t)row * C + 4 * c4) = o[i];
+      }
+    }
+    ln_row_stats<NV>(o, lane, C4, C, eps, mean, rstd);
+    if (lane == 0) {
+      if (mean_b) mean_b[row] = mean;
+      if (rstd_b) rstd_b[row] = rstd;
+    }
+#pragma unroll
+    for (int i = 0; i < NV; ++i) {
+      const int c4 = lane + 64 * i;
+      if (c4 < C4) {
+        const float4 t = ln_row_apply(o[i], mean, rstd, gb[i], bb[i], beta_b != nullptr);
+        *reinterpret_cast<uint2*>(h + (size_t)row * C + 4 * c4) = make_uint2(pack_bf16x2(t.x, t.y), pack_bf16x2(t.z, t.w));
+      }
+    }
+    if (more) {
+#pragma unroll
+      for (int i = 0; i < NV; ++i) { v[i] = ne[i]; pv[i] = np[i]; }
     }
   }
 }
@@ -291,6 +383,141 @@
       const float t = (r[c] + r[2048 + c]) + (r[4096 + c] + r[6144 + c]);
       ws[((size_t)blockIdx.x * 2 + pass) * C + c] = t;
     }
+  }
+}
+
+template <int NV>
+__global__ __launch_bounds__(256) void vit_embed_ln_bwd_kernel(const bf16_t* __restrict__ dyb, const float* __restrict__ x,
+                                                                const float* __restrict__ gamma, const float* __restrict__ mean,
+                                                                const float* __restrict__ rstd, bf16_t* dpatch, int ldp, float* dpos,
+                                                                float* dcls, float* ws, int nparts, int B, int P, int C, int accumulate) {
+  __shared__ float red[4 * 2048];
+  const int lane = threadIdx.x & 63, wave = threadIdx.x >> 6;
+  const int C4 = C >> 2;
+  const int ntok = P + 1;
+  const int M = B * ntok;
+  float4 gm[NV];
+#pragma unroll
+  for (int i = 0; i < NV; ++i) {
+    const int c4 = lane + 64 * i;
+    gm[i] = (c4 < C4) ? reinterpret_cast<const float4*>(gamma)[c4] : make_float4(0.f, 0.f, 0.f, 0.f);
+  }
+  if ((int)blockIdx.x >= ntok) {
+    const int pb = blockIdx.x - ntok;
+    float4 dg[NV], db[NV];
+#pragma unroll
+    for (int i = 0; i < NV; ++i) { dg[i] = make_float4(0.f, 0.f, 0.f, 0.f); db[i] = make_float4(0.f, 0.f, 0.f, 0.f); }
+    for (int row = pb * 4 + wave; row < M; row += nparts * 4) {
+      const float mu = mean[row], rs = rstd[row];
+#pragma unroll
+      for (int i = 0; i < NV; ++i) {
+        const int c4 = lane + 64 * i;
+        if (c4 < C4) {
+          const float4 xv = *reinterpret_cast<const float4*>(x + (size_t)row * C + 4 * c4);
+          const float4 dy = load_bf16x4(dyb + (size_t)row * C + 4 * c4);
+          const float4 xh = make_float4((xv.x - mu) * rs, (xv.y - mu) * rs, (xv.z - mu) * rs, (xv.w - mu) * rs);
+          dg[i].x += dy.x * xh.x; dg[i].y += dy.y * xh.y;
+          dg[i].z += dy.z * xh.z; dg[i].w += dy.w * xh.w;
+          db[i].x += dy.x; db[i].y += dy.y; db[i].z += dy.z; db[i].w += dy.w;
+        }
+      }
+    }
+    float* r = red;
+#pragma unroll
+    for (int pass = 0; pass < 2; ++pass) {
+      __syncthreads();
+#pragma unroll
+      for (int i = 0; i < NV; ++i) {
+        const int c4 = lane + 64 * i;
+        if (c4 < C4) *reinterpret_cast<float4*>(r + wave * 2048 + 4 * c4) = pass ? db[i] : dg[i];
+      }
+      __syncthreads();
+      for (int c = threadIdx.x; c < C; c += 256) {
+        const float t = (r[c] + r[2048 + c]) + (r[4096 + c] + r[6144 + c]);
+        ws[((size_t)pb * 2 + pass) * C + c] = t;
+      }
+    }
+    return;
+  }
+  const int t = blockIdx.x;
+  struct Raw { uint2 dy[NV]; float4 xv[NV]; float mu, rs; };
+  auto load_row = [&](int b, Raw& r) __attribute__((always_inline)) {
+    const size_t row = (size_t)b * ntok + t;
+    r.mu = mean[row]; r.rs = rstd[row];
+#pragma unroll
+    for (int i = 0; i < NV; ++i) {
+      const int c4 = lane + 64 * i;
+      const bool ok = c4 < C4;
+      r.dy[i] = ok ? *reinterpret_cast<const uint2*>(dyb + row * C + 4 * c4) : make_uint2(0u, 0u);
+      r.xv[i] = ok ? *reinterpret_cast<const float4*>(x + row * C + 4 * c4) : make_float4(0.f, 0.f, 0.f, 0.f);
+    }
+  };
+  auto widen = [](uint2 pk) {
+    return make_float4(bf16_to_f32((bf16_t)(pk.x & 0xffff)), bf16_to_f32((bf16_t)(pk.x >> 16)),
+                       bf16_to_f32((bf16_t)(pk.y & 0xffff)), bf16_to_f32((bf16_t)(pk.y >> 16)));
+  };
+  float4 acc = make_float4(0.f, 0.f, 0.f, 0.f);
+  Raw cur, nxt;
+  if (wave < B) load_row(wave, cur);
+  for (int b0 = 0; b0 < B; b0 += 4) {
+    const int b = b0 + wave;
+    if (b + 4 < B) load_row(b + 4, nxt);
+    if (b < B) {
+      const float mu = cur.mu, rs = cur.rs;
+      float4 xh[NV], dy[NV];
+      float s1 = 0.f, s2 = 0.f;
+#pragma unroll
+      for (int i = 0; i < NV; ++i) {
+        const int c4 = lane + 64 * i;
+        if (c4 < C4) {
+          const float4 xv = cur.xv[i];
+          dy[i] = widen(cur.dy[i]);
+          xh[i] = make_float4((xv.x - mu) * rs, (xv.y - mu) * rs, (xv.z - mu) * rs, (xv.w - mu) * rs);
+          const float a = dy[i].x * gm[i].x, b_ = dy[i].y * gm[i].y, c = dy[i].z * gm[i].z, d = dy[i].w * gm[i].w;
+          s1 += (a + b_) + (c + d);
+          s2 += (a * xh[i].x + b_ * xh[i].y) + (c * xh[i].z + d * xh[i].w);
+        }
+      }
+      const float c1 = wave_sum(s1) / (float)C, c2 = wave_sum(s2) / (float)C;
+      const float4 rv = make_float4(0.f, 0.f, 0.f, 0.f);
+#pragma unroll
+      for (int i = 0; i < NV; ++i) {
+        const int c4 = lane + 64 * i;
+        if (c4 < C4) {
+          float4 o;
+          o.x = rs * (dy[i].x * gm[i].x - c1 - xh[i].x * c2);
+          o.y = rs * (dy[i].y * gm[i].y - c1 - xh[i].y * c2);
+          o.z = rs * (dy[i].z * gm[i].z - c1 - xh[i].z * c2);
+          o.w = rs * (dy[i].w * gm[i].w - c1 - xh[i].w * c2);
+          o.x += rv.x; o.y += rv.y; o.z += rv.z; o.w += rv.w;
+          if (t > 0 && dpatch)
+            *reinterpret_cast<uint2*>(dpatch + ((size_t)b * P + t - 1) * ldp + 4 * c4) =
+                make_uint2(pack_bf16x2(o.x, o.y), pack_bf16x2(o.z, o.w));
+          *reinterpret_cast<float4*>(red + wave * 2048 + 4 * c4) = o;
+        }
+      }
+    }
+    __syncthreads();
+    if ((int)threadIdx.x < C4) {
+      const int nb = (B - b0) < 4 ? (B - b0) : 4;
+      for (int w = 0; w < nb; ++w) {
+        const float4 v = *reinterpret_cast<const float4*>(red + w * 2048 + 4 * threadIdx.x);
+        acc.x += v.x; acc.y += v.y; acc.z += v.z; acc.w += v.w;
+      }
+    }
+    __syncthreads();
+    if (b + 4 < B) cur = nxt;
+  }
+  if ((int)threadIdx.x < C4) {
+    if (t == 0) {
+      float4 cacc = acc;
+      float4* dc = reinterpret_cast<float4*>(dcls) + threadIdx.x;
+      if (accumulate) { const float4 o = *dc; cacc.x += o.x; cacc.y += o.y; cacc.z += o.z; cacc.w += o.w; }
+      *dc = cacc;
+    }
+    float4* dp = reinterpret_cast<float4*>(dpos + (size_t)t * C) + threadIdx.x;
+    if (accumulate) { const float4 o = *dp; acc.x += o.x; acc.y += o.y; acc.z += o.z; acc.w += o.w; }
+    *dp = acc;
   }
 }
 
@@ -409,6 +636,55 @@
   return rc;
 }
 
+extern "C" int lc2is_vit_embed_ln2_fwd(const float* patch, int ld_patch, const float* cls, const float* pos,
+                                       const float* gamma_a, const float* beta_a, const float* gamma_b, const float* beta_b,
+                                       float* x0, float* xf, void* h_bf16, float* mean_a, float* rstd_a, float* mean_b,
+                                       float* rstd_b, int B, int P, int C, float eps, lc2is_stream_t stream_) {
+  hipStream_t stream = (hipStream_t)stream_;
+  if (!patch || !cls || !pos || !gamma_a || !gamma_b || !h_bf16) return LC2IS_ERR_NULL;
+  if (B <= 0 || P <= 0 || C <= 0 || C % 4 || C > LN_MAXV * 256 || ld_patch < C || ld_patch % 4) return LC2IS_ERR_SHAPE;
+  if ((long)B * (P + 1) > 0x7fffffffL) return LC2IS_ERR_SHAPE;
+  const int M = B * (P + 1);
+#define EMB_FWD(NV_)                                                                                                        \
+  hipLaunchKernelGGL(vit_embed_ln2_fwd_kernel<NV_>, dim3(grid), dim3(256), 0, stream, patch, ld_patch, cls, pos, \
+                     gamma_a, beta_a, gamma_b, beta_b, x0, xf, (bf16_t*)h_bf16, mean_a, rstd_a, mean_b, rstd_b, B, P, C, eps)
+  const int nv = (C / 4 + 63) / 64;
+  const int cap = 256 * (nv <= 2 ? 4 : nv == 3 ? 3 : nv == 4 ? 2 : 1);
+  const int grid = (M + 3) / 4 < cap ? (M + 3) / 4 : cap;
+  if (nv <= 1) EMB_FWD(1); else if (nv == 2) EMB_FWD(2); else if (nv == 3) EMB_FWD(3);
+  else if (nv == 4) EMB_FWD(4); else if (nv <= 6) EMB_FWD(6); else EMB_FWD(8);
+#undef EMB_FWD
+  return lc2is_check_launch();
+}
+
+extern "C" int lc2is_vit_embed_ln_bwd(const void* dy_bf16, const float* x0, const float* gamma, const float* mean,
+                                      const float* rstd, void* dpatch_bf16, int ld_dpatch, float* dpos, float* dcls,
+                                      float* dgamma, float* dbeta, int accumulate_ln, int accumulate_emb, int B, int P, int C,
+                                      void* workspace, size_t workspace_bytes, lc2is_stream_t stream_) {
+  hipStream_t stream = (hipStream_t)stream_;
+  if (!dy_bf16 || !x0 || !gamma || !mean || !rstd || !dpos || !dcls) return LC2IS_ERR_NULL;
+  if (B <= 0 || P <= 0 || C <= 0 || C % 4 || (dpatch_bf16 && (ld_dpatch < C || ld_dpatch % 4))) return LC2IS_ERR_SHAPE;
+  if (C > 1024) return LC2IS_ERR_UNSUPPORTED;
+  if ((long)B * (P + 1) > 0x7fffffffL) return LC2IS_ERR_SHAPE;
+  const int M = B * (P + 1);
+  if (!workspace || workspace_bytes < lc2is_layernorm_bwd_workspace_bytes(M, C)) return LC2IS_ERR_WORKSPACE;
+  const int nparts = ln_bwd_blocks(M, C);
+#define EMB_BWD(NV_)                                                                                                          \
+  hipLaunchKernelGGL(vit_embed_ln_bwd_kernel<NV_>, dim3(P + 1 + nparts), dim3(256), 0, stream, (const bf16_t*)dy_bf16, x0, gamma, \
+                     mean, rstd, (bf16_t*)dpatch_bf16, ld_dpatch, dpos, dcls, (float*)workspace, nparts, B, P, C, accumulate_emb)
+  const int nv = (C / 4 + 63) / 64;
+  if (nv <= 1) EMB_BWD(1); else if (nv == 2) EMB_BWD(2); else if (nv == 3) EMB_BWD(3); else EMB_BWD(4);
+#undef EMB_BWD
+  int rc = lc2is_check_launch();
+  if (rc) return rc;
+  if (dgamma || dbeta) {
+    hipLaunchKernelGGL(partials_reduce_kernel, dim3((C + 31) / 32, 2), dim3(1024), 0, stream,
+                       (const float*)workspace, nparts, (size_t)2 * C, (size_t)C, C, dgamma, dbeta, accumulate_ln);
+    rc = lc2is_check_launch();
+  }
+  return rc;
+}
+
 extern "C" int lc2is_layernorm_bwd_partials(int M, int C) {
   if (M <= 0 || C <= 0 || C % 4 || C > LN_MAXV * 256) return 0;
   return ln_bwd_blocks(M, C);
diff --git a/lc2is_amd/csrc/misc.hip b/lc2is_amd/csrc/misc.hip
--- a/lc2is_amd/csrc/misc.hip
+++ b/lc2is_amd/csrc/misc.hip
@@ -247,6 +247,49 @@
   }
 }
 
+template <typename SrcT>
+__global__ __launch_bounds__(256) void rows_copy_zfill_kernel(const SrcT* __restrict__ src, int S_src, int src_off,
+                                                               float* dst, bf16_t* dst_b, int S_dst, int dst_off,
+                                                               int B, int n, int C) {
+  const int C4 = C >> 2;
+  const size_t total = (size_t)B * S_dst * C4;
+  for (size_t i = (size_t)blockIdx.x * 256 + threadIdx.x; i < total; i += (size_t)gridDim.x * 256) {
+    const int c4 = (int)(i % C4);
+    const size_t r = i / C4;
+    const int sd = (int)(r % S_dst), b = (int)(r / S_dst);
+    const int s = sd - dst_off;
+    const size_t o = r * C + 4 * c4;
+    float4 v = make_float4(0.f, 0.f, 0.f, 0.f);
+    uint2 pk = make_uint2(0u, 0u);
+    if (s >= 0 && s < n) {
+      const size_t si = ((size_t)b * S_src + src_off + s) * C + 4 * c4;
+      if constexpr (sizeof(SrcT) == 2) {
+        pk = *reinterpret_cast<const uint2*>(src + si);
+        v = make_float4(bf16_to_f32((bf16_t)(pk.x & 0xffff)), bf16_to_f32((bf16_t)(pk.x >> 16)),
+                        bf16_to_f32((bf16_t)(pk.y & 0xffff)), bf16_to_f32((bf16_t)(pk.y >> 16)));
+      } else {
+        v = *reinterpret_cast<const float4*>(src + si);
+        pk = make_uint2(pack_bf16x2(v.x, v.y), pack_bf16x2(v.z, v.w));
+      }
+    }
+    if (dst) *reinterpret_cast<float4*>(dst + o) = v;
+    if (dst_b) *reinterpret_cast<uint2*>(dst_b + o) = pk;
+  }
+}
+
+__global__ __launch_bounds__(256) void scale_cast_bf16_kernel(const float* __restrict__ src, int lds_, const float* __restrict__ a,
+                                                               const float* __restrict__ b, bf16_t* dst, int ldd, int M, int C) {
+  const float sc = b ? a[0] * b[0] : a[0];
+  const int C4 = C >> 2;
+  const size_t total = (size_t)M * C4;
+  for (size_t i = (size_t)blockIdx.x * 256 + threadIdx.x; i < total; i += (size_t)gridDim.x * 256) {
+    const int m = (int)(i / C4), c4 = (int)(i % C4);
+    const float4 v = *reinterpret_cast<const float4*>(src + (size_t)m * lds_ + 4 * c4);
+    *reinterpret_cast<uint2*>(dst + (size_t)m * ldd + 4 * c4) =
+        make_uint2(pack_bf16x2(v.x * sc, v.y * sc), pack_bf16x2(v.z * sc, v.w * sc));
+  }
+}
+
 __global__ __launch_bounds__(256) void sgd_kernel(float* p, const float* __restrict__ g, float* mom, size_t n4,
                                                    float lr, float momentum, float wd, float gscale) {
   for (size_t i = (size_t)blockIdx.x * 256 + threadIdx.x; i < n4; i += (size_t)gridDim.x * 256) {
@@ -426,6 +469,33 @@
   return lc2is_check_launch();
 }
 
+extern "C" int lc2is_rows_copy_zfill(const void* src, int src_is_bf16, int S_src, int src_off, float* dst_f32, void* dst_bf16,
+                                     int S_dst, int dst_off, int B, int n, int C, lc2is_stream_t stream_) {
+  hipStream_t stream = (hipStream_t)stream_;
+  if (!src || (!dst_f32 && !dst_bf16)) return LC2IS_ERR_NULL;
+  if (B <= 0 || n <= 0 || C <= 0 || C % 4 || src_off < 0 || dst_off < 0 || src_off + n > S_src ||
+      dst_off + n > S_dst)
+    return LC2IS_ERR_SHAPE;
+  const int grid = ew_grid((size_t)B * S_dst * C / 4);
+  if (src_is_bf16)
+    hipLaunchKernelGGL(rows_copy_zfill_kernel<bf16_t>, dim3(grid), dim3(256), 0, stream, (const bf16_t*)src, S_src, src_off,
+                       dst_f32, (bf16_t*)dst_bf16, S_dst, dst_off, B, n, C);
+  else
+    hipLaunchKernelGGL(rows_copy_zfill_kernel<float>, dim3(grid), dim3(256), 0, stream, (const float*)src, S_src, src_off,
+                       dst_f32, (bf16_t*)dst_bf16, S_dst, dst_off, B, n, C);
+  return lc2is_check_launch();
+}
+
+extern "C" int lc2is_scale_cast_bf16(const float* src, int ld_src, const float* scalar_a, const float* scalar_b, void* dst,
+                                     int ld_dst, int M, int C, lc2is_stream_t stream_) {
+  hipStream_t stream = (hipStream_t)stream_;
+  if (!src || !dst || !scalar_a) return LC2IS_ERR_NULL;
+  if (M <= 0 || C <= 0 || C % 4 || ld_src < C || ld_dst < C || ld_src % 4 || ld_dst % 4) return LC2IS_ERR_SHAPE;
+  hipLaunchKernelGGL(scale_cast_bf16_kernel, dim3(ew_grid((size_t)M * C / 4)), dim3(256), 0, stream, src, ld_src, scalar_a,
+                     scalar_b, (bf16_t*)dst, ld_dst, M, C);
+  return lc2is_check_launch();
+}
+
 extern "C" int lc2is_sgd_step(float* params, const float* grads, float* momentum_buf, size_t n, float lr,
                               float momentum, float weight_decay, float grad_scale, lc2is_stream_t stream_) {
   hipStream_t stream = (hipStream_t)stream_;
diff --git a/lc2is_amd/nn/clip.py b/lc2is_amd/nn/clip.py
--- a/lc2is_amd/nn/clip.py
+++ b/lc2is_amd/nn/clip.py
@@ -136,14 +136,14 @@
 _RESID_BF16 = __import__('os').environ.get("LC2IS_RESID_STREAM", "f32") == "bf16"
 
 
-def _stack_fwd(x, stack: _Stack, sh, a: ClipArch, B: int, S: int, kbias, causal: bool, save: bool):
+def _stack_fwd(x, stack: _Stack, sh, a: ClipArch, B: int, S: int, kbias, causal: bool, save: bool, ln0=None):
     C, H = a.hidden, a.heads
     D = C // H
     scale = D ** -0.5
     saved = []
     lean = x.dtype == torch.bfloat16
     fuse = (not lean) and ops.gemm_nt_ln_ok(x.shape[0], C, C) and ops.gemm_nt_ln_ok(x.shape[0], C, a.intermediate)
-    nxt_ln = None
+    nxt_ln = ln0
     layers = list(stack.layers)
     for li, (layer, s) in enumerate(zip(layers, sh)):
         if nxt_ln is not None:
@@ -338,11 +338,18 @@
         emb = self.enc.embeddings
         cols = ops.patchify(pixel_values.float().contiguous(), self.patch_size, sh["kpad"])
         _, pe, _ = ops.gemm_nt(cols, sh["wpatch"], None, out_bf16=None, out_f32=True)
-        x0 = ops.vit_embed_fwd(pe, emb.class_embedding, emb.position_embedding.weight, B, P)
-        xb, xf, m0, r0 = ops.layernorm_fwd(x0, self.enc.pre_layrnorm.weight, self.enc.pre_layrnorm.bias, a.eps,
-                                           save_stats=save, out_bf16=True if _RESID_BF16 else None,
-                                           out_f32=None if _RESID_BF16 else True)
-        x, saved = _stack_fwd(xb if _RESID_BF16 else xf, self.enc.encoder, sh["layers"], a, B, P + 1, None, False, save)
+        pre, ln0 = self.enc.pre_layrnorm, None
+        if ops.edge_fuse() and not _RESID_BF16:
+            l1 = self.enc.encoder.layers[0].layer_norm1
+            x0, xf, h, m0, r0, m1, r1 = ops.vit_embed_ln2_fwd(pe, emb.class_embedding, emb.position_embedding.weight, pre.weight,
+                                                              pre.bias, l1.weight, l1.bias, B, P, a.eps, save=save)
+            xb, ln0 = None, (h, m1, r1)
+        else:
+            x0 = ops.vit_embed_fwd(pe, emb.class_embedding, emb.position_embedding.weight, B, P)
+            xb, xf, m0, r0 = ops.layernorm_fwd(x0, pre.weight, pre.bias, a.eps,
+                                               save_stats=save, out_bf16=True if _RESID_BF16 else None,
+                                               out_f32=None if _RESID_BF16 else True)
+        x, saved = _stack_fwd(xb if _RESID_BF16 else xf, self.enc.encoder, sh["layers"], a, B, P + 1, None, False, save, ln0=ln0)
         if keep_cls and x.dtype == torch.float32:
             out = x.view(B, P + 1, a.hidden)
         else:
@@ -361,8 +368,12 @@
             g16 = ops.cast_bf16(g32)
         elif _GRAD_STREAM_BF16:
             g32 = None
-            g16 = torch.zeros(B * (P + 1), C, dtype=torch.bfloat16, device=gout.device)
-            ops.rows_copy(gout.reshape(B * P, C).float().contiguous(), P, 0, P + 1, 1, B, P, dst_bf16=g16)
+            if ops.edge_fuse():
+                g16 = torch.empty(B * (P + 1), C, dtype=torch.bfloat16, device=gout.device)
+                ops.rows_copy(gout.reshape(B * P, C).float().contiguous(), P, 0, P + 1, 1, B, P, dst_bf16=g16, zero_fill=True)
+            else:
+                g16 = torch.zeros(B * (P + 1), C, dtype=torch.bfloat16, device=gout.device)
+                ops.rows_copy(gout.reshape(B * P, C).float().contiguous(), P, 0, P + 1, 1, B, P, dst_bf16=g16)
         else:
             g32 = torch.zeros(B * (P + 1), C, dtype=torch.float32, device=gout.device)
             ops.rows_copy(gout.reshape(B * P, C).float().contiguous(), P, 0, P + 1, 1, B, P, dst_f32=g32)
@@ -372,15 +383,19 @@
                               final_f32=False)
         dg, accg = vec_grad(self.enc.pre_layrnorm.weight)
         db, _ = vec_grad(self.enc.pre_layrnorm.bias)
-        dx0, _, _, _ = ops.layernorm_bwd(g32 if g32 is not None else g16, saved["x0"], self.enc.pre_layrnorm.weight, saved["m0"], saved["r0"],
-                                         dgamma=dg, dbeta=db, accumulate=accg, want_bf16=False,
-                                         need_param_grads=dg is not None)
         emb = self.enc.embeddings
         gpos, accp = grad_buf(emb.position_embedding.weight)
         gcls, accc = grad_buf(emb.class_embedding)
         if accp != accc:
             raise RuntimeError("lc2is_amd: inconsistent gradient state of the ViT embeddings")
-        dpatch = ops.vit_embed_bwd(dx0, gpos, gcls, B, P, accumulate=accp)
+        if ops.edge_fuse() and g32 is None and C <= ops.VIT_EMBED_LN_BWD_CMAX:
+            dpatch = ops.vit_embed_ln_bwd(g16, saved["x0"], self.enc.pre_layrnorm.weight, saved["m0"], saved["r0"], gpos, gcls, B, P,
+                                          dgamma=dg, dbeta=db, accumulate_ln=accg, accumulate_emb=accp)
+        else:
+            dx0, _, _, _ = ops.layernorm_bwd(g32 if g32 is not None else g16, saved["x0"], self.enc.pre_layrnorm.weight, saved["m0"], saved["r0"],
+                                             dgamma=dg, dbeta=db, accumulate=accg, want_bf16=False,
+                                             need_param_grads=dg is not None)
+            dpatch = ops.vit_embed_bwd(dx0, gpos, gcls, B, P, accumulate=accp)
         gw, accw = grad_buf(emb.patch_embedding.weight)
         k = 3 * self.patch_size ** 2
         if sh["kpad"] == k:
diff --git a/lc2is_amd/nn/model.py b/lc2is_amd/nn/model.py
--- a/lc2is_amd/nn/model.py
+++ b/lc2is_amd/nn/model.py
@@ -86,6 +86,10 @@
         return loss2[0], None
     inv = loss2[1].masked_fill(loss2[1] == 0, 1.0).reciprocal() if save else None
     return loss2[0] / loss2[1], inv
+
+
+def _dev_scalar(t, like) -> bool:
+    return t.dtype == torch.float32 and t.numel() == 1 and t.device == like.device
 
 
 class _HeadFn(torch.autograd.Function):
@@ -171,10 +175,15 @@
             labels, info = ops.ohem_labels(scores, labels, B, g, g, K, 4, ops.INTERP_BICUBIC, ignore_index, ohem)
             self.last_ohem = (labels, info)
         if loss_opts is None:
+            fused_mean = ops.edge_fuse()
             loss2, dlo, _ = ops.head_upsample_ce(scores, labels.contiguous(), B, g, g, K, 4, ops.INTERP_BICUBIC,
-                                                 want_grad=save, ignore_index=ignore_index, grad_scale=1.0)
-            loss = loss2[0] / loss2[1]
-            inv_count = (1.0 / loss2[1].clamp_min(1.0)) if save else None
+                                                 want_grad=save, ignore_index=ignore_index, grad_scale=1.0, want_mean=fused_mean)
+            if fused_mean:
+                loss = loss2[2]
+                inv_count = loss2[3] if save else None
+            else:
+                loss = loss2[0] / loss2[1]
+                inv_count = (1.0 / loss2[1].clamp_min(1.0)) if save else None
         else:
             weight, label_smoothing, reduction = loss_opts
             loss2, dlo, _ = ops.head_upsample_ce(scores, labels.contiguous(), B, g, g, K, 4, ops.INTERP_BICUBIC,
@@ -191,7 +200,9 @@
         if saved["fused"] is not None:
             ds = saved["fused"]
             inv = saved["inv_count"]
-            if inv is None:
+            if inv is not None and ops.edge_fuse() and (gout is None or _dev_scalar(gout, ds)) and _dev_scalar(inv, ds):
+                ds16 = ops.scale_cast_bf16(ds, inv, None) if gout is None else ops.scale_cast_bf16(ds, gout, inv)
+            elif inv is None:
                 ds16 = ops.cast_bf16(ds if gout is None else ds * gout)
             else:
                 ds16 = ops.cast_bf16(ds * (inv if gout is None else gout * inv))
diff --git a/lc2is_amd/ops.py b/lc2is_amd/ops.py
--- a/lc2is_amd/ops.py
+++ b/lc2is_amd/ops.py
@@ -49,6 +49,11 @@
     "lc2is_text_embed_bwd": [_P, _P, _I, _P, _P, _I, _I, _I, _I, _I, _P],
     "lc2is_rows_copy_bf16": [_P, _I, _I, _P, _P, _I, _I, _I, _I, _I, _P],
     "lc2is_rows_copy_f32": [_P, _I, _I, _P, _P, _I, _I, _I, _I, _I, _P],
+    "lc2is_vit_embed_ln2_fwd": [_P, _I, _P, _P, _P, _P, _P, _P, _P, _P, _P, _P, _P, _P, _P, _I, _I, _I, _F, _P],
+    "lc2is_vit_embed_ln_bwd": [_P, _P, _P, _P, _P, _P, _I, _P, _P, _P, _P, _I, _I, _I, _I, _I, _P, _Z, _P],
+    "lc2is_rows_copy_zfill": [_P, _I, _I, _I, _P, _P, _I, _I, _I, _I, _I, _P],
+    "lc2is_scale_cast_bf16": [_P, _I, _P, _P, _P, _I, _I, _I, _P],
+    "lc2is_head_upsample_ce_mean": [_P, _I, _P, _P, _P, _I, _I, _I, _I, _I, _I, C.c_long, _F, _P, _Z, _P],
     "lc2is_sgd_step": [_P, _P, _P, _Z, _F, _F, _F, _F, _P],
     "lc2is_adamw_step": [_P, _P, _P, _P, _Z, _F, _F, _F, _F, _F, _I, _F, _P],
     "lc2is_grad_sumsq_blocks": [_Z],
@@ -573,6 +578,25 @@
         _lib.check(rc, "shadow_refresh")
 
 
+def edge_fuse() -> bool:
+    return os.environ.get("LC2IS_EDGE_FUSE", "1") != "0"
+
+
+def scale_cast_bf16(src: torch.Tensor, a: torch.Tensor, b: torch.Tensor | None = None, out: torch.Tensor | None = None):
+    _chk(src, torch.float32, "src")
+    for t, name in ((a, "a"), (b, "b")):
+        if t is not None:
+            _chk(t, torch.float32, name, None)
+            if t.numel() != 1:
+                raise RuntimeError(f"lc2is_amd.scale_cast_bf16: {name} must hold one element")
+    M, Cc = src.shape
+    out = out if out is not None else torch.empty((M, Cc), dtype=torch.bfloat16, device=src.device)
+    _chk(out, torch.bfloat16, "out")
+    _lib.check(_fn("lc2is_scale_cast_bf16")(_ptr(src), _ld(src), _ptr(a), _ptr(b), _ptr(out), _ld(out), M, Cc, _stream()),
+               "scale_cast_bf16")
+    return out
+
+
 def cast_bf16(src: torch.Tensor, out: torch.Tensor | None = None):
     _chk(src, torch.float32, "src")
     M, Cc = src.shape
@@ -623,6 +647,64 @@
     return dpatch
 
 
+VIT_EMBED_LN_BWD_CMAX = 1024
+
+
+def vit_embed_ln2_fwd(patch_f32, cls, pos, gamma_a, beta_a, gamma_b, beta_b, B: int, P: int, eps: float, *,
+                      save: bool = True):
+    _chk(patch_f32, torch.float32, "patch"); _chk(cls, torch.float32, "cls", 1); _chk(pos, torch.float32, "pos")
+    for t, name in ((gamma_a, "gamma_a"), (beta_a, "beta_a"), (gamma_b, "gamma_b"), (beta_b, "beta_b")):
+        _chk(t, torch.float32, name, 1)
+    Cc = patch_f32.shape[1]
+    if patch_f32.shape[0] != B * P or tuple(pos.shape) != (P + 1, Cc) or not pos.is_contiguous() or cls.numel() != Cc:
+        raise RuntimeError("lc2is_amd.vit_embed_ln2_fwd: patch [B*P, C], pos contiguous [P+1, C], cls [C] expected")
+    for t in (gamma_a, beta_a, gamma_b, beta_b):
+        if t is not None and t.numel() != Cc:
+            raise RuntimeError("lc2is_amd.vit_embed_ln2_fwd: LayerNorm vectors must have C elements")
+    dev, M = patch_f32.device, B * (P + 1)
+    f32 = dict(dtype=torch.float32, device=dev)
+    x0 = torch.empty((M, Cc), **f32) if save else None
+    xf = torch.empty((M, Cc), **f32)
+    h = torch.empty((M, Cc), dtype=torch.bfloat16, device=dev)
+    ma, ra, mb, rb = (torch.empty((M,), **f32) if save else None for _ in range(4))
+    rc = _fn("lc2is_vit_embed_ln2_fwd")(_ptr(patch_f32), _ld(patch_f32), _ptr(cls), _ptr(pos), _ptr(gamma_a), _ptr(beta_a),
+                                        _ptr(gamma_b), _ptr(beta_b), _ptr(x0), _ptr(xf), _ptr(h), _ptr(ma), _ptr(ra), _ptr(mb),
+                                        _ptr(rb), B, P, Cc, float(eps), _stream())
+    _lib.check(rc, f"vit_embed_ln2_fwd B={B} P={P} C={Cc}")
+    return x0, xf, h, ma, ra, mb, rb
+
+
+def vit_embed_ln_bwd(dy, x0, gamma, mean, rstd, dpos, dcls, B: int, P: int, *, dgamma=None, dbeta=None,
+                     accumulate_ln: bool = False, accumulate_emb: bool = False):
+    _chk(dy, torch.bfloat16, "dy"); _chk(x0, torch.float32, "x0"); _chk(gamma, torch.float32, "gamma", 1)
+    _chk(mean, torch.float32, "mean", 1); _chk(rstd, torch.float32, "rstd", 1)
+    _chk(dpos, torch.float32, "dpos"); _chk(dcls, torch.float32, "dcls", 1)
+    _chk(dgamma, torch.float32, "dgamma", 1); _chk(dbeta, torch.float32, "dbeta", 1)
+    M, Cc = x0.shape
+    if M != B * (P + 1) or tuple(dy.shape) != (M, Cc) or not dy.is_contiguous() or not x0.is_contiguous():
+        raise RuntimeError("lc2is_amd.vit_embed_ln_bwd: dy and x0 must be contiguous [B*(P+1), C]")
+    if mean.numel() != M or rstd.numel() != M or gamma.numel() != Cc or dcls.numel() != Cc or \
+            tuple(dpos.shape) != (P + 1, Cc) or not dpos.is_contiguous():
+        raise RuntimeError("lc2is_amd.vit_embed_ln_bwd: mean / rstd [M], gamma / dcls [C], dpos contiguous [P+1, C] expected")
+    dev = x0.device
+    dpatch = torch.empty((B * P, Cc), dtype=torch.bfloat16, device=dev)
+    nbytes = _fn("lc2is_layernorm_bwd_workspace_bytes")(M, Cc)
+    want = dgamma is not None or dbeta is not None
+    defer = _ln_defer if want else None
+    if defer is not None:
+        ws = torch.empty(max(int(nbytes), 16), dtype=torch.uint8, device=dev)
+        defer.append((ws, _fn("lc2is_layernorm_bwd_partials")(M, Cc), Cc, dgamma, dbeta, bool(accumulate_ln)))
+        pg, pb = None, None
+    else:
+        ws = workspace(nbytes, dev, "ln_bwd")
+        pg, pb = dgamma, dbeta
+    rc = _fn("lc2is_vit_embed_ln_bwd")(_ptr(dy), _ptr(x0), _ptr(gamma), _ptr(mean), _ptr(rstd), _ptr(dpatch), Cc, _ptr(dpos),
+                                       _ptr(dcls), _ptr(pg), _ptr(pb), int(accumulate_ln), int(accumulate_emb), B, P, Cc,
+                                       _ptr(ws), ws.numel(), _stream())
+    _lib.check(rc, f"vit_embed_ln_bwd B={B} P={P} C={Cc}")
+    return dpatch
+
+
 def text_embed_fwd(ids, tok, pos):
     _chk(ids, torch.int64, "input_ids"); _chk(tok, torch.float32, "tok"); _chk(pos, torch.float32, "pos")
     if not ids.is_contiguous():
@@ -644,7 +726,7 @@
 
 
 def rows_copy(src, S_src: int, src_off: int, S_dst: int, dst_off: int, B: int, n: int, *, dst_f32=None,
-              dst_bf16=None):
+              dst_bf16=None, zero_fill: bool = False):
     sb = src.dtype == torch.bfloat16
     _chk(src, torch.bfloat16 if sb else torch.float32, "src")
     Cc = src.shape[1]
@@ -653,6 +735,10 @@
     for t in (dst_f32, dst_bf16):
         if t is not None and (not t.is_contiguous() or tuple(t.shape) != (B * S_dst, Cc)):
             raise RuntimeError("lc2is_amd.rows_copy: dst must be contiguous [B*S_dst, C]")
+    if zero_fill:
+        _lib.check(_fn("lc2is_rows_copy_zfill")(_ptr(src), int(sb), S_src, src_off, _ptr(dst_f32), _ptr(dst_bf16), S_dst, dst_off,
+                                                B, n, Cc, _stream()), "rows_copy_zfill")
+        return
     _lib.check(_fn("lc2is_rows_copy_bf16" if sb else "lc2is_rows_copy_f32")(_ptr(src), S_src, src_off, _ptr(dst_f32), _ptr(dst_bf16),
                                                                             S_dst, dst_off, B, n, Cc, _stream()), "rows_copy")
 
@@ -790,7 +876,8 @@
 
 def head_upsample_ce(scores_lo, labels, B: int, h: int, w: int, C: int, S: int, mode: int = INTERP_BICUBIC, *,
                      want_grad: bool = False, want_scores: bool = False, want_loss: bool = True,
-                     ignore_index: int = -100, grad_scale: float = 1.0, class_weight=None, label_smoothing: float = 0.0):
+                     ignore_index: int = -100, grad_scale: float = 1.0, class_weight=None, label_smoothing: float = 0.0,
+                     want_mean: bool = False):
     _chk(scores_lo, torch.float32, "scores_lo"); _chk(labels, torch.int64, "labels", 3)
     opts = _ce_options(class_weight, label_smoothing, C, scores_lo.device) and want_loss
     if not scores_lo.is_contiguous():
@@ -801,11 +888,16 @@
         raise RuntimeError(f"lc2is_amd.head_upsample_ce: labels must be contiguous [{B},{h*S},{w*S}]")
     nbytes = _fn("lc2is_head_upsample_ce_workspace_bytes")(B, h, w, C, S, mode, int(want_grad)) if want_loss else 0
     alloc = torch.empty if nbytes else torch.zeros
-    loss = alloc(2, dtype=torch.float32, device=dev) if want_loss else None
+    if want_mean and (opts or want_scores or not want_loss or not nbytes):
+        raise RuntimeError("lc2is_amd.head_upsample_ce: want_mean needs S in {4, 8, 16}, a loss, and neither options nor scores")
+    loss = alloc(4 if want_mean else 2, dtype=torch.float32, device=dev) if want_loss else None
     dlo = alloc(scores_lo.shape, dtype=torch.float32, device=dev) if want_grad else None
     hi = torch.empty((B, C, h * S, w * S), dtype=torch.float32, device=dev) if want_scores else None
     ws = torch.empty(nbytes, dtype=torch.uint8, device=dev) if nbytes else None
-    if opts:
+    if want_mean:
+        rc = _fn("lc2is_head_upsample_ce_mean")(_ptr(scores_lo), ld, _ptr(labels), _ptr(dlo), _ptr(loss), B, h, w, C, S, mode,
+                                                ignore_index, grad_scale, _ptr(ws), nbytes, _stream())
+    elif opts:
         rc = _fn("lc2is_head_upsample_ce_opts")(_ptr(scores_lo), ld, _ptr(labels), _ptr(dlo), _ptr(hi), _ptr(loss), B, h,
                                                 w, C, S, mode, ignore_index, grad_scale, _ptr(class_weight),
                                                 label_smoothing, _ptr(ws), nbytes, _stream())
```

Result: no change. 1075 images/s (-0.2%).
